# choi403/ALG

Measured on AMD Instinct MI355X. Metric: frames/sec (whole node) CogVideoX-5B-I2V 49f x 50-step ALG, higher is better.
Workload: dtype bf16; 1 GPU; BASELINE config 2: CogVideoX-5B-I2V bf16, 49 frames @ 480x720, 50 steps, ALG interval down_up (resize_factor 0.25, interval [0, 0.04]), guidance 6.0; one video per GPU; layers=42, dit_sample_forwards=12, parallelism=dp1

## Files before the change

alg_amd/_lib.py:

```python
from __future__ import annotations

import ctypes
from collections import OrderedDict
import os
from ctypes import POINTER, Structure, byref, c_char_p, c_float, c_int, c_int32, c_int64, c_void_p

import torch

_HERE = os.path.dirname(os.path.abspath(__file__))
LIB_PATH = os.environ.get("ALG_HIP_LIB") or os.path.join(_HERE, "libalg_hip.so")

ALG_F32, ALG_BF16 = 0, 1
ACT_NONE, ACT_GELU_TANH, ACT_SILU = 0, 1, 2
GEMM_BIAS_PER_ROW, GEMM_PERMUTE_COLS, GEMM_GATE_F32, GEMM_GATE_SEG_STRIDE = 1, 4, 8, 16
GEMM_B_PACKED11 = 32

EXPORTS = (
    "alg_version", "alg_last_error", "alg_reload_env", "alg_down_up", "alg_gaussian_blur", "alg_cfg_ddim_step", "alg_gemm_bf16", "alg_gemm_bf16_pair", "alg_gemm_bf16_pair_qk", "alg_pack_b_p11", "alg_pack_b_p11_bytes",
    "alg_flash_attn_d64", "alg_layernorm_modulate", "alg_layernorm_modulate_fp8", "alg_qk_norm_rope", "alg_patchify", "alg_unpatchify",
    "alg_timestep_embedding", "alg_cfg_combine", "alg_lincomb", "alg_unipc_update", "alg_concat_cast", "alg_flash_attn_d128", "alg_layernorm_mod_f32", "alg_layernorm_mod_f32_fp8", "alg_rmsnorm_rope",
    "alg_wan_modulation", "alg_patchify3d", "alg_unpatchify3d", "alg_timestep_embedding_f32", "alg_linear_f32",
    "alg_gelu_erf", "alg_layernorm_modulate_seg", "alg_headnorm_rope", "alg_masked_mean", "alg_silu", "alg_gemm_fp8", "alg_quantize_fp8_rows",
    "alg_conv_cl_bf16", "alg_vae_groupnorm_workspace", "alg_vae_groupnorm_stats", "alg_vae_spatial_norm", "alg_vae_upsample",
    "alg_vae_pack_latent", "alg_vae_unpack_video", "alg_vae_group_norm", "alg_vae_pad", "alg_vae_repitch",
    "alg_vae_unpack_planes", "alg_rms_norm_rows", "alg_softmax_hilo", "alg_flash_attn_d128_ex", "alg_flash_attn_d128_dual", "alg_rope_half", "alg_patchify_t", "alg_unpatchify_t", "alg_qk_norm_rope_scaled", "alg_flash_attn_d64_ex", "alg_embed_rows", "alg_t5_layernorm", "alg_attn_bias", "alg_mul_bf16", "alg_quick_gelu",
    "alg_lowpass_tables_bytes", "alg_lowpass_tables_build", "alg_down_up_workspace_bytes", "alg_gaussian_blur_workspace_bytes",
    "alg_flash_attn_d64_workspace_bytes", "alg_calib_mfma_bf16", "alg_wall_clock_khz", "alg_attn_clock_tap",
    "alg_flash_attn_d128_fp8", "alg_quantize_fp8_khead", "alg_quantize_fp8_vt", "alg_rmsnorm_rope_fp8", "alg_headnorm_rope_fp8",
)
_RET_I64 = ("alg_vae_groupnorm_workspace", "alg_lowpass_tables_bytes", "alg_down_up_workspace_bytes",
            "alg_gaussian_blur_workspace_bytes", "alg_flash_attn_d64_workspace_bytes", "alg_pack_b_p11_bytes")


class AlgHipError(RuntimeError):
    pass


class GemmArgs(Structure):
    _fields_ = [
        ("A", c_void_p), ("B", c_void_p), ("C", c_void_p), ("bias", c_void_p), ("R", c_void_p), ("gate", c_void_p),
        ("lda", c_int64), ("ldb", c_int64), ("ldc", c_int64), ("ldr", c_int64),
        ("strideA", c_int64), ("strideB", c_int64), ("strideC", c_int64), ("strideR", c_int64),
        ("strideGate", c_int64),
        ("M", c_int32), ("N", c_int32), ("K", c_int32), ("batch", c_int32),
        ("seg_split", c_int32), ("act", c_int32), ("flags", c_int32),
        ("gate_seg_stride", c_int64), ("perm_col0", c_int32), ("conv_cin_log2", c_int32),
        ("a_scale", c_void_p), ("b_scale", c_void_p), ("strideAScale", c_int64), ("strideBScale", c_int64),
        ("conv_wp", c_int32), ("conv_hpwp", c_int32), ("conv_kw", c_int32), ("reserved1", c_int32),
    ]


class QkNormRopeArgs(Structure):
    _fields_ = [("wq", c_void_p), ("bq", c_void_p), ("wk", c_void_p), ("bk", c_void_p), ("cos_tab", c_void_p),
                ("sin_tab", c_void_p), ("heads", c_int32), ("text_len", c_int32), ("eps", c_float),
                ("q_scale", c_float)]


class VaeGeom(Structure):
    _fields_ = [(n, c_int32) for n in ("frames", "H", "W", "C", "first_len", "seg_len", "lat_first_single", "lat_rate",
                                       "lat_scale", "lat_h", "lat_w")]


_lib = None


def build_library(verbose=False):
    import subprocess

    src = os.path.join(_HERE, "csrc")
    r = subprocess.run(["make", "-C", src, "-j8"], capture_output=True, text=True)
    if verbose or r.returncode != 0:
        print(r.stdout[-4000:])
        print(r.stderr[-4000:])
    if r.returncode != 0:
        raise AlgHipError("building libalg_hip.so failed (see output above)")
    return LIB_PATH


def load_library():
    global _lib
    if _lib is not None:
        return _lib
    if not os.path.exists(LIB_PATH):
        raise AlgHipError(
            "%s not found: the HIP extension is not built (run `python -c 'import __graft_entry__ as g; g.build()'` "
            "or `make -C alg_amd/csrc`).  There is no CPU fallback for the ALG hot path." % LIB_PATH)
    lib = ctypes.CDLL(LIB_PATH)
    lib.alg_version.restype = c_int
    lib.alg_last_error.restype = c_char_p
    lib.alg_reload_env.restype = None
    lib.alg_reload_env.argtypes = []
    lib.alg_down_up.argtypes = [c_void_p, c_void_p, c_int64, c_int, c_int, c_int, c_int, c_int, c_int, c_void_p, c_void_p,
                                c_int64, c_void_p]
    lib.alg_gaussian_blur.argtypes = [c_void_p, c_void_p, c_int64, c_int, c_int, c_int, c_float, c_int, c_void_p, c_int64,
                                      c_void_p]
    lib.alg_lowpass_tables_bytes.argtypes = [c_int] * 4
    lib.alg_lowpass_tables_build.argtypes = [c_void_p, c_int64] + [c_int] * 4 + [c_void_p]
    lib.alg_down_up_workspace_bytes.argtypes = [c_int64] + [c_int] * 4
    lib.alg_gaussian_blur_workspace_bytes.argtypes = [c_int64] + [c_int] * 3
    lib.alg_flash_attn_d64_workspace_bytes.argtypes = [c_int] * 4
    lib.alg_pack_b_p11_bytes.argtypes = [c_int, c_int]
    lib.alg_pack_b_p11_bytes.restype = c_int64
    lib.alg_pack_b_p11.argtypes = [c_void_p, c_void_p, c_int, c_int, c_int64, c_void_p]
    lib.alg_cfg_ddim_step.argtypes = [c_void_p, c_int, c_void_p, c_int, c_int, c_int64, c_float, c_float, c_float,
                                      c_float, c_float, c_void_p]
    lib.alg_cfg_combine.argtypes = [c_void_p, c_void_p, c_int, c_int, c_int64, c_float, c_void_p]
    lib.alg_lincomb.argtypes = [POINTER(c_void_p), POINTER(c_float), POINTER(c_int), c_int, c_void_p, c_int, c_int64,
                                c_void_p]
    lib.alg_concat_cast.argtypes = [POINTER(c_void_p), c_int, POINTER(c_void_p), c_int, c_int] + [c_int64] * 7 + [
        c_void_p, c_int, c_void_p]
    lib.alg_flash_attn_d128.argtypes = [c_void_p] * 4 + [c_int] * 4 + [c_int64] * 8 + [c_float, c_void_p]
    lib.alg_flash_attn_d128_ex.argtypes = [c_void_p] * 4 + [c_int] * 4 + [c_int64] * 8 + [c_float, c_int, c_int, c_void_p]
    lib.alg_flash_attn_d128_dual.argtypes = ([c_void_p] * 3 + [c_int] + [c_int64] * 4 + [c_void_p] * 2 + [c_int] + [c_int64] * 4 +
                                             [c_void_p] + [c_int] * 3 + [c_int64] * 4 + [c_float, c_void_p])
    lib.alg_flash_attn_d128_fp8.argtypes = [c_void_p] * 7 + [c_int] * 4 + [c_int64] * 8 + [c_float, c_int, c_int, c_void_p]
    lib.alg_quantize_fp8_khead.argtypes = [c_void_p, c_int64, c_int64, c_void_p, c_int64, c_int64, c_void_p] + [c_int] * 4 + [c_void_p]
    lib.alg_quantize_fp8_vt.argtypes = [c_void_p, c_int64, c_int64, c_void_p, c_int64, c_int64, c_void_p] + [c_int] * 4 + [c_void_p]
    lib.alg_rmsnorm_rope_fp8.argtypes = [c_void_p] * 4 + [c_int64, c_int, c_int, c_int, c_float, c_void_p, c_int64, c_void_p,
                                         c_void_p, c_void_p]
    lib.alg_headnorm_rope_fp8.argtypes = [c_void_p] * 4 + [c_int64, c_int64, c_int, c_int, c_int, c_int, c_float, c_void_p, c_int64,
                                          c_int64, c_void_p, c_int64, c_void_p, c_void_p]
    lib.alg_rope_half.argtypes = [c_void_p, c_void_p, c_void_p, c_void_p, c_int64, c_int, c_int64, c_void_p]
    lib.alg_layernorm_mod_f32.argtypes = [c_void_p] * 6 + [c_int64, c_int, c_int, c_int, c_float, c_void_p]
    lib.alg_layernorm_mod_f32_fp8.argtypes = [c_void_p] * 7 + [c_int64, c_int, c_int, c_int, c_float, c_void_p]
    lib.alg_rmsnorm_rope.argtypes = [c_void_p] * 4 + [c_int64, c_int, c_int, c_int, c_float, c_void_p]
    lib.alg_wan_modulation.argtypes = [c_void_p] * 3 + [c_int] * 5 + [c_void_p]
    lib.alg_patchify3d.argtypes = [c_void_p, c_void_p] + [c_int] * 8 + [c_void_p]
    lib.alg_unpatchify3d.argtypes = [c_void_p, c_int64, c_void_p] + [c_int] * 8 + [c_void_p]
    lib.alg_layernorm_modulate_seg.argtypes = [c_void_p] * 6 + [c_int64, c_int64, c_int, c_int, c_int, c_int64, c_int64,
                                               c_int, c_float, c_void_p]
    lib.alg_headnorm_rope.argtypes = [c_void_p] * 4 + [c_int64, c_int64, c_int, c_int, c_int, c_int, c_float, c_void_p]
    lib.alg_masked_mean.argtypes = [c_void_p, c_void_p, c_void_p, c_int, c_int, c_int, c_void_p]
    lib.alg_silu.argtypes = [c_void_p, c_void_p, c_int64, c_void_p]
    lib.alg_rms_norm_rows.argtypes = [c_void_p, c_void_p, c_void_p, c_int64, c_int, c_int, c_int, c_void_p]
    lib.alg_softmax_hilo.argtypes = [c_void_p, c_void_p, c_void_p, c_int64, c_int, c_int64, ctypes.c_float, c_void_p]
    lib.alg_gemm_fp8.argtypes = [POINTER(GemmArgs), c_void_p]
    lib.alg_conv_cl_bf16.argtypes = [c_void_p] * 5 + [c_int] * 7 + [c_void_p]
    lib.alg_vae_groupnorm_workspace.argtypes = [POINTER(VaeGeom)]
    lib.alg_vae_groupnorm_stats.argtypes = [c_void_p, POINTER(VaeGeom), c_float, c_void_p, c_void_p, c_void_p]
    lib.alg_vae_spatial_norm.argtypes = [c_void_p] * 6 + [POINTER(VaeGeom), c_int, c_void_p]
    lib.alg_vae_group_norm.argtypes = [c_void_p] * 5 + [POINTER(VaeGeom), c_int, c_void_p]
    lib.alg_vae_pad.argtypes = [c_void_p, c_void_p] + [c_int] * 4 + [c_void_p]
    lib.alg_vae_repitch.argtypes = [c_void_p, c_void_p] + [c_int] * 6 + [c_void_p]
    lib.alg_vae_unpack_planes.argtypes = [c_void_p, c_void_p] + [c_int] * 4 + [c_void_p]
    lib.alg_embed_rows.argtypes = [c_void_p, c_void_p, c_void_p, c_int64, c_int, c_int, c_void_p]
    lib.alg_t5_layernorm.argtypes = [c_void_p, c_void_p, c_void_p, c_int64, c_int, c_float, c_void_p]
    lib.alg_attn_bias.argtypes = [c_void_p] * 7 + [c_int, c_int, c_int, c_int, c_int64, c_int64, c_float, c_int, c_void_p]
    lib.alg_quick_gelu.argtypes = [c_void_p, c_int64, c_void_p]
    lib.alg_mul_bf16.argtypes = [c_void_p, c_void_p, c_void_p, c_int64, c_void_p]
    lib.alg_vae_upsample.argtypes = [c_void_p, c_void_p] + [c_int] * 6 + [c_void_p]
    lib.alg_vae_pack_latent.argtypes = [c_void_p, c_int64, c_int64, c_void_p, c_int, c_int, c_int, c_int, c_float, c_void_p]
    lib.alg_vae_unpack_video.argtypes = [c_void_p, c_void_p, c_int, c_int, c_int, c_int, c_void_p]
    lib.alg_quantize_fp8_rows.argtypes = [c_void_p, c_int64, c_void_p, c_void_p, c_int64, c_int, c_void_p]
    lib.alg_timestep_embedding_f32.argtypes = [c_void_p, c_void_p, c_int, c_int, c_void_p]
    lib.alg_linear_f32.argtypes = [c_void_p] * 6 + [c_int] * 4 + [c_void_p]
    lib.alg_gelu_erf.argtypes = [c_void_p, c_int64, c_void_p]
    lib.alg_unipc_update.argtypes = [c_void_p] * 5 + [c_int64] + [c_float] * 6 + [c_void_p]
    lib.alg_gemm_bf16.argtypes = [POINTER(GemmArgs), c_void_p]
    lib.alg_gemm_bf16_pair.argtypes = [POINTER(GemmArgs), POINTER(GemmArgs), c_void_p]
    lib.alg_gemm_bf16_pair_qk.argtypes = [POINTER(GemmArgs), POINTER(GemmArgs), POINTER(QkNormRopeArgs), c_void_p]
    lib.alg_flash_attn_d64.argtypes = [c_void_p, c_void_p, c_void_p, c_void_p, c_int, c_int, c_int, c_int64, c_int64,
                                       c_int64, c_int64, c_int64, c_int64, c_float, c_void_p]
    lib.alg_layernorm_modulate.argtypes = [c_void_p, c_void_p, c_void_p, c_void_p, c_void_p, c_void_p, c_int64, c_int,
                                           c_int, c_int, c_int64, c_int64, c_int, c_float, c_void_p]
    lib.alg_layernorm_modulate_fp8.argtypes = [c_void_p] * 7 + [c_int64, c_int, c_int, c_int, c_int64, c_int, c_float, c_void_p]
    lib.alg_qk_norm_rope.argtypes = [c_void_p, c_void_p, c_void_p, c_void_p, c_void_p, c_void_p, c_void_p, c_int,
                                     c_int, c_int, c_int, c_float, c_void_p]
    lib.alg_qk_norm_rope_scaled.argtypes = [c_void_p] * 7 + [c_int, c_int, c_int, c_int, c_float, c_float, c_void_p]
    lib.alg_flash_attn_d64_ex.argtypes = [c_void_p, c_void_p, c_void_p, c_void_p, c_int, c_int, c_int, c_int64, c_int64,
                                          c_int64, c_int64, c_int64, c_int64, c_float, c_int, c_void_p, c_int64, c_void_p]
    lib.alg_patchify.argtypes = [c_void_p, c_int64, POINTER(c_void_p), c_void_p, c_int, c_int, c_int, c_int, c_int,
                                 c_int, c_void_p]
    lib.alg_unpatchify.argtypes = [c_void_p, c_void_p, c_int, c_int, c_int, c_int, c_int, c_int, c_void_p]
    lib.alg_patchify_t.argtypes = [c_void_p, c_int64, POINTER(c_void_p), c_void_p] + [c_int] * 7 + [c_void_p]
    lib.alg_unpatchify_t.argtypes = [c_void_p, c_void_p] + [c_int] * 7 + [c_void_p]
    lib.alg_timestep_embedding.argtypes = [c_void_p, c_void_p, c_int, c_int, c_int, c_void_p]
    lib.alg_calib_mfma_bf16.argtypes = [c_void_p, c_int, ctypes.c_uint, c_int, c_void_p, c_void_p]
    lib.alg_attn_clock_tap.argtypes = [c_void_p, c_int]
    for name in EXPORTS:
        fn = getattr(lib, name)
        if name == "alg_attn_clock_tap":
            fn.restype = None
        elif name not in ("alg_version", "alg_last_error", "alg_reload_env"):
            fn.restype = c_int64 if name in _RET_I64 else c_int
    _lib = lib
    return lib


def reload_env():
    load_library().alg_reload_env()


def _check(rc, what):
    if rc != 0:
        msg = load_library().alg_last_error()
        raise AlgHipError("%s failed (code %d): %s" % (what, rc, msg.decode() if msg else "?"))


def _stream():
    return c_void_p(torch.cuda.current_stream().cuda_stream)


def _dt(t):
    if t.dtype == torch.float32:
        return ALG_F32
    if t.dtype == torch.bfloat16:
        return ALG_BF16
    raise AlgHipError("unsupported dtype %s (the HIP path handles float32 and bfloat16)" % t.dtype)


def _dev(t, name):
    if not t.is_cuda:
        raise AlgHipError("%s must be a device tensor: the ALG hot path is HIP-only (no CPU fallback)" % name)
    return t


def _ptr(t):
    return c_void_p(t.data_ptr()) if t is not None else c_void_p(0)



_TABLES = OrderedDict()
_TABLES_MAX = 64
_SCRATCH = {}
_PINNED = {}


def _stream_key(t):
    return (t.device.index, torch.cuda.current_stream(t.device).cuda_stream)


def _capturing():
    return torch.cuda.is_available() and torch.cuda.is_current_stream_capturing()


def _pin(t):
    _PINNED[id(t)] = t
    return t


def release_captured_buffers():
    _PINNED.clear()


def clear_caches():
    _TABLES.clear()
    _SCRATCH.clear()


def lowpass_tables(x, h1, w1):
    lib = load_library()
    H, W = x.shape[-2:]
    key = _stream_key(x) + (H, W, h1, w1)
    cap = _capturing()
    t = _TABLES.get(key)
    if t is not None:
        _TABLES.move_to_end(key)
        return _pin(t) if cap else t
    n = int(lib.alg_lowpass_tables_bytes(H, W, h1, w1))
    if n <= 0:
        return None
    t = torch.empty(n, dtype=torch.uint8, device=x.device)
    _check(lib.alg_lowpass_tables_build(_ptr(t), n, H, W, h1, w1, _stream()), "alg_lowpass_tables_build")
    if cap:
        return _pin(t)
    _TABLES[key] = t
    while len(_TABLES) > _TABLES_MAX:
        _TABLES.popitem(last=False)
    return t


def scratch(ref, nbytes, tag):
    if nbytes <= 0:
        return None
    key = _stream_key(ref) + (tag,)
    t = _SCRATCH.get(key)
    cap = _capturing()
    if t is None or t.numel() < nbytes:
        t = torch.empty(int(nbytes), dtype=torch.uint8, device=ref.device)
        if cap:
            return _pin(t)
        _SCRATCH[key] = t
    return _pin(t) if cap else t


def calib_mfma_bf16(sink, iters, seed=1, blocks=0, clocks=None):
    lib = load_library()
    if clocks is not None:
        if int(blocks) <= 0:
            blocks = 2 * torch.cuda.get_device_properties(sink.device).multi_processor_count
        if not (clocks.is_cuda and clocks.device == sink.device and clocks.dtype == torch.int64 and clocks.is_contiguous()
                and clocks.numel() >= 4 * int(blocks)):
            raise AlgHipError("calib_mfma_bf16: clocks must be a contiguous int64 tensor on the sink's device with >= 4 * %d "
                              "elements" % int(blocks))
    rc = lib.alg_calib_mfma_bf16(_ptr(_dev(sink, "sink")), int(iters), int(seed), int(blocks), _ptr(clocks), _stream())
    if rc <= 0:
        _check(rc if rc < 0 else -1, "alg_calib_mfma_bf16")
    return rc


def wall_clock_khz():
    return int(load_library().alg_wall_clock_khz())


def attn_clock_tap(buffer):
    lib = load_library()
    if buffer is None:
        lib.alg_attn_clock_tap(None, 0)
        return
    if not (buffer.is_cuda and buffer.dtype == torch.int64 and buffer.is_contiguous() and buffer.dim() == 2 and buffer.shape[1] == 4):
        raise AlgHipError("attn_clock_tap needs a contiguous int64 device tensor [slots, 4]")
    lib.alg_attn_clock_tap(_ptr(buffer), int(buffer.shape[0]))


def clock_mhz_from_taps(taps, wall_khz):
    t = taps.detach().cpu().to(torch.float64)
    dc, dw = t[:, 2] - t[:, 0], t[:, 3] - t[:, 1]
    ok = (dc > 0) & (dw > 0)
    if not bool(ok.any()) or wall_khz <= 0:
        return None
    mhz = dc[ok] / dw[ok] * (wall_khz / 1e3)
    return {"mean": float(mhz.mean()), "min": float(mhz.min()), "max": float(mhz.max()), "workgroups": int(ok.sum())}


def down_up(x, h1, w1, round_intermediate=True):
    lib = load_library()
    _dev(x, "x")
    if not x.is_contiguous():
        raise AlgHipError("down_up needs a contiguous tensor")
    H, W = x.shape[-2:]
    planes = x.numel() // (H * W) if x.numel() else 0
    out = torch.empty_like(x)
    if planes == 0:
        return out
    wsb = int(lib.alg_down_up_workspace_bytes(planes, H, W, h1, w1))
    ws = scratch(x, wsb, "down_up")
    tables = lowpass_tables(x, h1, w1) if wsb == 0 else None
    _check(lib.alg_down_up(_ptr(x), _ptr(out), planes, H, W, h1, w1, _dt(x), 1 if round_intermediate else 0,
                           _ptr(tables), _ptr(ws), wsb, _stream()), "alg_down_up")
    return out


def gaussian_blur(x, ksize, sigma):
    lib = load_library()
    _dev(x, "x")
    if not x.is_contiguous():
        raise AlgHipError("gaussian_blur needs a contiguous tensor")
    H, W = x.shape[-2:]
    planes = x.numel() // (H * W) if x.numel() else 0
    out = torch.empty_like(x)
    wsb = int(lib.alg_gaussian_blur_workspace_bytes(planes, H, W, int(ksize))) if planes else 0
    ws = scratch(x, wsb, "gaussian")
    _check(lib.alg_gaussian_blur(_ptr(x), _ptr(out), planes, H, W, int(ksize), float(sigma), _dt(x), _ptr(ws), wsb,
                                 _stream()), "alg_gaussian_blur")
    return out


def cfg_ddim_step_(pred, latents, n_pass, guidance_scale, sqrt_alpha_t, sqrt_beta_t, coef_a, coef_b):
    lib = load_library()
    _dev(pred, "pred")
    _dev(latents, "latents")
    if not (pred.is_contiguous() and latents.is_contiguous()):
        raise AlgHipError("cfg_ddim_step_ needs contiguous tensors")
    numel = latents.numel()
    if pred.numel() != n_pass * numel:
        raise AlgHipError("pred has %d elements, expected n_pass*numel = %d" % (pred.numel(), n_pass * numel))
    _check(lib.alg_cfg_ddim_step(_ptr(pred), _dt(pred), _ptr(latents), _dt(latents), n_pass, numel,
                                 float(guidance_scale), float(sqrt_alpha_t), float(sqrt_beta_t), float(coef_a),
                                 float(coef_b), _stream()), "alg_cfg_ddim_step")
    return latents


def cfg_combine(pred, n_pass, guidance_scale):
    lib = load_library()
    _dev(pred, "pred")
    if not pred.is_contiguous() or pred.shape[0] % n_pass:
        raise AlgHipError("cfg_combine needs a contiguous [n_pass * B, ...] tensor")
    out = torch.empty((pred.shape[0] // n_pass,) + tuple(pred.shape[1:]), device=pred.device, dtype=pred.dtype)
    _check(lib.alg_cfg_combine(_ptr(pred), _ptr(out), _dt(pred), n_pass, out.numel(), float(guidance_scale), _stream()),
           "alg_cfg_combine")
    return out


def lincomb(terms, out_dtype, out=None):
    lib = load_library()
    xs = [t for _, t in terms]
    for t in xs:
        _dev(t, "term")
        if not t.is_contiguous() or t.shape != xs[0].shape:
            raise AlgHipError("lincomb needs contiguous tensors of one shape")
    n = len(xs)
    if out is None:
        out = torch.empty(xs[0].shape, device=xs[0].device, dtype=out_dtype)
    elif out.dtype != out_dtype or out.shape != xs[0].shape or not out.is_contiguous():
        raise AlgHipError("lincomb: `out` must be a contiguous tensor of the requested dtype and shape")
    arr = (c_void_p * n)(*[t.data_ptr() for t in xs])
    cf = (c_float * n)(*[float(c) for c, _ in terms])
    dts = (c_int * n)(*[_dt(t) for t in xs])
    _check(lib.alg_lincomb(arr, cf, dts, n, _ptr(out), ALG_F32 if out_dtype == torch.float32 else ALG_BF16,
                           out.numel(), _stream()), "alg_lincomb")
    return out


def concat_cast(src0, src1, O, A0, A1, R, s0_ostride, s1_ostride, a1_off, out_dtype):
    lib = load_library()
    n = len(src0)
    for t in list(src0) + list(src1):
        _dev(t, "concat source")
        if not t.is_contiguous():
            raise AlgHipError("concat_cast needs contiguous sources")
    out = torch.empty((n, O, A0 + A1, R), device=src0[0].device, dtype=out_dtype)
    a0 = (c_void_p * n)(*[t.data_ptr() for t in src0])
    a1 = (c_void_p * n)(*[t.data_ptr() for t in src1])
    _check(lib.alg_concat_cast(a0, _dt(src0[0]), a1, _dt(src1[0]), n, O, A0, A1, R, s0_ostride, s1_ostride, a1_off,
                               _ptr(out), ALG_F32 if out_dtype == torch.float32 else ALG_BF16, _stream()),
           "alg_concat_cast")
    return out


def rope_half_(x, cos, sin, pos, rows, heads, x_rstride, x_off=0):
    _check(load_library().alg_rope_half(_p(x, x_off), _p(cos), _p(sin), _p(pos), rows, heads, x_rstride, _stream()),
           "alg_rope_half")
    return x


def flash_attn_d128_dual(q, k, vt, Skv, k_bs, k_rs, vt_bs, vt_rs, k2, vt2, Skv2, k2_bs, k2_rs, vt2_bs, vt2_rs, o, batch, heads, Sq,
                         q_bs, q_rs, o_bs, o_rs, scale):
    lib = load_library()
    for t in (q, k, vt, k2, vt2, o):
        _dev(t, "attention operand")
    _check(lib.alg_flash_attn_d128_dual(_p(q), _p(k), _p(vt), Skv, k_bs, k_rs, vt_bs, vt_rs, _p(k2), _p(vt2), Skv2, k2_bs, k2_rs,
                                        vt2_bs, vt2_rs, _p(o), batch, heads, Sq, q_bs, q_rs, o_bs, o_rs, float(scale), _stream()),
           "alg_flash_attn_d128_dual")
    return o


def flash_attn_d128(q, k, vt, o, batch, heads, Sq, Skv, q_bs, q_rs, k_bs, k_rs, vt_bs, vt_rs, o_bs, o_rs, scale,
                    q_off=0, k_off=0, vt_off=0, o_off=0, kv_group=1, causal=False):
    lib = load_library()
    for t in (q, k, vt, o):
        _dev(t, "attention operand")
    at = lambda t, off: c_void_p(t.data_ptr() + 2 * off)
    if kv_group != 1 or causal:
        _check(lib.alg_flash_attn_d128_ex(at(q, q_off), at(k, k_off), at(vt, vt_off), at(o, o_off), batch, heads, Sq, Skv, q_bs,
                                          q_rs, k_bs, k_rs, vt_bs, vt_rs, o_bs, o_rs, float(scale), int(kv_group),
                                          int(bool(causal)), _stream()), "alg_flash_attn_d128_ex")
        return o
    _check(lib.alg_flash_attn_d128(at(q, q_off), at(k, k_off), at(vt, vt_off), at(o, o_off), batch, heads, Sq, Skv, q_bs, q_rs, k_bs, k_rs, vt_bs, vt_rs, o_bs, o_rs, float(scale),
                                   _stream()), "alg_flash_attn_d128")
    return o


def flash_attn_d128_fp8(q8, q_scale, k8, k_scale, vt8, vt_scale, o, batch, heads, Sq, Skv, q_bs, q_rs, k_bs, k_rs, vt_bs, vt_rs,
                        o_bs, o_rs, scale, q_off=0, qs_off=0, k_off=0, ks_off=0, vt_off=0, vts_off=0, o_off=0, kv_group=1,
                        causal=False):
    lib = load_library()
    for t in (q8, q_scale, k8, k_scale, vt8, vt_scale, o):
        _dev(t, "attention operand")
    for t in (q8, k8, vt8):
        if t.element_size() != 1:
            raise AlgHipError("flash_attn_d128_fp8 takes e4m3 bytes (uint8 / float8_e4m3fn), got %s" % t.dtype)
    _check(lib.alg_flash_attn_d128_fp8(_p(q8, q_off), _p(q_scale, qs_off), _p(k8, k_off), _p(k_scale, ks_off), _p(vt8, vt_off),
                                       _p(vt_scale, vts_off), _p(o, o_off), batch, heads, Sq, Skv, q_bs, q_rs, k_bs, k_rs, vt_bs,
                                       vt_rs, o_bs, o_rs, float(scale), int(kv_group), int(bool(causal)), _stream()),
           "alg_flash_attn_d128_fp8")
    return o


def quantize_fp8_khead(x, q, scale, batch, heads, S, x_bs, x_rs, q_bs, q_rs, x_off=0, q_off=0, scale_off=0, scale_given=False):
    _check(load_library().alg_quantize_fp8_khead(_p(x, x_off), x_bs, x_rs, _p(q, q_off), q_bs, q_rs, _p(scale, scale_off), batch,
                                                 heads, S, int(bool(scale_given)), _stream()), "alg_quantize_fp8_khead")
    return q, scale


def quantize_fp8_vt(x, q, scale, batch, rows, Skv, x_bs, x_rs, q_bs, q_rs, src_permuted=True, x_off=0, q_off=0, scale_off=0):
    _check(load_library().alg_quantize_fp8_vt(_p(x, x_off), x_bs, x_rs, _p(q, q_off), q_bs, q_rs, _p(scale, scale_off), batch,
                                              rows, Skv, int(bool(src_permuted)), _stream()), "alg_quantize_fp8_vt")
    return q, scale


def rmsnorm_rope_fp8(x, weight, cos, sin, x_rstride, batch, rows, D, eps, q8, q8_rstride, scale=None, head_scale=None, x_off=0,
                     q8_off=0, scale_off=0, hs_off=0):
    _check(load_library().alg_rmsnorm_rope_fp8(_p(x, x_off), _p(weight), _p(cos), _p(sin), x_rstride, batch, rows, D, float(eps),
                                               _p(q8, q8_off), q8_rstride, _p(scale, scale_off), _p(head_scale, hs_off), _stream()),
           "alg_rmsnorm_rope_fp8")
    return q8


def headnorm_rope_fp8(x, weight, cos, sin, x_rstride, x_bstride, batch, rows, heads, rope_tokens, eps, q8, q8_rstride, q8_bstride,
                      scale=None, scale_bstride=0, head_scale=None, x_off=0, q8_off=0, scale_off=0, hs_off=0):
    _check(load_library().alg_headnorm_rope_fp8(_p(x, x_off), _p(weight), _p(cos), _p(sin), x_rstride, x_bstride, batch, rows,
                                                heads, rope_tokens, float(eps), _p(q8, q8_off), q8_rstride, q8_bstride,
                                                _p(scale, scale_off), scale_bstride, _p(head_scale, hs_off), _stream()),
           "alg_headnorm_rope_fp8")
    return q8


def _p(t, off=0):
    if t is None:
        return c_void_p(0)
    _dev(t, "tensor")
    return c_void_p(t.data_ptr() + off * t.element_size())


def layernorm_mod_f32(x, y, weight, bias, scale, shift, mod_bstride, batch, rows, D, eps, scale_off=0, shift_off=0):
    _check(load_library().alg_layernorm_mod_f32(_p(x), _p(y), _p(weight), _p(bias), _p(scale, scale_off),
                                                _p(shift, shift_off), mod_bstride, batch, rows, D, float(eps), _stream()),
           "alg_layernorm_mod_f32")
    return y


def layernorm_mod_f32_fp8(x, q8, q8_scale, weight, bias, scale, shift, mod_bstride, batch, rows, D, eps, scale_off=0,
                          shift_off=0):
    _check(load_library().alg_layernorm_mod_f32_fp8(_p(x), _p(q8), _p(q8_scale), _p(weight), _p(bias),
                                                    _p(scale, scale_off), _p(shift, shift_off), mod_bstride, batch, rows,
                                                    D, float(eps), _stream()), "alg_layernorm_mod_f32_fp8")
    return q8


def rmsnorm_rope_(x, weight, cos, sin, x_rstride, batch, rows, D, eps, x_off=0):
    _check(load_library().alg_rmsnorm_rope(_p(x, x_off), _p(weight), _p(cos), _p(sin), x_rstride, batch, rows, D,
                                           float(eps), _stream()), "alg_rmsnorm_rope")
    return x


def wan_modulation(table, vec, out, layers, batch, J, D, vec_per_j):
    _check(load_library().alg_wan_modulation(_p(table), _p(vec), _p(out), layers, batch, J, D, int(vec_per_j), _stream()),
           "alg_wan_modulation")
    return out


def patchify3d(x, out, n, C, F, H, W, ph, pw, Kpad):
    _check(load_library().alg_patchify3d(_p(x), _p(out), n, C, F, H, W, ph, pw, Kpad, _stream()), "alg_patchify3d")
    return out


def unpatchify3d(x, ldin, out, n, C, F, H, W, ph, pw, channel_major=False):
    _check(load_library().alg_unpatchify3d(_p(x), ldin, _p(out), n, C, F, H, W, ph, pw, int(channel_major), _stream()),
           "alg_unpatchify3d")
    return out


def layernorm_modulate_seg(x, y, weight, bias, scale, shift, mod_bstride, seg_stride, batch, rows, D, seg_split, eps,
                           x_bstride=None, y_bstride=None, x_off=0, y_off=0, scale_off=0, shift_off=0):
    x_bstride = rows * D if x_bstride is None else x_bstride
    y_bstride = rows * D if y_bstride is None else y_bstride
    _check(load_library().alg_layernorm_modulate_seg(_p(x, x_off), _p(y, y_off), _p(weight), _p(bias), _p(scale, scale_off),
                                                     _p(shift, shift_off), mod_bstride, seg_stride, batch, rows, D,
                                                     x_bstride, y_bstride, seg_split, float(eps), _stream()),
           "alg_layernorm_modulate_seg")
    return y


def headnorm_rope_(x, weight, cos, sin, x_rstride, x_bstride, batch, rows, heads, rope_tokens, eps, x_off=0):
    _check(load_library().alg_headnorm_rope(_p(x, x_off), _p(weight), _p(cos), _p(sin), x_rstride, x_bstride, batch, rows,
                                            heads, rope_tokens, float(eps), _stream()), "alg_headnorm_rope")
    return x


def masked_mean(x, valid, out, batch, L, D):
    _check(load_library().alg_masked_mean(_p(x), _p(valid), _p(out), batch, L, D, _stream()), "alg_masked_mean")
    return out


def silu(x, y):
    _check(load_library().alg_silu(_p(x), _p(y), x.numel(), _stream()), "alg_silu")
    return y


def rms_norm_rows(x, gamma, y, rows, C, Cp, silu=True):
    _check(load_library().alg_rms_norm_rows(_p(x), _p(gamma), _p(y), rows, C, Cp, int(silu), _stream()), "alg_rms_norm_rows")
    return y


def softmax_hilo(neg_hi, lo, p, rows, cols, ld, scale):
    _check(load_library().alg_softmax_hilo(_p(neg_hi), _p(lo), _p(p), rows, cols, ld, float(scale), _stream()),
           "alg_softmax_hilo")
    return p


CONV_PLAIN, CONV_PAIR, CONV_STRIDE2 = 0, 1, 2


def conv_cl(x, w, bias, res, y, frames, Hp, Wp, Cin, Cout, kt, pair=False, stride2=False, x_off=0, y_off=0, res_off=0):
    mode = CONV_STRIDE2 if stride2 else (CONV_PAIR if pair else CONV_PLAIN)
    _check(load_library().alg_conv_cl_bf16(_p(x, x_off), _p(w), _p(bias), _p(res, res_off), _p(y, y_off), frames, Hp, Wp,
                                           Cin, Cout, kt, mode, _stream()), "alg_conv_cl_bf16")
    return y


def embed_rows(ids, table, out):
    _check(load_library().alg_embed_rows(_p(ids), _p(table), _p(out), ids.numel(), table.shape[1], table.shape[0],
                                         _stream()), "alg_embed_rows")
    return out


def t5_layernorm(x, weight, y, rows, D, eps):
    _check(load_library().alg_t5_layernorm(_p(x), _p(weight), _p(y), rows, D, eps, _stream()), "alg_t5_layernorm")
    return y


def attn_bias(qkv, out, bias_table, rel_bucket, key_mask, batch, heads, L, scale=1.0, head_dim=64, causal=False):
    inner = heads * head_dim
    _check(load_library().alg_attn_bias(_p(qkv), _p(qkv, inner), _p(qkv, 2 * inner), _p(out), _p(bias_table),
                                        _p(rel_bucket), _p(key_mask), batch, heads, head_dim, L, 3 * inner, inner,
                                        float(scale), int(causal), _stream()), "alg_attn_bias")
    return out


def quick_gelu_(x):
    _check(load_library().alg_quick_gelu(_p(x), x.numel(), _stream()), "alg_quick_gelu")
    return x


def mul_bf16(a, b, out):
    _check(load_library().alg_mul_bf16(_p(a), _p(b), _p(out), a.numel(), _stream()), "alg_mul_bf16")
    return out


def vae_group_norm(x, stats, gamma, beta, out, g, silu=True):
    _check(load_library().alg_vae_group_norm(_p(x), _p(stats), _p(gamma), _p(beta), _p(out), byref(g), int(silu),
                                             _stream()), "alg_vae_group_norm")
    return out


def vae_pad(x, out, frames, H, W, C):
    _check(load_library().alg_vae_pad(_p(x), _p(out), frames, H, W, C, _stream()), "alg_vae_pad")
    return out


def vae_repitch(x, out, frames, H, W, C, src_rows, src_wp):
    _check(load_library().alg_vae_repitch(_p(x), _p(out), frames, H, W, C, src_rows, src_wp, _stream()), "alg_vae_repitch")
    return out


def vae_unpack_planes(x, out, frames, H, W, C):
    _check(load_library().alg_vae_unpack_planes(_p(x), _p(out), frames, H, W, C, _stream()), "alg_vae_unpack_planes")
    return out


def pack_conv_pair(w, bias, taps_t):
    co = w.shape[0]
    w = w.reshape(co, taps_t, 3, 3, -1)
    wp = w.new_zeros(2, co, taps_t, 3, 4, w.shape[-1])
    wp[0, :, :, :, 0:3] = w
    wp[1, :, :, :, 1:4] = w
    return wp.reshape(2 * co, -1).contiguous(), torch.cat([bias, bias]).contiguous()


def vae_geom(**kw):
    g = VaeGeom()
    for k, v in kw.items():
        setattr(g, k, v)
    return g


def vae_groupnorm_workspace(g):
    n = load_library().alg_vae_groupnorm_workspace(byref(g))
    if n < 0:
        _check(1, "alg_vae_groupnorm_workspace")
    return n


def vae_groupnorm_stats(x, g, eps, workspace, stats):
    _check(load_library().alg_vae_groupnorm_stats(_p(x), byref(g), eps, _p(workspace), _p(stats), _stream()),
           "alg_vae_groupnorm_stats")
    return stats


def vae_spatial_norm(x, stats, gamma, beta, zyb, out, g, silu=True):
    _check(load_library().alg_vae_spatial_norm(_p(x), _p(stats), _p(gamma), _p(beta), _p(zyb), _p(out), byref(g),
                                               int(silu), _stream()), "alg_vae_spatial_norm")
    return out


def vae_upsample(x, out, frames_out, H, W, C, compress_time, first_single):
    _check(load_library().alg_vae_upsample(_p(x), _p(out), frames_out, H, W, C, int(compress_time), int(first_single),
                                           _stream()), "alg_vae_upsample")
    return out


def vae_pack_latent(z, c_stride, frame_stride, out, frames, h, w, channels, scale, z_off=0):
    _check(load_library().alg_vae_pack_latent(_p(z, z_off), c_stride, frame_stride, _p(out), frames, h, w, channels, scale,
                                              _stream()), "alg_vae_pack_latent")
    return out


def vae_unpack_video(x, out, frames, H, W, to_uint8=False):
    _check(load_library().alg_vae_unpack_video(_p(x), _p(out), frames, H, W, int(to_uint8), _stream()),
           "alg_vae_unpack_video")
    return out


def timestep_embedding_f32(t, out, n, dim):
    _check(load_library().alg_timestep_embedding_f32(_p(t), _p(out), n, dim, _stream()), "alg_timestep_embedding_f32")
    return out


def linear_f32(x, W, b, y, y_bf16, y_silu_bf16, M, N, K, act=0):
    _check(load_library().alg_linear_f32(_p(x), _p(W), _p(b), _p(y), _p(y_bf16), _p(y_silu_bf16), M, N, K, act, _stream()),
           "alg_linear_f32")


def gelu_erf_(x):
    _check(load_library().alg_gelu_erf(_p(x), x.numel(), _stream()), "alg_gelu_erf")
    return x


def unipc_update(x, m0, m1, m_new, r, c, k, rk=1.0, rho0=0.0, rho_new=0.0):
    lib = load_library()
    for t in (x, m0, m1, m_new):
        if t is None:
            continue
        _dev(t, "unipc term")
        if t.dtype != torch.float32 or not t.is_contiguous() or t.shape != x.shape:
            raise AlgHipError("unipc_update needs contiguous fp32 tensors of one shape")
    out = torch.empty_like(x)
    p = lambda t: None if t is None else _ptr(t)
    _check(lib.alg_unipc_update(p(x), p(m0), p(m1), p(m_new), _ptr(out), x.numel(), float(r), float(c), float(k),
                                float(rk), float(rho0), float(rho_new), _stream()), "alg_unipc_update")
    return out


def gemm_args(A, B, C, M, N, K, lda, ldb, ldc, bias=None, R=None, ldr=0, gate=None, batch=1, strideA=0, strideB=0,
              strideC=0, strideR=0, strideGate=0, seg_split=0, act=ACT_NONE, flags=0, a_off=0, b_off=0, c_off=0, r_off=0,
              gate_off=0, gate_seg_stride=None, bias_off=0, perm_col0=0, a_scale=None, b_scale=None, strideAScale=0,
              strideBScale=0, a_scale_off=0, b_scale_off=0):
    args = GemmArgs()
    fp8 = a_scale is not None
    if isinstance(B, PackedB):
        if fp8:
            raise AlgHipError("a packed B holds bf16 weight fragments for GEMM schedule 11: the e4m3 GEMM takes a row-major B")
        if (B.N, B.K) != (N, K) or b_off or strideB:
            raise AlgHipError("packed B was built for N = %d, K = %d (shared by the batch, no offset)" % (B.N, B.K))
        flags |= GEMM_B_PACKED11
    args.A = A.data_ptr() + A.element_size() * a_off
    args.B = B.data_ptr() + B.element_size() * b_off
    if fp8:
        args.a_scale = a_scale.data_ptr() + 4 * a_scale_off
        args.b_scale = b_scale.data_ptr() + 4 * b_scale_off
        args.strideAScale, args.strideBScale = strideAScale, strideBScale
    args.C = C.data_ptr() + 2 * c_off
    args.bias = (bias.data_ptr() + 2 * bias_off) if bias is not None else None
    if gate_seg_stride is not None:
        flags |= GEMM_GATE_SEG_STRIDE
        args.gate_seg_stride = gate_seg_stride
    args.R = (R.data_ptr() + 2 * r_off) if R is not None else None
    args.gate = (gate.data_ptr() + gate.element_size() * gate_off) if gate is not None else None
    args.lda, args.ldb, args.ldc, args.ldr = lda, ldb, ldc, ldr
    args.strideA, args.strideB, args.strideC, args.strideR, args.strideGate = strideA, strideB, strideC, strideR, strideGate
    args.M, args.N, args.K, args.batch = M, N, K, batch
    args.seg_split, args.act, args.flags = seg_split, act, flags
    args.perm_col0 = perm_col0
    return args, fp8


class PackedB:

    def __init__(self, w):
        lib = load_library()
        _dev(w, "weight")
        if w.dtype != torch.bfloat16 or w.dim() != 2 or w.stride(1) != 1:
            raise AlgHipError("PackedB takes a 2-D bf16 weight with unit column stride")
        self.N, self.K = int(w.shape[0]), int(w.shape[1])
        nbytes = int(lib.alg_pack_b_p11_bytes(self.N, self.K))
        if nbytes <= 0:
            raise AlgHipError("PackedB: K = %d must be a positive multiple of 64" % self.K)
        self.data = torch.empty(nbytes, dtype=torch.uint8, device=w.device)
        _check(lib.alg_pack_b_p11(_ptr(w), _ptr(self.data), self.N, self.K, int(w.stride(0)), _stream()), "alg_pack_b_p11")

    def data_ptr(self):
        return self.data.data_ptr()

    def element_size(self):
        return 2


def gemm(*a, **kw):
    lib = load_library()
    args, fp8 = gemm_args(*a, **kw)
    if fp8:
        _check(lib.alg_gemm_fp8(ctypes.byref(args), _stream()), "alg_gemm_fp8")
    else:
        _check(lib.alg_gemm_bf16(ctypes.byref(args), _stream()), "alg_gemm_bf16")


def gemm_pair(first, second):
    lib = load_library()
    a, fa = gemm_args(*first[0], **first[1])
    b, fb = gemm_args(*second[0], **second[1])
    if fa or fb:
        raise AlgHipError("gemm_pair takes bf16 problems")
    _check(lib.alg_gemm_bf16_pair(ctypes.byref(a), ctypes.byref(b), _stream()), "alg_gemm_bf16_pair")


def gemm_pair_qk(first, second, wq, bq, wk, bk, cos, sin, heads, text_len, eps, q_scale=1.0):
    lib = load_library()
    a, fa = gemm_args(*first[0], **first[1])
    b, fb = gemm_args(*second[0], **second[1])
    if fa or fb:
        raise AlgHipError("gemm_pair_qk takes bf16 problems")
    ptrs = [t.data_ptr() if t is not None else None for t in (wq, bq, wk, bk, cos, sin)]
    e = QkNormRopeArgs(*ptrs, heads, text_len, float(eps), float(q_scale))
    _check(lib.alg_gemm_bf16_pair_qk(ctypes.byref(a), ctypes.byref(b), ctypes.byref(e), _stream()), "alg_gemm_bf16_pair_qk")


def quantize_fp8_rows(x, q, scale, rows, K, x_rstride=None, x_off=0, q_off=0, scale_off=0):
    x_rstride = K if x_rstride is None else x_rstride
    _check(load_library().alg_quantize_fp8_rows(_p(x, x_off), x_rstride, _p(q, q_off), _p(scale, scale_off), rows, K,
                                                _stream()), "alg_quantize_fp8_rows")
    return q, scale


ATTN_Q_PRESCALED = 1


def flash_attn_d64(q, k, vt, o, batch, heads, S, q_bstride, q_rstride, vt_bstride, vt_rstride, o_bstride, o_rstride,
                   scale, q_off=0, k_off=0, q_prescaled=False):
    lib = load_library()
    flags = ATTN_Q_PRESCALED if q_prescaled else 0
    wsb = int(lib.alg_flash_attn_d64_workspace_bytes(batch, heads, S, flags))
    ws = scratch(o, wsb, "attn_d64")
    _check(lib.alg_flash_attn_d64_ex(c_void_p(q.data_ptr() + 2 * q_off), c_void_p(k.data_ptr() + 2 * k_off), _ptr(vt),
                                     _ptr(o), batch, heads, S, q_bstride, q_rstride, vt_bstride, vt_rstride, o_bstride,
                                     o_rstride, float(scale), flags, _ptr(ws), wsb, _stream()),
           "alg_flash_attn_d64")


def layernorm_modulate(x, y, weight, bias, scale, shift, mod_bstride, batch, rows, D, seg_split, eps,
                       x_bstride=None, y_bstride=None, x_off=0, y_off=0, scale_off=0, shift_off=0):
    lib = load_library()
    x_bstride = rows * D if x_bstride is None else x_bstride
    y_bstride = rows * D if y_bstride is None else y_bstride
    sc = c_void_p(scale.data_ptr() + 2 * scale_off) if scale is not None else c_void_p(0)
    sh = c_void_p(shift.data_ptr() + 2 * shift_off) if shift is not None else c_void_p(0)
    _check(lib.alg_layernorm_modulate(c_void_p(x.data_ptr() + 2 * x_off), c_void_p(y.data_ptr() + 2 * y_off),
                                      _ptr(weight), _ptr(bias), sc, sh, mod_bstride, batch, rows, D, x_bstride,
                                      y_bstride, seg_split, float(eps), _stream()), "alg_layernorm_modulate")


def layernorm_modulate_fp8(x, q8, q8_scale, weight, bias, scale, shift, mod_bstride, batch, rows, D, seg_split, eps,
                           x_bstride=None, x_off=0, scale_off=0, shift_off=0, q8_off=0, q8_scale_off=0):
    x_bstride = rows * D if x_bstride is None else x_bstride
    _check(load_library().alg_layernorm_modulate_fp8(_p(x, x_off), _p(q8, q8_off), _p(q8_scale, q8_scale_off), _p(weight), _p(bias),
                                                     _p(scale, scale_off), _p(shift, shift_off), mod_bstride, batch, rows, D,
                                                     x_bstride, seg_split, float(eps), _stream()), "alg_layernorm_modulate_fp8")
    return q8, q8_scale


def qk_norm_rope_(qk, wq, bq, wk, bk, cos, sin, batch, S, heads, text_len, eps, q_scale=1.0):
    lib = load_library()
    _check(lib.alg_qk_norm_rope_scaled(_ptr(qk), _ptr(wq), _ptr(bq), _ptr(wk), _ptr(bk), _ptr(cos), _ptr(sin), batch, S,
                                       heads, text_len, float(eps), float(q_scale), _stream()), "alg_qk_norm_rope")


def patchify(latents, lat_bstride, conds, out, n_samples, frames, C, H, W, p, p_t=1):
    lib = load_library()
    arr = (c_void_p * n_samples)(*[c.data_ptr() for c in conds])
    _check(lib.alg_patchify_t(_ptr(latents), lat_bstride, arr, _ptr(out), n_samples, frames, C, H, W, p, p_t, _stream()),
           "alg_patchify")


def unpatchify(x, out, n_samples, frames, C, H, W, p, p_t=1):
    lib = load_library()
    _check(lib.alg_unpatchify_t(_ptr(x), _ptr(out), n_samples, frames, C, H, W, p, p_t, _stream()), "alg_unpatchify")


def timestep_embedding(t, out, n, dim, flip_sin_to_cos=True):
    lib = load_library()
    _check(lib.alg_timestep_embedding(_ptr(t), _ptr(out), n, dim, 1 if flip_sin_to_cos else 0, _stream()),
           "alg_timestep_embedding")
```

alg_amd/csrc/gemm.hip:

```cpp
#include <stdlib.h>

#include "common.h"

namespace alg {
constexpr int BM = 256, BN = 256;
int launch_gemm_p6(const alg_gemm_args* a, int m_tiles, int n_tiles, int64_t nwg, hipStream_t s);
int launch_gemm_p9(const alg_gemm_args* a, int m_tiles, int n_tiles, int64_t nwg, hipStream_t s);
int launch_gemm_p9_pair(const alg_gemm_args* a, int m_tiles_a, int n_tiles_a, const alg_gemm_args* b, int m_tiles_b, int n_tiles_b,
                        hipStream_t s);
int launch_gemm_p9_pair_qk(const alg_gemm_args* a, int m_tiles_a, int n_tiles_a, const alg_gemm_args* b, int m_tiles_b, int n_tiles_b,
                           const alg_qk_norm_rope_args* e, hipStream_t s);
int launch_gemm_p10(const alg_gemm_args* a, int m_tiles, int n_tiles, int64_t nwg, hipStream_t s);
int launch_gemm_p10_pair(const alg_gemm_args* a, int m_tiles_a, int n_tiles_a, const alg_gemm_args* b, int m_tiles_b, int n_tiles_b,
                         hipStream_t s);
int launch_gemm_p10_pair_qk(const alg_gemm_args* a, int m_tiles_a, int n_tiles_a, const alg_gemm_args* b, int m_tiles_b, int n_tiles_b,
                            const alg_qk_norm_rope_args* e, hipStream_t s);
int launch_gemm_p11(const alg_gemm_args* a, int m_tiles, int n_tiles, int64_t nwg, hipStream_t s);
int launch_gemm_p6_fp8(const alg_gemm_args* a, int m_tiles, int n_tiles, int64_t nwg, hipStream_t s);
int launch_gemm_p9_fp8(const alg_gemm_args* a, int m_tiles, int n_tiles, int64_t nwg, hipStream_t s);
int launch_gemm_p6_conv(const alg_gemm_args* a, int m_tiles, int n_tiles, int64_t nwg, hipStream_t s);
static int gemm_pipe() { return opt(OPT_GEMM_PIPE); }
static bool asm_pipe() { return gemm_pipe() == 9 || gemm_pipe() == 10; }
}

using namespace alg;

static int gemm_entry(const alg_gemm_args* a, void* stream, bool fp8, bool validate_only = false) {
  if (!a || !a->A || !a->B || !a->C) {
    set_error("alg_gemm_bf16: null argument");
    return ALG_EINVAL;
  }
  if (a->M <= 0 || a->N <= 0 || a->K <= 0 || a->batch <= 0) {
    set_error("alg_gemm_bf16: bad shape M=%d N=%d K=%d batch=%d", a->M, a->N, a->K, a->batch);
    return ALG_EINVAL;
  }
  if (a->K % (fp8 ? 128 : 64) != 0) {
    set_error("alg_gemm_%s: K=%d must be a multiple of %d", fp8 ? "fp8" : "bf16", a->K, fp8 ? 128 : 64);
    return ALG_EINVAL;
  }
  const int al = fp8 ? 16 : 8;
  if (a->lda % al || a->ldb % al || a->strideA % al || a->strideB % al || ((uintptr_t)a->A & 15) ||
      ((uintptr_t)a->B & 15)) {
    set_error("alg_gemm: A/B must be 16-byte aligned with lda/ldb/strides multiples of 16 bytes");
    return ALG_EINVAL;
  }
  if (fp8 && (!a->a_scale || !a->b_scale || ((uintptr_t)a->b_scale & 15) || (a->strideBScale & 3))) {
    set_error("alg_gemm_fp8: a_scale / b_scale are required (b_scale 16-byte aligned)");
    return ALG_EINVAL;
  }
  if (a->act < ALG_ACT_NONE || a->act > ALG_ACT_SILU) {
    set_error("alg_gemm_bf16: unknown activation %d", a->act);
    return ALG_EINVAL;
  }
  if ((a->flags & ALG_GEMM_PERMUTE_COLS) && (a->R || a->gate)) {
    set_error("alg_gemm_bf16: PERMUTE_COLS cannot be combined with residual/gate");
    return ALG_EINVAL;
  }
  if (a->R && a->act != ALG_ACT_NONE) {
    set_error("alg_gemm_bf16: an activation cannot be combined with the residual epilogue");
    return ALG_EINVAL;
  }
  if (a->gate && !a->R) {
    set_error("alg_gemm_bf16: gate needs a residual");
    return ALG_EINVAL;
  }
  if ((a->N & 3) == 0) {
    const bool bad = (a->ldc & 3) || (a->strideC & 3) || ((uintptr_t)a->C & 7) ||
                     (a->bias && !(a->flags & ALG_GEMM_BIAS_PER_ROW) && ((uintptr_t)a->bias & 7)) ||
                     (a->R && ((a->ldr & 3) || (a->strideR & 3) || ((uintptr_t)a->R & 7))) ||
                     (a->gate && ((a->strideGate & 3) ||
                                  ((uintptr_t)a->gate & ((a->flags & ALG_GEMM_GATE_F32) ? 15 : 7))));
    if (bad) {
      set_error("alg_gemm_bf16: C/bias/R/gate must be 8-byte aligned with ldc/ldr/strides multiples of 4 elements");
      return ALG_EINVAL;
    }
  }
  if (a->conv_wp) {
    const int cl = a->conv_cin_log2;
    const int taps = (cl >= 6 && cl <= 12) ? a->K >> cl : 0;
    const int kw = a->conv_kw;
    if (fp8 || (kw != 3 && kw != 4) || (taps != 3 * kw && taps != 9 * kw) || (taps << cl) != a->K ||
        (a->lda != ((int64_t)(kw - 2) << cl) && !(kw == 3 && a->lda == (2ll << cl))) || a->conv_wp < 3 ||
        a->conv_hpwp < 3 * a->conv_wp || a->act != ALG_ACT_NONE ||
        ((2ll * a->conv_hpwp + 2ll * a->conv_wp + 3) << cl) >= (1ll << 31)) {
      set_error("alg_gemm_bf16: bad convolution addressing (cin_log2=%d K=%d lda=%lld wp=%d hpwp=%d)", cl, a->K,
                (long long)a->lda, a->conv_wp, a->conv_hpwp);
      return ALG_EINVAL;
    }
  }
  if (a->flags & ALG_GEMM_B_PACKED11) {
    if (fp8) {
      set_error("alg_gemm_fp8: a packed B (ALG_GEMM_B_PACKED11) holds bf16 fragments for schedule 11; the e4m3 GEMM reads a row-major B");
      return ALG_EINVAL;
    }
    if (a->conv_wp) {
      set_error("alg_gemm_bf16: convolution addressing cannot be combined with a packed B (ALG_GEMM_B_PACKED11)");
      return ALG_EINVAL;
    }
    if (a->K < 128 || 256 * a->lda * 2 + (int64_t)a->K * 2 >= (1ll << 32) || a->strideB != 0 ||
        (a->flags & (ALG_GEMM_BIAS_PER_ROW | ALG_GEMM_PERMUTE_COLS)) || ((uintptr_t)a->B & 15)) {
      set_error("alg_gemm_bf16: a packed B (ALG_GEMM_B_PACKED11) needs K >= 128, 32-bit byte offsets inside a 256-row A panel, a B shared by "
                "the batch (strideB = 0) and a plain column layout (no per-row bias / column permutation)");
      return ALG_EINVAL;
    }
  }
  if (validate_only) return ALG_OK;
  if ((int64_t)a->M * a->ldc >= (1ll << 31) || (a->R && (int64_t)a->M * a->ldr >= (1ll << 31))) {
    const int64_t ld = (a->R && a->ldr > a->ldc) ? a->ldr : a->ldc;
    const int64_t rows = ((1ll << 31) - 1) / ld / BM * BM;
    if (a->conv_wp || rows <= 0) {
      set_error("alg_gemm_bf16: M*ldc must stay below 2^31 (32-bit epilogue offsets)");
      return ALG_ELIMIT;
    }
    const int64_t esz = fp8 ? 1 : 2;
    for (int64_t m0 = 0; m0 < a->M; m0 += rows) {
      alg_gemm_args c = *a;
      c.M = (int32_t)((a->M - m0) < rows ? (a->M - m0) : rows);
      c.A = (const char*)a->A + m0 * a->lda * esz;
      c.C = (char*)a->C + m0 * a->ldc * 2;
      if (a->R) c.R = (const char*)a->R + m0 * a->ldr * 2;
      if (a->bias && (a->flags & ALG_GEMM_BIAS_PER_ROW)) c.bias = (const char*)a->bias + m0 * 2;
      if (a->a_scale) c.a_scale = a->a_scale + m0;
      c.seg_split = a->seg_split > m0 ? (int32_t)(a->seg_split - m0) : 0;
      const int rc = gemm_entry(&c, stream, fp8);
      if (rc != ALG_OK) return rc;
    }
    return ALG_OK;
  }
  const int m_tiles = (a->M + BM - 1) / BM, n_tiles = (a->N + BN - 1) / BN;
  const int64_t nwg = (int64_t)m_tiles * n_tiles * a->batch;
  if (nwg > 0x7fffffff) {
    set_error("alg_gemm_bf16: grid too large");
    return ALG_ELIMIT;
  }
  hipStream_t s = (hipStream_t)stream;
  if (fp8) {
    if (asm_pipe() && a->K >= 256 && 256 * a->lda + (int64_t)a->K < (1ll << 32) && 256 * a->ldb + (int64_t)a->K < (1ll << 32))
      return launch_gemm_p9_fp8(a, m_tiles, n_tiles, nwg, s);
    return launch_gemm_p6_fp8(a, m_tiles, n_tiles, nwg, s);
  }
  if (a->conv_wp) return launch_gemm_p6_conv(a, m_tiles, n_tiles, nwg, s);
  if (a->flags & ALG_GEMM_B_PACKED11) return launch_gemm_p11(a, m_tiles, n_tiles, nwg, s);
  switch (gemm_pipe()) {
    case 9:
    case 10:
      if (a->K >= 128 && 256 * a->lda * 2 + (int64_t)a->K * 2 < (1ll << 32) && 256 * a->ldb * 2 + (int64_t)a->K * 2 < (1ll << 32))
        return gemm_pipe() == 10 ? launch_gemm_p10(a, m_tiles, n_tiles, nwg, s) : launch_gemm_p9(a, m_tiles, n_tiles, nwg, s);
      return launch_gemm_p6(a, m_tiles, n_tiles, nwg, s);
    default: return launch_gemm_p6(a, m_tiles, n_tiles, nwg, s);
  }
}

extern "C" int alg_gemm_bf16(const alg_gemm_args* a, void* stream) { return gemm_entry(a, stream, false); }

static bool pair_eligible(const alg_gemm_args* a) {
  return a && a->A && a->B && a->C && !(a->flags & ALG_GEMM_B_PACKED11) && !a->R && !a->gate && a->act == ALG_ACT_NONE &&
         !a->conv_wp && a->M > 0 && a->N > 0 && a->batch > 0 && a->K >= 128 && a->K % 64 == 0 && 256 * a->lda * 2 + (int64_t)a->K * 2 < (1ll << 32) &&
         256 * a->ldb * 2 + (int64_t)a->K * 2 < (1ll << 32) && (int64_t)a->M * a->ldc < (1ll << 31) &&
         !(a->lda % 8 || a->ldb % 8 || a->strideA % 8 || a->strideB % 8 || ((uintptr_t)a->A & 15) || ((uintptr_t)a->B & 15)) &&
         ((a->N & 3) != 0 || !((a->ldc & 3) || (a->strideC & 3) || ((uintptr_t)a->C & 7) ||
                               (a->bias && !(a->flags & ALG_GEMM_BIAS_PER_ROW) && ((uintptr_t)a->bias & 7))));
}

extern "C" int alg_gemm_bf16_pair(const alg_gemm_args* a, const alg_gemm_args* b, void* stream) {
  int rc = gemm_entry(a, stream, false, true);
  if (rc == ALG_OK) rc = gemm_entry(b, stream, false, true);
  if (rc != ALG_OK) return rc;
  if (asm_pipe() && pair_eligible(a) && pair_eligible(b)) {
    const int64_t ta = (int64_t)((a->M + BM - 1) / BM) * ((a->N + BN - 1) / BN) * a->batch;
    const int64_t tb = (int64_t)((b->M + BM - 1) / BM) * ((b->N + BN - 1) / BN) * b->batch;
    if (ta + tb <= 0x7fffffff)
      return (gemm_pipe() == 10 ? launch_gemm_p10_pair : launch_gemm_p9_pair)(a, (a->M + BM - 1) / BM, (a->N + BN - 1) / BN, b, (b->M + BM - 1) / BM, (b->N + BN - 1) / BN,
                                 (hipStream_t)stream);
  }
  rc = gemm_entry(a, stream, false);
  return rc != ALG_OK ? rc : gemm_entry(b, stream, false);
}

extern "C" int alg_gemm_bf16_pair_qk(const alg_gemm_args* a, const alg_gemm_args* b, const alg_qk_norm_rope_args* e, void* stream) {
  int rc = gemm_entry(a, stream, false, true);
  if (rc == ALG_OK) rc = gemm_entry(b, stream, false, true);
  if (rc != ALG_OK) return rc;
  if (!e || !e->wq || !e->bq || !e->wk || !e->bk || e->heads <= 0 || e->text_len < 0 || e->text_len > a->M ||
      (e->cos_tab == nullptr) != (e->sin_tab == nullptr)) {
    set_error("alg_gemm_bf16_pair_qk: bad LayerNorm / rotary arguments");
    return ALG_EINVAL;
  }
  if (((uintptr_t)e->wq & 15) || ((uintptr_t)e->bq & 15) || ((uintptr_t)e->wk & 15) || ((uintptr_t)e->bk & 15) ||
      ((uintptr_t)e->cos_tab & 15) || ((uintptr_t)e->sin_tab & 15) || ((uintptr_t)a->C & 15)) {
    set_error("alg_gemm_bf16_pair_qk: pointers must be 16-byte aligned");
    return ALG_EINVAL;
  }
  if (a->N != 2 * e->heads * 64 || a->ldc != a->N || a->strideC != (int64_t)a->M * a->N || (a->flags & ALG_GEMM_PERMUTE_COLS) ||
      a->R || a->act != ALG_ACT_NONE) {
    set_error("alg_gemm_bf16_pair_qk: qk must be a plain GEMM onto the contiguous [batch][S][2][heads][64] tensor (N=%d heads=%d ldc=%lld)",
              a->N, e->heads, (long long)a->ldc);
    return ALG_EINVAL;
  }
  const bool fused = asm_pipe() && pair_eligible(a) && pair_eligible(b) && e->heads % 4 == 0 &&
                     !(a->bias && (a->flags & ALG_GEMM_BIAS_PER_ROW));
  if (fused) {
    const int64_t ta = (int64_t)((a->M + BM - 1) / BM) * ((a->N + BN - 1) / BN) * a->batch;
    const int64_t tb = (int64_t)((b->M + BM - 1) / BM) * ((b->N + BN - 1) / BN) * b->batch;
    if (ta + tb <= 0x7fffffff)
      return (gemm_pipe() == 10 ? launch_gemm_p10_pair_qk : launch_gemm_p9_pair_qk)(a, (a->M + BM - 1) / BM, (a->N + BN - 1) / BN, b, (b->M + BM - 1) / BM, (b->N + BN - 1) / BN, e,
                                    (hipStream_t)stream);
  }
  rc = alg_gemm_bf16_pair(a, b, stream);
  if (rc != ALG_OK) return rc;
  return alg_qk_norm_rope_scaled(a->C, e->wq, e->bq, e->wk, e->bk, e->cos_tab, e->sin_tab, a->batch, a->M, e->heads, e->text_len,
                                 e->eps, e->q_scale, stream);
}

extern "C" int alg_gemm_fp8(const alg_gemm_args* a, void* stream) { return gemm_entry(a, stream, true); }

extern "C" int alg_conv_cl_bf16(const void* x, const void* w, const void* bias, const void* res, void* y, int frames,
                                int Hp, int Wp, int Cin, int Cout, int kt, int mode, void* stream) {
  const bool pair = mode == ALG_CONV_PAIR, down = mode == ALG_CONV_STRIDE2;
  if (frames <= 0 || Hp < 3 || Wp < 3 || (kt != 1 && kt != 3) || Cin < 64 || (Cin & (Cin - 1)) || Cout <= 0 || (Cout & 3) ||
      mode < 0 || mode > ALG_CONV_STRIDE2 || (pair && (((Hp * Wp) & 1) || Cout > 128)) ||
      (down && (kt != 1 || (Hp & 1) || (Wp & 1)))) {
    set_error("alg_conv_cl_bf16: bad shape frames=%d Hp=%d Wp=%d Cin=%d Cout=%d kt=%d (Cin a power of two >= 64, Cout %% 4 == 0)",
              frames, Hp, Wp, Cin, Cout, kt);
    return ALG_EINVAL;
  }
  alg_gemm_args a = {};
  a.A = x, a.B = w, a.C = y, a.bias = bias, a.R = res;
  const int vox = pair ? 2 : 1, kw = pair ? 4 : 3;
  a.lda = (int64_t)vox * Cin, a.ldb = (int64_t)kt * 3 * kw * Cin, a.ldc = (int64_t)vox * Cout, a.ldr = a.ldc;
  a.strideA = (int64_t)Hp * Wp * Cin, a.strideB = 0, a.strideC = (int64_t)Hp * Wp * Cout, a.strideR = a.strideC;
  a.M = Hp * Wp / vox, a.N = vox * Cout, a.K = kt * 3 * kw * Cin, a.batch = frames;
  a.act = ALG_ACT_NONE;
  a.conv_cin_log2 = __builtin_ctz((unsigned)Cin), a.conv_wp = Wp, a.conv_hpwp = Hp * Wp, a.conv_kw = kw;
  if (down) {
    a.A = (const bf16_t*)x + (int64_t)(Wp + 1) * Cin;
    a.lda = 2ll * Cin;
    a.M = (Hp - 2) / 2 * Wp;
    a.strideC = a.strideR = (int64_t)a.M * Cout;
  }
  return gemm_entry(&a, stream, false);
}
```

alg_amd/csrc/gemm_kernel.h:

```cpp
#pragma once
#include <stdlib.h>

#include <type_traits>

#include "common.h"
#include "qk_norm_rope.h"
#ifdef ALG_P9_LOOP_INC
#include ALG_P9_LOOP_INC
#else
#include "gemm_p9_loop.inc"
#endif
#include "gemm_p9_fp8_loop.inc"
#ifdef ALG_P11_LOOP_INC
#include ALG_P11_LOOP_INC
#else
#include "gemm_p11_loop.inc"
#endif
#ifdef ALG_P10_LOOP_INC
#include ALG_P10_LOOP_INC
#else
#include "gemm_p10_loop.inc"
#endif

#ifndef ALG_FP8_MX
#define ALG_FP8_MX 1
#endif

namespace alg {

#ifdef ALG_ABL_NOSTORE
#define ALG_STORE16(ptr, val) asm volatile("" ::"v"((val).x), "v"((val).y), "v"((val).z), "v"((val).w))
#else
#define ALG_STORE16(ptr, val) (*(uint4*)(ptr) = (val))
#endif
#ifdef ALG_GEMM_TAP
static __device__ uint64_t gemm_tap_buf[1024 * 4];
static inline int gemm_tap_read(uint64_t* host) { return hipMemcpyFromSymbol(host, HIP_SYMBOL(gemm_tap_buf), sizeof(uint64_t) * 4096) == hipSuccess ? 0 : -1; }
#endif

#ifndef ALG_AUX_A
#define ALG_AUX_A 0
#endif
#ifndef ALG_AUX_B
#define ALG_AUX_B 0
#endif
constexpr int BM = 256, BN = 256;
constexpr int GEMM_LDS = 128 * 1024;
constexpr int GEMM_LDS_P9 = 160 * 1024;
constexpr int GROUP_M = 8;

template <int V>
struct IntC { static constexpr int value = V; };

template <typename F, int... I>
__device__ __forceinline__ void static_for_impl(F&& f, std::integer_sequence<int, I...>) {
  (f(IntC<I>{}), ...);
}
template <int N, typename F>
__device__ __forceinline__ void static_for(F&& f) {
  static_for_impl(f, std::make_integer_sequence<int, N>{});
}

template <int BLK>
__device__ __forceinline__ f32x16 read_acc_block() {
  float f[16];
  asm volatile("v_accvgpr_read_b32 %0, a[%c16]\n\tv_accvgpr_read_b32 %1, a[%c17]\n\tv_accvgpr_read_b32 %2, a[%c18]\n\t"
               "v_accvgpr_read_b32 %3, a[%c19]\n\tv_accvgpr_read_b32 %4, a[%c20]\n\tv_accvgpr_read_b32 %5, a[%c21]\n\t"
               "v_accvgpr_read_b32 %6, a[%c22]\n\tv_accvgpr_read_b32 %7, a[%c23]\n\tv_accvgpr_read_b32 %8, a[%c24]\n\t"
               "v_accvgpr_read_b32 %9, a[%c25]\n\tv_accvgpr_read_b32 %10, a[%c26]\n\tv_accvgpr_read_b32 %11, a[%c27]\n\t"
               "v_accvgpr_read_b32 %12, a[%c28]\n\tv_accvgpr_read_b32 %13, a[%c29]\n\tv_accvgpr_read_b32 %14, a[%c30]\n\t"
               "v_accvgpr_read_b32 %15, a[%c31]\n\ts_nop 0"
               : "=v"(f[0]), "=v"(f[1]), "=v"(f[2]), "=v"(f[3]), "=v"(f[4]), "=v"(f[5]), "=v"(f[6]), "=v"(f[7]), "=v"(f[8]),
                 "=v"(f[9]), "=v"(f[10]), "=v"(f[11]), "=v"(f[12]), "=v"(f[13]), "=v"(f[14]), "=v"(f[15])
               : "n"(BLK * 16), "n"(BLK * 16 + 1), "n"(BLK * 16 + 2), "n"(BLK * 16 + 3), "n"(BLK * 16 + 4), "n"(BLK * 16 + 5),
                 "n"(BLK * 16 + 6), "n"(BLK * 16 + 7), "n"(BLK * 16 + 8), "n"(BLK * 16 + 9), "n"(BLK * 16 + 10),
                 "n"(BLK * 16 + 11), "n"(BLK * 16 + 12), "n"(BLK * 16 + 13), "n"(BLK * 16 + 14), "n"(BLK * 16 + 15)
               : ALG_GEMM_P9_ACC_CLOBBERS);
  f32x16 r;
#pragma unroll
  for (int e = 0; e < 16; ++e) r[e] = f[e];
  return r;
}

typedef const __attribute__((address_space(1))) void* gptr_t;
typedef __attribute__((address_space(3))) void* lptr_t;

__device__ __forceinline__ float act_apply(float x, int act) {
  if (act == ALG_ACT_GELU_TANH) {
    const float k1 = -2.0f * 1.4426950408889634f * 0.7978845608028654f, k2 = 0.044715f * k1;
    return x * __builtin_amdgcn_rcpf(1.0f + __builtin_amdgcn_exp2f(x * fmaf(k2, x * x, k1)));
  }
  if (act == ALG_ACT_SILU) {
    return x * __builtin_amdgcn_rcpf(1.0f + __builtin_amdgcn_exp2f(-1.4426950408889634f * x));
  }
  return x;
}

__device__ __forceinline__ void unpack4(const uint2 v, float (&f)[4]) {
  f[0] = __uint_as_float(v.x << 16);
  f[1] = __uint_as_float(v.x & 0xffff0000u);
  f[2] = __uint_as_float(v.y << 16);
  f[3] = __uint_as_float(v.y & 0xffff0000u);
}

struct GemmNoPair {};
struct GemmPairArgs {
  alg_gemm_args p;
  int m_tiles, n_tiles, group_m;
};
struct GemmPairQkArgs : GemmPairArgs {
  QkNormRope qe;
};
template <int PAIR> struct GemmPairT { typedef GemmNoPair type; };
template <> struct GemmPairT<1> { typedef GemmPairArgs type; };
template <> struct GemmPairT<2> { typedef GemmPairQkArgs type; };
template <int ACT, bool RES, int PIPE, int WNW = 4, bool FP8 = false, bool CONV = false, int PAIR = 0>
__global__ __launch_bounds__((PIPE == 11 ? 1 : 2) * WNW * 64) void gemm_bf16_kernel(
    const alg_gemm_args p1, int m_tiles1, int n_tiles1, int group_m1, const typename GemmPairT<PAIR>::type pr) {
  constexpr bool P9 = PIPE == 9 || PIPE == 10 || PIPE == 11;
  constexpr bool M16 = PIPE == 10 || PIPE == 11;
  constexpr bool P11 = PIPE == 11;
  constexpr int WMW = P11 ? 1 : 2;
  constexpr int MT = BM / WMW / 32;
  static_assert(!PAIR || (P9 && !P11 && !RES && ACT == ALG_ACT_NONE), "the pair launch is built for the plain schedule-9 / 10 kernels");
  static_assert(!FP8 || PIPE == 6 || PIPE == 9, "the fp8 operands are built on the ping-pong schedule and on schedule 9");
  static_assert(!CONV || (PIPE == 6 && !FP8), "the convolution addressing is built on the bf16 ping-pong schedule");
  typedef typename std::conditional<FP8, uint8_t, bf16_t>::type elem_t;
  constexpr int EPS = 16 / (int)sizeof(elem_t);
  constexpr int GEMM_THREADS = WMW * WNW * 64;
  constexpr int NT = BN / WNW / 32;
  static_assert(PIPE == 0 || PIPE == 6 || PIPE == 7 || PIPE == 8 || P9,
                "schedules built: 0 (2-stage ring), 6 (ping-pong), 7 (4-wave interleaved), 8 (4-wave BK = 32 ring), 9 / 10 (asm loops)");
  static_assert((PIPE == 7 || PIPE == 8 || PIPE == 9 || PIPE == 10) == (WNW == 2) && P11 == (WNW == 4 && WMW == 1),
                "PIPE 7 / 8 / 9 / 10 are the 2 x 2 4-wave layouts, 11 the 1 x 4 one, the others run 8 waves");
  static_assert(!P11 || (!FP8 && !CONV), "schedule 11 takes bf16 plain GEMM addressing with a packed B");
  static_assert(!P9 || !CONV, "schedules 9 / 10 take plain GEMM addressing (bf16, or e4m3 on 9 since round 4)");
  constexpr bool BK64 = true;
  constexpr bool PP = PIPE == 6;
  constexpr int BK = FP8 ? 128 : 64;
  constexpr int NSTAGE = 2;
  constexpr int ROW_BYTES = BK * (int)sizeof(elem_t);
  constexpr int SLOTS = ROW_BYTES / 16;
  constexpr int TILE_BYTES = BM * ROW_BYTES;
  constexpr int STAGE_BYTES = 2 * TILE_BYTES;
  constexpr int LD_PER_OP = TILE_BYTES / (GEMM_THREADS * 16);
  constexpr int ROWS_PER_LD = GEMM_THREADS / SLOTS;
  static_assert(NSTAGE * STAGE_BYTES == GEMM_LDS, "ring must fill the 128 KiB LDS budget");

  extern __shared__ __attribute__((aligned(16))) char smem[];
  const int tid = threadIdx.x;
  const int lane = tid & 63;
  const int wave = __builtin_amdgcn_readfirstlane(tid >> 6);
  const int wm = wave / WNW, wn = wave % WNW;

  constexpr int abl = 0;
#ifdef ALG_GEMM_TAP
  uint64_t tap_loop = 0, tap_tiles = 0;
  const uint64_t tap_c0 = __builtin_readcyclecounter(), tap_r0 = wall_clock64();
#endif
  group_m1 &= 0xffff;
  const int total1 = m_tiles1 * n_tiles1 * p1.batch;
  auto do_tile = [&](const int wg_in) __attribute__((always_inline)) {
  bool second = false;
  if constexpr (PAIR) second = wg_in >= total1;
  const alg_gemm_args& p = [&]() -> const alg_gemm_args& {
    if constexpr (PAIR) return second ? pr.p : p1;
    else return p1;
  }();
  int m_tiles = m_tiles1, n_tiles = n_tiles1, group_m = group_m1, wg = wg_in;
  if constexpr (PAIR) {
    if (second) m_tiles = pr.m_tiles, n_tiles = pr.n_tiles, group_m = pr.group_m, wg = wg_in - total1;
  }
  const int tiles = m_tiles * n_tiles;
  const int b = wg / tiles;
  int t = wg - b * tiles;
  const int grp = t / (group_m * n_tiles);
  const int first_m = grp * group_m;
  const int gsize = min(m_tiles - first_m, group_m);
  t -= grp * group_m * n_tiles;
  const int m0 = (first_m + t % gsize) * BM;
  const int n0 = (t / gsize) * BN;

  const elem_t* A = (const elem_t*)p.A + (int64_t)b * p.strideA;
  const elem_t* B = (const elem_t*)p.B + (int64_t)b * p.strideB;

  const int srow = tid / SLOTS;
  const int sw_src = !BK64 ? ((tid >> 4) & 3) : ((tid >> 4) & 7);
  const int sslot = (tid & (SLOTS - 1)) ^ sw_src;
  const elem_t* a_src[LD_PER_OP];
  const elem_t* b_src[LD_PER_OP];
#pragma unroll
  for (int i = 0; i < LD_PER_OP; ++i) {
    const int r = i * ROWS_PER_LD + srow;
    const int am = (abl & 8) ? 0 : m0, bn = (abl & 8) ? 0 : n0;
    a_src[i] = A + (int64_t)min(am + r, p.M - 1) * p.lda + sslot * EPS;
    b_src[i] = B + (int64_t)min(bn + r, p.N - 1) * p.ldb + sslot * EPS;
  }
  auto a_koff = [&](int kt) -> int {
    if constexpr (CONV) {
      const int cl = p.conv_cin_log2 - 6;
      const int tap = kt >> cl;
      const bool k4 = p.conv_kw == 4;
      const int dt = k4 ? tap / 12 : tap / 9, r9 = tap - dt * (k4 ? 12 : 9);
      const int dy = k4 ? r9 >> 2 : r9 / 3, dx = r9 - dy * (k4 ? 4 : 3);
      return ((dt * p.conv_hpwp + dy * p.conv_wp + dx) << p.conv_cin_log2) + (kt & ((1 << cl) - 1)) * BK;
    } else {
      return kt * BK;
    }
  };
  auto stage = [&](int buf, int kt) {
    char* base = smem + buf * STAGE_BYTES;
#pragma unroll
    for (int i = 0; i < LD_PER_OP; ++i) {
      __builtin_amdgcn_global_load_lds((gptr_t)(a_src[i] + kt * BK),
                                       (lptr_t)(base + (i * GEMM_THREADS + wave * 64) * 16), 16, 0, 0);
      __builtin_amdgcn_global_load_lds((gptr_t)(b_src[i] + kt * BK),
                                       (lptr_t)(base + TILE_BYTES + (i * GEMM_THREADS + wave * 64) * 16), 16, 0, 0);
    }
  };

  auto stage_piece = [&](int buf, int kt, int w) {
    char* base = smem + buf * STAGE_BYTES;
    const int i = w >> 1;
    if (w & 1)
      __builtin_amdgcn_global_load_lds((gptr_t)(b_src[i] + kt * BK),
                                       (lptr_t)(base + TILE_BYTES + (i * GEMM_THREADS + wave * 64) * 16), 16, 0, 0);
    else
      __builtin_amdgcn_global_load_lds((gptr_t)(a_src[i] + kt * BK),
                                       (lptr_t)(base + (i * GEMM_THREADS + wave * 64) * 16), 16, 0, 0);
  };

  const int l31 = lane & 31, h2 = lane >> 5;
  const int sw = !BK64 ? ((l31 >> 2) & 3) : ((l31 >> 1) & 7);
  const int a_row_off = (wm * 128 + l31) * ROW_BYTES;
  const int b_row_off = (wn * (NT * 32) + l31) * ROW_BYTES;
  auto pp_a_row = [&](int mt) { return ((mt >> 1) * 128 + wm * 64 + (mt & 1) * 32 + l31) * ROW_BYTES; };
  auto pp_b_row = [&](int nt) { return (nt * 128 + wn * 32 + l31) * ROW_BYTES; };

  auto fma_frag = [](const bf16x8 bfrag, const bf16x8 afrag, f32x16 c) -> f32x16 {
    if constexpr (FP8) {
      typedef long l2 __attribute__((ext_vector_type(2)));
      const l2 bq = __builtin_bit_cast(l2, bfrag), aq = __builtin_bit_cast(l2, afrag);
      c = __builtin_amdgcn_mfma_f32_32x32x16_fp8_fp8(bq[0], aq[0], c, 0, 0, 0);
      return __builtin_amdgcn_mfma_f32_32x32x16_fp8_fp8(bq[1], aq[1], c, 0, 0, 0);
    } else {
      return __builtin_amdgcn_mfma_f32_32x32x16_bf16(bfrag, afrag, c, 0, 0, 0);
    }
  };

  f32x16 acc[4][NT];
  if constexpr (!P9) {
#pragma unroll
    for (int i = 0; i < 4; ++i)
#pragma unroll
      for (int j = 0; j < NT; ++j)
#pragma unroll
        for (int e = 0; e < 16; ++e) acc[i][j][e] = 0.0f;
  }
  auto get_acc = [&](auto mt_c, auto nt_c) -> f32x16 {
    constexpr int mt = decltype(mt_c)::value, nt = decltype(nt_c)::value;
    if constexpr (P9)
      return read_acc_block<NT * mt + nt>();
    else
      return acc[mt][nt];
  };

  auto load_frags = [&](const char* As, const char* Bs, int ks, bf16x8 (&af)[4], bf16x8 (&bfr)[NT]) {
    const int so = ((2 * ks + h2) ^ sw) * 16;
#pragma unroll
    for (int nt = 0; nt < NT; ++nt) bfr[nt] = *(const bf16x8*)(Bs + b_row_off + nt * 32 * ROW_BYTES + so);
#pragma unroll
    for (int mt = 0; mt < 4; ++mt) af[mt] = *(const bf16x8*)(As + a_row_off + mt * 32 * ROW_BYTES + so);
  };
  auto mma = [&](const bf16x8 (&af)[4], const bf16x8 (&bfr)[NT]) {
#pragma unroll
    for (int mt = 0; mt < 4; ++mt)
#pragma unroll
      for (int nt = 0; nt < NT; ++nt)
        acc[mt][nt] = fma_frag(bfr[nt], af[mt], acc[mt][nt]);
  };
  auto compute = [&](int buf) {
    const char* As = smem + buf * STAGE_BYTES;
    const char* Bs = As + TILE_BYTES;
    constexpr int KS = BK / 16;
    bf16x8 af0[4], bf0[NT], af1[4], bf1[NT];
    load_frags(As, Bs, 0, af0, bf0);
    auto interleave = [&]() {
#pragma unroll
      for (int i = 0; i < 4 + NT; ++i) {
        __builtin_amdgcn_sched_group_barrier(0x008, 1, 0);
        __builtin_amdgcn_sched_group_barrier(0x100, 1, 0);
      }
      __builtin_amdgcn_sched_group_barrier(0x008, 4 * NT - (4 + NT), 0);
    };
    __builtin_amdgcn_sched_barrier(0);
#pragma unroll
    for (int ks = 0; ks < KS; ks += 2) {
      load_frags(As, Bs, ks + 1, af1, bf1);
      mma(af0, bf0);
      interleave();
      __builtin_amdgcn_sched_barrier(0);
      if (ks + 2 < KS) {
        load_frags(As, Bs, ks + 2, af0, bf0);
        mma(af1, bf1);
        interleave();
      } else {
        mma(af1, bf1);
      }
      __builtin_amdgcn_sched_barrier(0);
    }
  };

  const int nk = p.K / BK;
  if constexpr (PIPE == 0) {
    stage(0, 0);
    for (int kt = 0; kt < nk; ++kt) {
      asm volatile("s_waitcnt vmcnt(0)" ::: "memory");
      __syncthreads();
      if (kt + 1 < nk) stage((kt + 1) & 1, kt + 1);
      compute(kt & 1);
    }
  } else if constexpr (PIPE == 6) {
    auto stage_half = [&](int kt, int kind) {
      char* base = smem + (kt & 1) * STAGE_BYTES + (kind >> 1) * TILE_BYTES;
#pragma unroll
      for (int ii = 0; ii < 2; ++ii) {
        const int i = (kind & 1) * 2 + ii;
        const elem_t* src = (kind >> 1) ? b_src[i] + kt * BK : a_src[i] + a_koff(kt);
        if (kind >> 1)
          __builtin_amdgcn_global_load_lds((gptr_t)src, (lptr_t)(base + (i * GEMM_THREADS + wave * 64) * 16), 16, 0, ALG_AUX_B);
        else
          __builtin_amdgcn_global_load_lds((gptr_t)src, (lptr_t)(base + (i * GEMM_THREADS + wave * 64) * 16), 16, 0, ALG_AUX_A);
      }
    };
    bf16x8 af[2][4], b0f[4], b1f[4];
    auto load_a = [&](const char* As, int half) {
#pragma unroll
      for (int m2 = 0; m2 < 2; ++m2)
#pragma unroll
        for (int ks = 0; ks < 4; ++ks)
          af[m2][ks] = *(const bf16x8*)(As + pp_a_row(half * 2 + m2) + (((2 * ks + h2) ^ sw) * 16));
    };
    auto load_b = [&](const char* Bs, int half, bf16x8 (&bf)[4]) {
#pragma unroll
      for (int ks = 0; ks < 4; ++ks) bf[ks] = *(const bf16x8*)(Bs + pp_b_row(half) + (((2 * ks + h2) ^ sw) * 16));
    };
    auto quad = [&](int mh, int nt, const bf16x8 (&bf)[4]) {
      __builtin_amdgcn_s_setprio(1);
      if constexpr (FP8 && ALG_FP8_MX) {
        typedef int i8v __attribute__((ext_vector_type(8)));
        typedef int i4v __attribute__((ext_vector_type(4)));
        auto cat = [](const bf16x8 lo, const bf16x8 hi) -> i8v {
          const i4v l = __builtin_bit_cast(i4v, lo), h = __builtin_bit_cast(i4v, hi);
          return i8v{l[0], l[1], l[2], l[3], h[0], h[1], h[2], h[3]};
        };
#pragma unroll
        for (int kp = 0; kp < 2; ++kp) {
          const i8v bq = cat(bf[2 * kp], bf[2 * kp + 1]);
#pragma unroll
          for (int m2 = 0; m2 < 2; ++m2)
            acc[mh * 2 + m2][nt] = __builtin_amdgcn_mfma_scale_f32_32x32x64_f8f6f4(
                bq, cat(af[m2][2 * kp], af[m2][2 * kp + 1]), acc[mh * 2 + m2][nt], 0, 0, 0, 0x7f7f7f7f, 0, 0x7f7f7f7f);
        }
      } else {
#pragma unroll
        for (int ks = 0; ks < 4; ++ks)
#pragma unroll
          for (int m2 = 0; m2 < 2; ++m2)
            acc[mh * 2 + m2][nt] = fma_frag(bf[ks], af[m2][ks], acc[mh * 2 + m2][nt]);
      }
      __builtin_amdgcn_s_setprio(0);
    };
    auto enter_mfma = [&]() {
      asm volatile("s_waitcnt lgkmcnt(0)" ::: "memory");
      __builtin_amdgcn_s_barrier();
      __builtin_amdgcn_sched_barrier(0);
    };
    auto leave_mfma = [&]() {
      __builtin_amdgcn_sched_barrier(0);
      __builtin_amdgcn_s_barrier();
      __builtin_amdgcn_sched_barrier(0);
    };
    stage_half(0, 0); stage_half(0, 3); stage_half(0, 1); stage_half(0, 2);
    if (nk > 1) {
      stage_half(1, 0); stage_half(1, 3); stage_half(1, 1);
      asm volatile("s_waitcnt vmcnt(6)" ::: "memory");
    } else {
      asm volatile("s_waitcnt vmcnt(0)" ::: "memory");
    }
    __builtin_amdgcn_s_barrier();
    if (wm == 1) __builtin_amdgcn_s_barrier();
    for (int t = 0; t < nk; ++t) {
      const char* As = smem + (t & 1) * STAGE_BYTES;
      const char* Bs = As + TILE_BYTES;
      bool do_b0 = true, do_b1 = true;
      if constexpr (CONV) {
        if (p.conv_kw == 4 && p.N == 256) {
          const int dx = (t >> (p.conv_cin_log2 - 6)) & 3;
          do_b0 = dx != 3, do_b1 = dx != 0;
        }
      }
      load_a(As, 0);
      if (do_b0) load_b(Bs, 0, b0f);
      if (t + 1 < nk) stage_half(t + 1, 2);
      enter_mfma();
      if (do_b0) quad(0, 0, b0f);
      leave_mfma();
      if (do_b1) load_b(Bs, 1, b1f);
      if (t + 2 < nk) stage_half(t + 2, 0);
      enter_mfma();
      if (do_b1) quad(0, 1, b1f);
      leave_mfma();
      load_a(As, 1);
      if (t + 2 < nk) stage_half(t + 2, 3);
      enter_mfma();
      if (do_b1) quad(1, 1, b1f);
      leave_mfma();
      if (t + 2 < nk) {
        stage_half(t + 2, 1);
        asm volatile("s_waitcnt vmcnt(6)" ::: "memory");
      } else {
        asm volatile("s_waitcnt vmcnt(0)" ::: "memory");
      }
      enter_mfma();
      if (do_b0) quad(1, 0, b0f);
      leave_mfma();
    }
// ... 578 lines not shown
              gq[4] = gfb[nt].x; gq[5] = gfb[nt].y; gq[6] = gfb[nt].z; gq[7] = gfb[nt].w;
            }
            float y[8];
#pragma unroll
            for (int k = 0; k < 4; ++k) {
              const float x0 = __uint_as_float(u[k] << 16), x1 = __uint_as_float(u[k] & 0xffff0000u);
              const float r0f = __uint_as_float(ru[k] << 16), r1f = __uint_as_float(ru[k] & 0xffff0000u);
              if constexpr (KIND == 0) {
                y[2 * k] = r0f + x0;
                y[2 * k + 1] = r1f + x1;
              } else if constexpr (KIND == 1) {
                const uint32_t pk = pack_bf2(__uint_as_float(gu[k] << 16) * x0, __uint_as_float(gu[k] & 0xffff0000u) * x1);
                y[2 * k] = r0f + __uint_as_float(pk << 16);
                y[2 * k + 1] = r1f + __uint_as_float(pk & 0xffff0000u);
              } else {
                float m0_ = gq[2 * k] * x0, m1_ = gq[2 * k + 1] * x1;
                asm volatile("" : "+v"(m0_), "+v"(m1_));
                y[2 * k] = r0f + m0_;
                y[2 * k + 1] = r1f + m1_;
              }
            }
            if (ok) {
              uint4 outv;
              outv.x = pack_bf2(y[0], y[1]); outv.y = pack_bf2(y[2], y[3]);
              outv.z = pack_bf2(y[4], y[5]); outv.w = pack_bf2(y[6], y[7]);
              ALG_STORE16(cp + voff, outv);
            }
            __builtin_amdgcn_sched_barrier(0);
          });
        };
        if (gkind == 0) { res_loop(IntC<0>{}); return; }
        if (gkind == 1) { res_loop(IntC<1>{}); return; }
        if (gkind == 2) { res_loop(IntC<2>{}); return; }
      } else {
        const int lrow = lane_e >> 2, ch = lane_e & 3;
        const uint32_t voff = (uint32_t)(lrow * ldc + ch * 8) * 2;
        const char* ldsl = my + lrow * 64 + ((ch ^ ((lrow >> 2) & 3)) * 16);
        auto plain_loop = [&](auto perm_c) {
          constexpr bool PERM = decltype(perm_c)::value != 0;
          static_for<NIT / 8>([&](auto grp_c) {
            constexpr int g0 = decltype(grp_c)::value * 8;
            uint4 raw[8];
            static_for<8>([&](auto j_c) {
              constexpr int it = g0 + decltype(j_c)::value;
              raw[decltype(j_c)::value] = *(const uint4*)(ldsl + (it >> 1) * 2048 + (it & 1) * 1024);
            });
            static_for<8>([&](auto j_c) {
              constexpr int it = g0 + decltype(j_c)::value;
              constexpr int blk = it >> 1, mt = blk / NT, nt = blk % NT;
              const int r0 = m0 + blk_row(mt) + (it & 1) * 16, cb = n0 + blk_col(nt);
              const uint4 outv = raw[decltype(j_c)::value];
              if (lrow < p.M - r0 && ch * 8 < p.N - cb) {
                if constexpr (PERM) {
                  const int c0 = cb + ch * 8;
                  bf16_t* crow = Cb + (int64_t)(r0 + lrow) * ldc;
                  const int base = col0 + (c0 & ~12), b3 = (c0 >> 3) & 1;
                  *(uint2*)(crow + base + (b3 << 2)) = make_uint2(outv.x, outv.y);
                  *(uint2*)(crow + base + 8 + (b3 << 2)) = make_uint2(outv.z, outv.w);
                } else {
                  ALG_STORE16((char*)(Cb + (int64_t)r0 * ldc + cb) + voff, outv);
                }
              }
            });
            __builtin_amdgcn_sched_barrier(0);
          });
        };
        if constexpr (PAIR == 2) {
          if (!second) {
            const QkNormRope& e = pr.qe;
            const bool is_k = n0 >= e.heads * 64;
            const float qs = is_k ? 1.0f : e.q_scale;
            float wA[8], bA[8], wB[8], bB[8];
            unpack8(*(const uint4*)((is_k ? e.wk : e.wq) + ch * 8), wA);
            unpack8(*(const uint4*)((is_k ? e.wk : e.wq) + 32 + ch * 8), wB);
            unpack8(*(const uint4*)((is_k ? e.bk : e.bq) + ch * 8), bA);
            unpack8(*(const uint4*)((is_k ? e.bk : e.bq) + 32 + ch * 8), bB);
            const bool any_rope = e.cos_tab && e.text_len < p.M;
            float tab[2][32] = {};
            bool rp[2];
            auto fetch = [&](auto u_c) {
              constexpr int u = decltype(u_c)::value, slot = u & 1;
              const int srow = m0 + blk_row(u >> 1) + (u & 1) * 16 + lrow;
              rp[slot] = any_rope && srow >= e.text_len && srow < p.M;
              if (any_rope) {
                const int64_t pos = rp[slot] ? (int64_t)(srow - e.text_len) * 64 + ch * 8 : (int64_t)ch * 8;
                const float4 c0 = *(const float4*)(e.cos_tab + pos), c1 = *(const float4*)(e.cos_tab + pos + 4);
                const float4 c2 = *(const float4*)(e.cos_tab + pos + 32), c3 = *(const float4*)(e.cos_tab + pos + 36);
                const float4 s0 = *(const float4*)(e.sin_tab + pos), s1 = *(const float4*)(e.sin_tab + pos + 4);
                const float4 s2 = *(const float4*)(e.sin_tab + pos + 32), s3 = *(const float4*)(e.sin_tab + pos + 36);
                const float4 q[8] = {c0, c1, c2, c3, s0, s1, s2, s3};
#pragma unroll
                for (int k = 0; k < 8; ++k)
                  tab[slot][4 * k] = q[k].x, tab[slot][4 * k + 1] = q[k].y, tab[slot][4 * k + 2] = q[k].z, tab[slot][4 * k + 3] = q[k].w;
              }
            };
            fetch(IntC<0>{});
            static_for<8>([&](auto u_c) {
              constexpr int u = decltype(u_c)::value, mt = u >> 1, half = u & 1, slot = u & 1;
              uint4 raw[4];
              static_for<4>([&](auto nt_c) {
                constexpr int nt = decltype(nt_c)::value;
                raw[nt] = *(const uint4*)(ldsl + (mt * NT + nt) * 2048 + half * 1024);
              });
              const bool roped = rp[slot];
              float csA[8], csB[8], snA[8], snB[8];
#pragma unroll
              for (int k = 0; k < 8; ++k)
                csA[k] = tab[slot][k], csB[k] = tab[slot][8 + k], snA[k] = tab[slot][16 + k], snB[k] = tab[slot][24 + k];
              if constexpr (u + 1 < 8) fetch(IntC<u + 1>{});
              static_for<2>([&](auto hh_c) {
                constexpr int hh = decltype(hh_c)::value;
                uint4& ra = raw[2 * hh];
                uint4& rb = raw[2 * hh + 1];
                float va[8], vb[8];
                unpack8(ra, va);
                unpack8(rb, vb);
                float sa = qk_chunk_sum(va), sb = qk_chunk_sum(vb);
                sa += __shfl_xor(sa, 1, 64); sb += __shfl_xor(sb, 1, 64);
                sa += __shfl_xor(sa, 2, 64); sb += __shfl_xor(sb, 2, 64);
                const float mean = qk_mean(sa + sb);
                float qa = qk_chunk_sqdev(va, mean), qb = qk_chunk_sqdev(vb, mean);
                qa += __shfl_xor(qa, 1, 64); qb += __shfl_xor(qb, 1, 64);
                qa += __shfl_xor(qa, 2, 64); qb += __shfl_xor(qb, 2, 64);
                const float rstd = qk_rstd(qa + qb, e.eps);
                float oa[8], ob[8];
                qk_ln_chunk(va, mean, rstd, wA, bA, roped, qs, oa);
                qk_ln_chunk(vb, mean, rstd, wB, bB, roped, qs, ob);
                float ta[8], tb[8];
#pragma unroll
                for (int k = 0; k < 8; ++k) ta[k] = oa[k], tb[k] = ob[k];
                qk_rope_chunk(ta, csA, snA, qs);
                qk_rope_chunk(tb, csB, snB, qs);
#pragma unroll
                for (int k = 0; k < 8; ++k) oa[k] = roped ? ta[k] : oa[k], ob[k] = roped ? tb[k] : ob[k];
                ra = pack8(oa);
                rb = pack8(ob);
              });
              const int r0 = m0 + blk_row(mt) + half * 16;
              static_for<4>([&](auto nt_c) {
                constexpr int nt = decltype(nt_c)::value;
                const int cb = n0 + blk_col(nt);
                if (lrow < p.M - r0 && ch * 8 < p.N - cb) *(uint4*)((char*)(Cb + (int64_t)r0 * ldc + cb) + voff) = raw[nt];
              });
              __builtin_amdgcn_sched_barrier(0);
            });
            return;
          }
        }
        if (perm) plain_loop(IntC<1>{}); else plain_loop(IntC<0>{});
        return;
      }
#pragma unroll
      for (int it = 0; it < NIT; ++it) {
        const int blk = it >> 1, mt = blk / NT, nt = blk % NT;
        const int rr = (it & 1) * 16 + (lane_e >> 2), ch = lane_e & 3;
        const uint4 raw = *(const uint4*)(my + blk * 2048 + rr * 64 + ((ch ^ ((rr >> 2) & 3)) * 16));
        const int row = m0 + blk_row(mt) + rr;
        const int c0 = n0 + blk_col(nt) + ch * 8;
        if (row < p.M && c0 < p.N) {
          uint4 outv = raw;
          if (RES) {
            float x[8], r[8], gq[8];
            const uint32_t u[4] = {raw.x, raw.y, raw.z, raw.w};
            const uint4 rraw = rbuf[it];
            const uint32_t ru[4] = {rraw.x, rraw.y, rraw.z, rraw.w};
#pragma unroll
            for (int k = 0; k < 4; ++k) {
              x[2 * k] = __uint_as_float(u[k] << 16);
              x[2 * k + 1] = __uint_as_float(u[k] & 0xffff0000u);
              r[2 * k] = __uint_as_float(ru[k] << 16);
              r[2 * k + 1] = __uint_as_float(ru[k] & 0xffff0000u);
              gq[2 * k] = gq[2 * k + 1] = 1.0f;
            }
            const bool seg1 = row >= p.seg_split;
            if (gate) {
              if (gate_f32) {
                const float* gp = (const float*)p.gate + (int64_t)b * p.strideGate + (seg1 ? gate_seg : 0) + c0;
                const float4 g0 = *(const float4*)gp, g1 = *(const float4*)(gp + 4);
                gq[0] = g0.x; gq[1] = g0.y; gq[2] = g0.z; gq[3] = g0.w; gq[4] = g1.x; gq[5] = g1.y; gq[6] = g1.z; gq[7] = g1.w;
              } else {
                const uint4 graw = *(const uint4*)(gate + (seg1 ? gate_seg : 0) + c0);
                const uint32_t gu[4] = {graw.x, graw.y, graw.z, graw.w};
#pragma unroll
                for (int k = 0; k < 4; ++k) {
                  gq[2 * k] = __uint_as_float(gu[k] << 16);
                  gq[2 * k + 1] = __uint_as_float(gu[k] & 0xffff0000u);
                }
              }
            }
            float y[8];
#pragma unroll
            for (int k = 0; k < 8; ++k) y[k] = gate_f32 ? r[k] + gq[k] * x[k] : r[k] + rbf(gq[k] * x[k]);
            outv.x = pack_bf2(y[0], y[1]); outv.y = pack_bf2(y[2], y[3]);
            outv.z = pack_bf2(y[4], y[5]); outv.w = pack_bf2(y[6], y[7]);
          }
          bf16_t* crow = Cb + row * ldc;
          if (perm) {
            const int base = col0 + (c0 & ~12), b3 = (c0 >> 3) & 1;
            *(uint2*)(crow + base + (b3 << 2)) = make_uint2(outv.x, outv.y);
            *(uint2*)(crow + base + 8 + (b3 << 2)) = make_uint2(outv.z, outv.w);
          } else {
            *(uint4*)(crow + c0) = outv;
          }
        }
      }
      return;
    }
  }

  auto epilogue_band = [&](auto mt_c) {
    constexpr int mt = decltype(mt_c)::value;
    int row_[NRQ], rowc_[NRQ];
    float brow_[NRQ];
#pragma unroll
    for (int r = 0; r < NRQ; ++r) {
      row_[r] = (PP ? m0 + (mt >> 1) * 128 + wm * 64 + (mt & 1) * 32 : m0 + wm * (MT * 32) + mt * 32) + quad_row(2 * r, lane);
      rowc_[r] = row_[r] < p.M ? row_[r] : p.M - 1;
      brow_[r] = (bias && bias_row) ? bf2f(bias[rowc_[r]]) : 0.0f;
    }
    const float a_sc = FP8 ? p.a_scale[(int64_t)b * p.strideAScale + rowc_[0]] : 1.0f;
    static_for<NT>([&](auto nt_c) {
      constexpr int nt = decltype(nt_c)::value;
      const f32x16 blk = get_acc(mt_c, nt_c);
#pragma unroll
      for (int g = 0; g < 4; ++g) {
        const int row = row_[rq(g)], rowc = rowc_[rq(g)];
        const bool row_ok = row < p.M;
        const float brow = brow_[rq(g)];
        const bool seg1 = row >= p.seg_split;
        const int n = (PP ? n0 + nt * 128 + wn * 32 : n0 + wn * (NT * 32) + nt * 32) + quad_col(g, lane);
        if (n_vec) {
          if (n < p.N) {
            float bv[4] = {0.f, 0.f, 0.f, 0.f}, gv[4] = {1.f, 1.f, 1.f, 1.f}, rv[4] = {0.f, 0.f, 0.f, 0.f};
            if (bias && !bias_row) unpack4(*(const uint2*)(bias + n), bv);
            if (RES && gate) {
              if (gate_f32) {
                const float4 g4 = *(const float4*)((const float*)p.gate + (int64_t)b * p.strideGate + (seg1 ? gate_seg : 0) + n);
                gv[0] = g4.x; gv[1] = g4.y; gv[2] = g4.z; gv[3] = g4.w;
              } else {
                unpack4(*(const uint2*)(gate + (seg1 ? gate_seg : 0) + n), gv);
              }
            }
            if (RES) unpack4(*(const uint2*)(R + rowc * ldr + n), rv);
            float sv[4] = {1.f, 1.f, 1.f, 1.f};
            if (FP8) {
              const float4 s4 = *(const float4*)(p.b_scale + (int64_t)b * p.strideBScale + n);
              sv[0] = s4.x * a_sc; sv[1] = s4.y * a_sc; sv[2] = s4.z * a_sc; sv[3] = s4.w * a_sc;
            }
            float v[4];
#pragma unroll
            for (int i = 0; i < 4; ++i) {
              const float dot = FP8 ? blk[4 * g + i] * sv[i] : blk[4 * g + i];
              float x = rbf(dot + bv[i] + brow);
              if (ACT != ALG_ACT_NONE) x = rbf(act_apply(x, ACT));
              if (RES) x = gate_f32 ? rv[i] + gv[i] * x : rv[i] + rbf(gv[i] * x);
              v[i] = x;
            }
            if (row_ok) {
              const int nc = perm ? col0 + ((n & ~12) | ((n & 4) << 1) | ((n & 8) >> 1)) : n;
              uint2 o;
              o.x = pack_bf2(v[0], v[1]);
              o.y = pack_bf2(v[2], v[3]);
              *(uint2*)(Cb + row * ldc + nc) = o;
            }
          }
        } else {
#pragma unroll
          for (int i = 0; i < 4; ++i) {
            const int nn = n + i;
            if (nn < p.N && row_ok) {
              const float dot = FP8 ? blk[4 * g + i] * (a_sc * p.b_scale[(int64_t)b * p.strideBScale + nn]) : blk[4 * g + i];
              float x = rbf(dot + ((bias && !bias_row) ? bf2f(bias[nn]) : 0.0f) + brow);
              if (ACT != ALG_ACT_NONE) x = rbf(act_apply(x, ACT));
              if (RES) {
                if (gate_f32) {
                  x = bf2f(R[rowc * ldr + nn]) +
                      ((const float*)p.gate)[(int64_t)b * p.strideGate + (seg1 ? gate_seg : 0) + nn] * x;
                } else {
                  const float gg = gate ? bf2f(gate[(seg1 ? gate_seg : 0) + nn]) : 1.0f;
                  x = bf2f(R[rowc * ldr + nn]) + rbf(gg * x);
                }
              }
              const int nj = nn + col0;
              const int nc = perm ? ((nj & ~12) | ((nj & 4) << 1) | ((nj & 8) >> 1)) : nn;
              Cb[row * ldc + nc] = f2bf(x);
            }
          }
        }
      }
    });
  };
#ifndef ALG_EPI_STAGED_ONLY
  static_for<MT>([&](auto mt_c) { epilogue_band(mt_c); });
#endif
  };

  int total_wg = total1;
  if constexpr (PAIR) total_wg += pr.m_tiles * pr.n_tiles * pr.p.batch;
  for (int L = blockIdx.x; L < total_wg; L += gridDim.x) {
    const int xcd = L & 7, q = total_wg >> 3, r = total_wg & 7;
    const int wg = (xcd < r ? xcd * (q + 1) : r * (q + 1) + (xcd - r) * q) + (L >> 3);
    if (L != (int)blockIdx.x) __syncthreads();
    do_tile(wg);
  }
#ifdef ALG_GEMM_TAP
  if (threadIdx.x == 0 && blockIdx.x < 1024) {
    uint64_t* t = gemm_tap_buf + blockIdx.x * 4;
    t[0] = __builtin_readcyclecounter() - tap_c0, t[1] = wall_clock64() - tap_r0, t[2] = tap_loop, t[3] = tap_tiles;
  }
#endif
}

inline unsigned gemm_grid(int64_t nwg) {
  static std::atomic<int> cus{0};
  int n = cus.load();
  if (n == 0) {
    hipDeviceProp_t prop;
    int dev = 0;
    n = (hipGetDevice(&dev) == hipSuccess && hipGetDeviceProperties(&prop, dev) == hipSuccess) ? prop.multiProcessorCount : 256;
    n &= ~7;
    if (n < 8) n = 8;
    cus.store(n);
  }
  return (unsigned)(nwg < n ? nwg : n);
}

inline int gemm_group_m(int pipe, int n_tiles = 0, int K = 0) {
  const int dflt = (pipe != 9 && pipe != 10 && pipe != 11) ? GROUP_M : n_tiles >= 32 ? 4 : (K >= 8192 && n_tiles <= 16) ? 2 : 3;
#ifdef ALG_GROUP_M_OVERRIDE
  return ALG_GROUP_M_OVERRIDE;
#endif
  return dflt;
}

}

using namespace alg;

template <int PIPE, int WNW = 4, bool FP8 = false>
int launch_gemm(const alg_gemm_args* a, int m_tiles, int n_tiles, int64_t nwg, hipStream_t s) {
  constexpr int LDS = (PIPE == 9 || PIPE == 10 || PIPE == 11) ? GEMM_LDS_P9 : GEMM_LDS;
  static PerDeviceOnce attr_set;
  const int dev_slot = current_device_slot();
  if (!device_done(attr_set, dev_slot)) {
    const void* fns[4] = {(const void*)gemm_bf16_kernel<ALG_ACT_NONE, true, PIPE, WNW, FP8>,
                          (const void*)gemm_bf16_kernel<ALG_ACT_GELU_TANH, false, PIPE, WNW, FP8>,
                          (const void*)gemm_bf16_kernel<ALG_ACT_SILU, false, PIPE, WNW, FP8>,
                          (const void*)gemm_bf16_kernel<ALG_ACT_NONE, false, PIPE, WNW, FP8>};
    for (const void* fn : fns) {
      hipError_t e = hipFuncSetAttribute(fn, hipFuncAttributeMaxDynamicSharedMemorySize, LDS);
      if (e != hipSuccess) {
        set_error("alg_gemm_bf16: hipFuncSetAttribute(%d B LDS): %s", LDS, hipGetErrorString(e));
        return ALG_ELAUNCH;
      }
    }
    device_mark(attr_set, dev_slot);
  }
  const dim3 grid(gemm_grid(nwg)), block((PIPE == 11 ? 1 : 2) * WNW * 64);
  const int gm = gemm_group_m(PIPE, n_tiles, a->K);
  if (a->R) {
    hipLaunchKernelGGL((gemm_bf16_kernel<ALG_ACT_NONE, true, PIPE, WNW, FP8>), grid, block, LDS, s, *a, m_tiles,
                       n_tiles, gm, GemmNoPair{});
  } else if (a->act == ALG_ACT_GELU_TANH) {
    hipLaunchKernelGGL((gemm_bf16_kernel<ALG_ACT_GELU_TANH, false, PIPE, WNW, FP8>), grid, block, LDS, s, *a, m_tiles,
                       n_tiles, gm, GemmNoPair{});
  } else if (a->act == ALG_ACT_SILU) {
    hipLaunchKernelGGL((gemm_bf16_kernel<ALG_ACT_SILU, false, PIPE, WNW, FP8>), grid, block, LDS, s, *a, m_tiles,
                       n_tiles, gm, GemmNoPair{});
  } else {
    hipLaunchKernelGGL((gemm_bf16_kernel<ALG_ACT_NONE, false, PIPE, WNW, FP8>), grid, block, LDS, s, *a, m_tiles,
                       n_tiles, gm, GemmNoPair{});
  }
  return check_launch("alg_gemm_bf16");
}
```

alg_amd/csrc/gemm_p10.hip:

```cpp
#include "gemm_kernel.h"

namespace alg {
int launch_gemm_p10(const alg_gemm_args* a, int m_tiles, int n_tiles, int64_t nwg, hipStream_t s) {
  return launch_gemm<10, 2>(a, m_tiles, n_tiles, nwg, s);
}

int launch_gemm_p10_pair(const alg_gemm_args* a, int m_tiles_a, int n_tiles_a, const alg_gemm_args* b, int m_tiles_b, int n_tiles_b,
                        hipStream_t s) {
  const void* fn = (const void*)gemm_bf16_kernel<ALG_ACT_NONE, false, 10, 2, false, false, 1>;
  static PerDeviceOnce attr_set;
  const int dev_slot = current_device_slot();
  if (!device_done(attr_set, dev_slot)) {
    hipError_t e = hipFuncSetAttribute(fn, hipFuncAttributeMaxDynamicSharedMemorySize, GEMM_LDS_P9);
    if (e != hipSuccess) {
      set_error("alg_gemm_bf16_pair: hipFuncSetAttribute(%d B LDS): %s", GEMM_LDS_P9, hipGetErrorString(e));
      return ALG_ELAUNCH;
    }
    device_mark(attr_set, dev_slot);
  }
  const int64_t nwg = (int64_t)m_tiles_a * n_tiles_a * a->batch + (int64_t)m_tiles_b * n_tiles_b * b->batch;
  GemmPairArgs pr;
  pr.p = *b, pr.m_tiles = m_tiles_b, pr.n_tiles = n_tiles_b, pr.group_m = gemm_group_m(10, n_tiles_b, b->K) & 0xffff;
  hipLaunchKernelGGL((gemm_bf16_kernel<ALG_ACT_NONE, false, 10, 2, false, false, 1>), dim3(gemm_grid(nwg)), dim3(256),
                     GEMM_LDS_P9, s, *a, m_tiles_a, n_tiles_a, gemm_group_m(10, n_tiles_a, a->K), pr);
  return check_launch("alg_gemm_bf16_pair");
}

int launch_gemm_p10_pair_qk(const alg_gemm_args* a, int m_tiles_a, int n_tiles_a, const alg_gemm_args* b, int m_tiles_b, int n_tiles_b,
                           const alg_qk_norm_rope_args* e, hipStream_t s) {
  const void* fn = (const void*)gemm_bf16_kernel<ALG_ACT_NONE, false, 10, 2, false, false, 2>;
  static PerDeviceOnce attr_set;
  const int dev_slot = current_device_slot();
  if (!device_done(attr_set, dev_slot)) {
    hipError_t err = hipFuncSetAttribute(fn, hipFuncAttributeMaxDynamicSharedMemorySize, GEMM_LDS_P9);
    if (err != hipSuccess) {
      set_error("alg_gemm_bf16_pair_qk: hipFuncSetAttribute(%d B LDS): %s", GEMM_LDS_P9, hipGetErrorString(err));
      return ALG_ELAUNCH;
    }
    device_mark(attr_set, dev_slot);
  }
  const int64_t nwg = (int64_t)m_tiles_a * n_tiles_a * a->batch + (int64_t)m_tiles_b * n_tiles_b * b->batch;
  GemmPairQkArgs pr;
  pr.p = *b, pr.m_tiles = m_tiles_b, pr.n_tiles = n_tiles_b, pr.group_m = gemm_group_m(10, n_tiles_b, b->K) & 0xffff;
  pr.qe.wq = (const bf16_t*)e->wq, pr.qe.bq = (const bf16_t*)e->bq, pr.qe.wk = (const bf16_t*)e->wk, pr.qe.bk = (const bf16_t*)e->bk;
  pr.qe.cos_tab = e->cos_tab, pr.qe.sin_tab = e->sin_tab, pr.qe.heads = e->heads, pr.qe.text_len = e->text_len;
  pr.qe.eps = e->eps, pr.qe.q_scale = e->q_scale;
  hipLaunchKernelGGL((gemm_bf16_kernel<ALG_ACT_NONE, false, 10, 2, false, false, 2>), dim3(gemm_grid(nwg)), dim3(256),
                     GEMM_LDS_P9, s, *a, m_tiles_a, n_tiles_a, gemm_group_m(10, n_tiles_a, a->K), pr);
  return check_launch("alg_gemm_bf16_pair_qk");
}
}

#ifdef ALG_GEMM_TAP
extern "C" int alg_dbg_gemm_tap(uint64_t* host) { return alg::gemm_tap_read(host); }
#endif
```

alg_amd/csrc/gemm_p11.hip:

```cpp
#include "gemm_kernel.h"

namespace alg {
int launch_gemm_p11(const alg_gemm_args* a, int m_tiles, int n_tiles, int64_t nwg, hipStream_t s) {
  return launch_gemm<11, 4>(a, m_tiles, n_tiles, nwg, s);
}

__global__ __launch_bounds__(256) void pack_b_p11_kernel(const bf16_t* __restrict__ w, uint4* __restrict__ out, int N, int K, int64_t ldb,
                                                          int64_t total) {
  const int64_t i = (int64_t)blockIdx.x * 256 + threadIdx.x;
  if (i >= total) return;
  const int lane = (int)(i & 63);
  const int f = (int)((i >> 6) & 7), wv = (int)((i >> 9) & 3);
  const int64_t tile = i >> 11;
  const int nkt = K / 64;
  const int kt = (int)(tile % nkt);
  const int64_t nt = tile / nkt;
  const int n = (int)(nt * 256) + wv * 64 + (f & 3) * 16 + (lane & 15);
  const int k = kt * 64 + (f >> 2) * 32 + (lane >> 4) * 8;
  uint4 v = make_uint4(0u, 0u, 0u, 0u);
  if (n < N) v = *(const uint4*)(w + (int64_t)n * ldb + k);
  out[i] = v;
}
}

using namespace alg;

extern "C" int64_t alg_pack_b_p11_bytes(int N, int K) {
  if (N <= 0 || K <= 0 || K % 64) return 0;
  return (int64_t)((N + 255) / 256) * (K / 64) * 32768;
}

extern "C" int alg_pack_b_p11(const void* w, void* packed, int N, int K, int64_t ldb, void* stream) {
  if (!w || !packed || N <= 0 || K < 128 || K % 64 || ldb < K || ldb % 8 || ((uintptr_t)w & 15) || ((uintptr_t)packed & 15)) {
    set_error("alg_pack_b_p11: bad argument (N=%d K=%d ldb=%lld; K a multiple of 64 and >= 128, 16-byte aligned rows)", N, K, (long long)ldb);
    return ALG_EINVAL;
  }
  const int64_t total = alg_pack_b_p11_bytes(N, K) / 16;
  hipLaunchKernelGGL(pack_b_p11_kernel, dim3((unsigned)((total + 255) / 256)), dim3(256), 0, (hipStream_t)stream, (const bf16_t*)w,
                     (uint4*)packed, N, K, ldb, total);
  return check_launch("alg_pack_b_p11");
}

#ifdef ALG_GEMM_TAP
extern "C" int alg_dbg_gemm_tap(uint64_t* host) { return alg::gemm_tap_read(host); }
#endif
```

alg_amd/csrc/norm.hip:

```cpp
#include "common.h"
#include "qk_norm_rope.h"

namespace alg {

__device__ __forceinline__ float wave_sum(float v) {
#pragma unroll
  for (int m = 32; m >= 1; m >>= 1) v += __shfl_xor(v, m, 64);
  return v;
}

template <int ITERS>
__global__ __launch_bounds__(256) void ln_mod_kernel(const bf16_t* __restrict__ x, bf16_t* __restrict__ y,
                                                     const bf16_t* __restrict__ w, const bf16_t* __restrict__ bs,
                                                     const bf16_t* __restrict__ scale,
                                                     const bf16_t* __restrict__ shift, int64_t mod_bs,
                                                     int64_t x_bs, int64_t y_bs, int64_t total_rows, int rows,
                                                     int seg_split, int64_t seg_stride, float eps) {
  constexpr int D = ITERS * 512;
  const int lane = threadIdx.x & 63;
  const int64_t row = (int64_t)blockIdx.x * 4 + (threadIdx.x >> 6);
  if (row >= total_rows) return;
  const int bidx = (int)(row / rows);
  const int r = (int)(row - (int64_t)bidx * rows);
  const int seg = r >= seg_split ? 1 : 0;
  const bf16_t* xr = x + (int64_t)bidx * x_bs + (int64_t)r * D;
  float v[ITERS][8];
  float s = 0.0f;
#pragma unroll
  for (int i = 0; i < ITERS; ++i) {
    unpack8(*(const uint4*)(xr + i * 512 + lane * 8), v[i]);
#pragma unroll
    for (int k = 0; k < 8; ++k) s += v[i][k];
  }
  const float mean = wave_sum(s) * (1.0f / D);
  float q = 0.0f;
#pragma unroll
  for (int i = 0; i < ITERS; ++i)
#pragma unroll
    for (int k = 0; k < 8; ++k) {
      const float d = v[i][k] - mean;
      q = fmaf(d, d, q);
    }
  const float rstd = rsqrtf(wave_sum(q) * (1.0f / D) + eps);
  const bf16_t* sc = scale ? scale + (int64_t)bidx * mod_bs + (int64_t)seg * seg_stride : nullptr;
  const bf16_t* sh = shift ? shift + (int64_t)bidx * mod_bs + (int64_t)seg * seg_stride : nullptr;
  bf16_t* yr = y + (int64_t)bidx * y_bs + (int64_t)r * D;
#pragma unroll
  for (int i = 0; i < ITERS; ++i) {
    const int c0 = i * 512 + lane * 8;
    float wv[8], bv[8], o[8];
    if (w) unpack8(*(const uint4*)(w + c0), wv);
    if (bs) unpack8(*(const uint4*)(bs + c0), bv);
#pragma unroll
    for (int k = 0; k < 8; ++k) {
      float n = (v[i][k] - mean) * rstd;
      if (w) n = n * wv[k];
      if (bs) n = n + bv[k];
      o[k] = rbf(n);
    }
    if (sc) {
      float scv[8], shv[8];
      unpack8(*(const uint4*)(sc + c0), scv);
      unpack8(*(const uint4*)(sh + c0), shv);
#pragma unroll
      for (int k = 0; k < 8; ++k) o[k] = rbf(rbf(o[k] * rbf(1.0f + scv[k])) + shv[k]);
    }
    *(uint4*)(yr + c0) = pack8(o);
  }
}

template <int ITERS>
__global__ __launch_bounds__(256) void ln_mod_rows_kernel(const bf16_t* __restrict__ x, bf16_t* __restrict__ y,
                                                          const bf16_t* __restrict__ w, const bf16_t* __restrict__ bs,
                                                          const bf16_t* __restrict__ scale,
                                                          const bf16_t* __restrict__ shift, int64_t mod_bs, int64_t x_bs,
                                                          int64_t y_bs, int64_t total_rows, int rows, int seg_split,
                                                          int64_t seg_stride, float eps, int rpw) {
  constexpr int D = ITERS * 512;
  const int lane = threadIdx.x & 63;
  const int64_t row0 = ((int64_t)blockIdx.x * 4 + (threadIdx.x >> 6)) * rpw;
  if (row0 >= total_rows) return;
  const int64_t row_end = row0 + rpw < total_rows ? row0 + rpw : total_rows;
  uint4 wp[ITERS], bp[ITERS], s1p[ITERS], shp[ITERS];
#pragma unroll
  for (int i = 0; i < ITERS; ++i) {
    wp[i] = *(const uint4*)(w + i * 512 + lane * 8);
    bp[i] = *(const uint4*)(bs + i * 512 + lane * 8);
  }
  auto src = [&](int64_t row) -> const bf16_t* {
    const int bidx = (int)(row / rows);
    return x + (int64_t)bidx * x_bs + (int64_t)(row - (int64_t)bidx * rows) * D + lane * 8;
  };
  uint4 nxt[ITERS];
  {
    const bf16_t* xr = src(row0);
#pragma unroll
    for (int i = 0; i < ITERS; ++i) nxt[i] = *(const uint4*)(xr + i * 512);
  }
  int cur_key = -1;
  for (int64_t row = row0; row < row_end; ++row) {
    float v[ITERS][8];
    float s = 0.0f;
#pragma unroll
    for (int i = 0; i < ITERS; ++i) {
      unpack8(nxt[i], v[i]);
#pragma unroll
      for (int k = 0; k < 8; ++k) s += v[i][k];
    }
    if (row + 1 < row_end) {
      const bf16_t* xr = src(row + 1);
#pragma unroll
      for (int i = 0; i < ITERS; ++i) nxt[i] = *(const uint4*)(xr + i * 512);
    }
    const int bidx = (int)(row / rows);
    const int r = (int)(row - (int64_t)bidx * rows);
    const int key = bidx * 2 + (r >= seg_split ? 1 : 0);
    if (key != cur_key) {
      cur_key = key;
      const int64_t off = (int64_t)bidx * mod_bs + (int64_t)(key & 1) * seg_stride + lane * 8;
#pragma unroll
      for (int i = 0; i < ITERS; ++i) {
        float scv[8];
        unpack8(*(const uint4*)(scale + off + i * 512), scv);
#pragma unroll
        for (int k = 0; k < 8; ++k) scv[k] = 1.0f + scv[k];
        s1p[i] = pack8(scv);
        shp[i] = *(const uint4*)(shift + off + i * 512);
      }
    }
    const float mean = wave_sum(s) * (1.0f / D);
    float q = 0.0f;
#pragma unroll
    for (int i = 0; i < ITERS; ++i)
#pragma unroll
      for (int k = 0; k < 8; ++k) {
        const float d = v[i][k] - mean;
        q = fmaf(d, d, q);
      }
    const float rstd = rsqrtf(wave_sum(q) * (1.0f / D) + eps);
    bf16_t* yr = y + (int64_t)bidx * y_bs + (int64_t)r * D + lane * 8;
#pragma unroll
    for (int i = 0; i < ITERS; ++i) {
      float wv[8], bv[8], s1[8], shv[8], o[8];
      unpack8(wp[i], wv);
      unpack8(bp[i], bv);
      unpack8(s1p[i], s1);
      unpack8(shp[i], shv);
#pragma unroll
      for (int k = 0; k < 8; ++k) {
        float n = (v[i][k] - mean) * rstd;
        n = n * wv[k];
        n = n + bv[k];
        o[k] = rbf(rbf(rbf(n) * s1[k]) + shv[k]);
      }
      *(uint4*)(yr + i * 512) = pack8(o);
    }
  }
}


template <int CTRL, int ROW_MASK>
__device__ __forceinline__ float dpp_max(float v) {
  const int i = __builtin_bit_cast(int, v);
  return fmaxf(v, __builtin_bit_cast(float, __builtin_amdgcn_update_dpp(i, i, CTRL, ROW_MASK, 0xf, false)));
}
__device__ __forceinline__ float wave_max(float v) {
  v = dpp_max<0xB1, 0xf>(v);
  v = dpp_max<0x4E, 0xf>(v);
  v = dpp_max<0x141, 0xf>(v);
  v = dpp_max<0x140, 0xf>(v);
  v = dpp_max<0x142, 0xa>(v);
  v = dpp_max<0x143, 0xc>(v);
  return __builtin_bit_cast(float, __builtin_amdgcn_readlane(__builtin_bit_cast(int, v), 63));
}

template <int ITERS>
__device__ __forceinline__ void quantize_row_store(const float (&v)[ITERS][8], int lane, uint8_t* __restrict__ qr,
                                                   float* __restrict__ scale_out) {
  float amax = 0.0f;
#pragma unroll
  for (int i = 0; i < ITERS; ++i)
#pragma unroll
    for (int k = 0; k < 8; ++k) amax = fmaxf(amax, fabsf(v[i][k]));
  amax = wave_max(amax);
  const float qs = amax > 0.0f ? amax * (1.0f / 448.0f) : 1.0f;
  const float inv = 1.0f / qs;
  if (lane == 0) *scale_out = qs;
#pragma unroll
  for (int i = 0; i < ITERS; ++i) {
    float f[8];
#pragma unroll
    for (int k = 0; k < 8; ++k) f[k] = fminf(fmaxf(v[i][k] * inv, -448.0f), 448.0f);
    int lo = 0, hi = 0;
    lo = __builtin_amdgcn_cvt_pk_fp8_f32(f[0], f[1], lo, false);
    lo = __builtin_amdgcn_cvt_pk_fp8_f32(f[2], f[3], lo, true);
    hi = __builtin_amdgcn_cvt_pk_fp8_f32(f[4], f[5], hi, false);
    hi = __builtin_amdgcn_cvt_pk_fp8_f32(f[6], f[7], hi, true);
    *(uint2*)(qr + i * 512 + lane * 8) = make_uint2((unsigned)lo, (unsigned)hi);
  }
}

template <int ITERS>
__global__ __launch_bounds__(256) void ln_mod_fp8_kernel(const bf16_t* __restrict__ x, uint8_t* __restrict__ q8,
                                                         float* __restrict__ q8_scale, const bf16_t* __restrict__ w,
                                                         const bf16_t* __restrict__ bs, const bf16_t* __restrict__ scale,
                                                         const bf16_t* __restrict__ shift, int64_t mod_bs, int64_t x_bs,
                                                         int64_t total_rows, int rows, int seg_split, int64_t seg_stride,
                                                         float eps) {
  constexpr int D = ITERS * 512;
  const int lane = threadIdx.x & 63;
  const int64_t row = (int64_t)blockIdx.x * 4 + (threadIdx.x >> 6);
  if (row >= total_rows) return;
  const int bidx = (int)(row / rows);
  const int r = (int)(row - (int64_t)bidx * rows);
  const int seg = r >= seg_split ? 1 : 0;
  const bf16_t* xr = x + (int64_t)bidx * x_bs + (int64_t)r * D;
  float v[ITERS][8];
  float s = 0.0f;
#pragma unroll
  for (int i = 0; i < ITERS; ++i) {
    unpack8(*(const uint4*)(xr + i * 512 + lane * 8), v[i]);
#pragma unroll
    for (int k = 0; k < 8; ++k) s += v[i][k];
  }
  const float mean = wave_sum(s) * (1.0f / D);
  float q = 0.0f;
#pragma unroll
  for (int i = 0; i < ITERS; ++i)
#pragma unroll
    for (int k = 0; k < 8; ++k) {
      const float d = v[i][k] - mean;
      q = fmaf(d, d, q);
    }
  const float rstd = rsqrtf(wave_sum(q) * (1.0f / D) + eps);
  const bf16_t* sc = scale ? scale + (int64_t)bidx * mod_bs + (int64_t)seg * seg_stride : nullptr;
  const bf16_t* sh = shift ? shift + (int64_t)bidx * mod_bs + (int64_t)seg * seg_stride : nullptr;
#pragma unroll
  for (int i = 0; i < ITERS; ++i) {
    const int c0 = i * 512 + lane * 8;
    float wv[8], bv[8];
    if (w) unpack8(*(const uint4*)(w + c0), wv);
    if (bs) unpack8(*(const uint4*)(bs + c0), bv);
#pragma unroll
    for (int k = 0; k < 8; ++k) {
      float n = (v[i][k] - mean) * rstd;
      if (w) n = n * wv[k];
      if (bs) n = n + bv[k];
      v[i][k] = rbf(n);
    }
    if (sc) {
      float scv[8], shv[8];
      unpack8(*(const uint4*)(sc + c0), scv);
      unpack8(*(const uint4*)(sh + c0), shv);
#pragma unroll
      for (int k = 0; k < 8; ++k) v[i][k] = rbf(rbf(v[i][k] * rbf(1.0f + scv[k])) + shv[k]);
    }
  }
  quantize_row_store<ITERS>(v, lane, q8 + row * D, q8_scale + row);
}

__global__ __launch_bounds__(256) void qk_norm_rope_kernel(bf16_t* __restrict__ qk, const bf16_t* __restrict__ wq,
                                                           const bf16_t* __restrict__ bq,
                                                           const bf16_t* __restrict__ wk,
                                                           const bf16_t* __restrict__ bk,
                                                           const float* __restrict__ cos_tab,
                                                           const float* __restrict__ sin_tab, int64_t total_vec, int S,
                                                           int heads, int text_len, float eps, float q_scale) {
  const int lane = threadIdx.x & 63;
  const int sub = lane & 7;
  const int64_t vec = ((int64_t)blockIdx.x * 4 + (threadIdx.x >> 6)) * 8 + (lane >> 3);
  const bool live = vec < total_vec;
  const int64_t vv = live ? vec : total_vec - 1;
  const int hv = (int)(vv % (2 * heads));
  const int64_t tok = vv / (2 * heads);
  const int s = (int)(tok % S);
  const bool is_k = hv >= heads;
  bf16_t* ptr = qk + vv * 64 + sub * 8;
  float v[8];
  unpack8(*(const uint4*)ptr, v);
  float sum = qk_chunk_sum(v);
  sum += __shfl_xor(sum, 1, 64);
  sum += __shfl_xor(sum, 2, 64);
  sum += __shfl_xor(sum, 4, 64);
  const float mean = qk_mean(sum);
  float q = qk_chunk_sqdev(v, mean);
  q += __shfl_xor(q, 1, 64);
  q += __shfl_xor(q, 2, 64);
  q += __shfl_xor(q, 4, 64);
  const float rstd = qk_rstd(q, eps);
  float wv[8], bv[8];
  unpack8(*(const uint4*)((is_k ? wk : wq) + sub * 8), wv);
  unpack8(*(const uint4*)((is_k ? bk : bq) + sub * 8), bv);
  float o[8];
  const float qs = is_k ? 1.0f : q_scale;
  const bool roped = s >= text_len && cos_tab;
  qk_ln_chunk(v, mean, rstd, wv, bv, roped, qs, o);
  if (roped) {
    const int64_t pos = (int64_t)(s - text_len) * 64 + sub * 8;
    const float4 c0 = *(const float4*)(cos_tab + pos), c1 = *(const float4*)(cos_tab + pos + 4);
    const float4 s0 = *(const float4*)(sin_tab + pos), s1 = *(const float4*)(sin_tab + pos + 4);
    const float cs[8] = {c0.x, c0.y, c0.z, c0.w, c1.x, c1.y, c1.z, c1.w};
    const float sn[8] = {s0.x, s0.y, s0.z, s0.w, s1.x, s1.y, s1.z, s1.w};
    qk_rope_chunk(o, cs, sn, qs);
  }
  if (live) *(uint4*)ptr = pack8(o);
}

__global__ __launch_bounds__(256) void qk_norm_rope_token_kernel(bf16_t* __restrict__ qk, const bf16_t* __restrict__ wq,
                                                                 const bf16_t* __restrict__ bq, const bf16_t* __restrict__ wk,
                                                                 const bf16_t* __restrict__ bk, const float* __restrict__ cos_tab,
                                                                 const float* __restrict__ sin_tab, int64_t tokens, int S, int heads,
                                                                 int text_len, float eps, float q_scale) {
  const int lane = threadIdx.x & 63;
  const int sub = lane & 7, slot = lane >> 3;
  const int64_t tok = (int64_t)blockIdx.x * 4 + (threadIdx.x >> 6);
  if (tok >= tokens) return;
  const int s = (int)(tok % S);
  const bool roped = s >= text_len && cos_tab;
  float cs[8], sn[8];
  if (roped) {
    const int64_t pos = (int64_t)(s - text_len) * 64 + sub * 8;
    const float4 c0 = *(const float4*)(cos_tab + pos), c1 = *(const float4*)(cos_tab + pos + 4);
    const float4 s0 = *(const float4*)(sin_tab + pos), s1 = *(const float4*)(sin_tab + pos + 4);
    cs[0] = c0.x, cs[1] = c0.y, cs[2] = c0.z, cs[3] = c0.w, cs[4] = c1.x, cs[5] = c1.y, cs[6] = c1.z, cs[7] = c1.w;
    sn[0] = s0.x, sn[1] = s0.y, sn[2] = s0.z, sn[3] = s0.w, sn[4] = s1.x, sn[5] = s1.y, sn[6] = s1.z, sn[7] = s1.w;
  }
  float wqv[8], bqv[8], wkv[8], bkv[8];
  unpack8(*(const uint4*)(wq + sub * 8), wqv);
  unpack8(*(const uint4*)(bq + sub * 8), bqv);
  unpack8(*(const uint4*)(wk + sub * 8), wkv);
  unpack8(*(const uint4*)(bk + sub * 8), bkv);
  bf16_t* const base = qk + tok * (int64_t)(2 * heads) * 64 + sub * 8;
  const int passes = 2 * heads / 8;
  for (int p0 = 0; p0 < passes; p0 += 4) {
    uint4 raw[4];
#pragma unroll
    for (int u = 0; u < 4; ++u) raw[u] = *(const uint4*)(base + (int64_t)((p0 + u) * 8 + slot) * 64);
#pragma unroll
    for (int u = 0; u < 4; ++u) {
      const int hv = (p0 + u) * 8 + slot;
      const bool is_k = hv >= heads;
      float v[8];
      unpack8(raw[u], v);
      float sum = qk_chunk_sum(v);
      sum += __shfl_xor(sum, 1, 64);
      sum += __shfl_xor(sum, 2, 64);
      sum += __shfl_xor(sum, 4, 64);
      const float mean = qk_mean(sum);
      float q = qk_chunk_sqdev(v, mean);
      q += __shfl_xor(q, 1, 64);
      q += __shfl_xor(q, 2, 64);
      q += __shfl_xor(q, 4, 64);
      const float rstd = qk_rstd(q, eps);
      const float qs = is_k ? 1.0f : q_scale;
      float o[8];
      qk_ln_chunk(v, mean, rstd, is_k ? wkv : wqv, is_k ? bkv : bqv, roped, qs, o);
      if (roped) qk_rope_chunk(o, cs, sn, qs);
      *(uint4*)(base + (int64_t)hv * 64) = pack8(o);
    }
  }
}

}

using namespace alg;

extern "C" int alg_layernorm_modulate(const void* x, void* y, const void* weight, const void* bias,
                                      const void* scale, const void* shift, int64_t mod_bstride, int batch, int rows,
                                      int D, int64_t x_bstride, int64_t y_bstride, int seg_split, float eps,
                                      void* stream) {
  return alg_layernorm_modulate_seg(x, y, weight, bias, scale, shift, mod_bstride, D, batch, rows, D, x_bstride, y_bstride,
                                    seg_split, eps, stream);
}

extern "C" int alg_layernorm_modulate_seg(const void* x, void* y, const void* weight, const void* bias,
                                          const void* scale, const void* shift, int64_t mod_bstride,
                                          int64_t seg_stride, int batch, int rows, int D, int64_t x_bstride,
                                          int64_t y_bstride, int seg_split, float eps, void* stream) {
  if (!x || !y || batch <= 0 || rows <= 0 || D <= 0 || seg_stride % 8) {
    set_error("alg_layernorm_modulate: bad argument (batch=%d rows=%d D=%d)", batch, rows, D);
    return ALG_EINVAL;
  }
  if (D % 512 != 0 || D > 8192) {
    set_error("alg_layernorm_modulate: D=%d must be a multiple of 512 and <= 8192", D);
    return ALG_EINVAL;
  }
  if ((scale == nullptr) != (shift == nullptr)) {
    set_error("alg_layernorm_modulate: scale and shift must be given together");
    return ALG_EINVAL;
  }
  if (((uintptr_t)x & 15) || ((uintptr_t)y & 15) || ((uintptr_t)weight & 15) || ((uintptr_t)bias & 15) ||
      ((uintptr_t)scale & 15) || ((uintptr_t)shift & 15) || (mod_bstride % 8) || (x_bstride % 8) ||
      (y_bstride % 8)) {
    set_error("alg_layernorm_modulate: pointers must be 16-byte aligned");
    return ALG_EINVAL;
  }
  const int64_t total = (int64_t)batch * rows;
  const unsigned grid = (unsigned)((total + 3) / 4);
  hipStream_t s = (hipStream_t)stream;
  if (weight && bias && scale && D <= 3072 && total >= 4096) {
    const int64_t resident_waves = (int64_t)device_cus() * 8;
    const int rpw = (int)std::max<int64_t>(8, (total + resident_waves - 1) / resident_waves);
    const unsigned g2 = (unsigned)((total + 4 * (int64_t)rpw - 1) / (4 * (int64_t)rpw));
#define LN_ROWS(I)                                                                                                      \
  case I:                                                                                                               \
    hipLaunchKernelGGL((ln_mod_rows_kernel<I>), dim3(g2), dim3(256), 0, s, (const bf16_t*)x, (bf16_t*)y,                 \
                       (const bf16_t*)weight, (const bf16_t*)bias, (const bf16_t*)scale, (const bf16_t*)shift,          \
                       mod_bstride, x_bstride, y_bstride, total, rows, seg_split, seg_stride, eps, rpw);                \
    break;
    switch (D / 512) { LN_ROWS(1) LN_ROWS(2) LN_ROWS(3) LN_ROWS(4) LN_ROWS(5) LN_ROWS(6) }
#undef LN_ROWS
    return check_launch("alg_layernorm_modulate");
  }
#define LN_CASE(I)                                                                                                  \
  case I:                                                                                                           \
    hipLaunchKernelGGL(ln_mod_kernel<I>, dim3(grid), dim3(256), 0, s, (const bf16_t*)x, (bf16_t*)y,                  \
                       (const bf16_t*)weight, (const bf16_t*)bias, (const bf16_t*)scale, (const bf16_t*)shift,      \
                       mod_bstride, x_bstride, y_bstride, total, rows, seg_split, seg_stride, eps);                                                   \
    break;
  switch (D / 512) {
    LN_CASE(1) LN_CASE(2) LN_CASE(3) LN_CASE(4) LN_CASE(5) LN_CASE(6) LN_CASE(7) LN_CASE(8)
    LN_CASE(9) LN_CASE(10) LN_CASE(11) LN_CASE(12) LN_CASE(13) LN_CASE(14) LN_CASE(15) LN_CASE(16)
  }
#undef LN_CASE
  return check_launch("alg_layernorm_modulate");
}

extern "C" int alg_layernorm_modulate_fp8(const void* x, void* q8, float* q8_scale, const void* weight, const void* bias,
                                          const void* scale, const void* shift, int64_t mod_bstride, int batch, int rows,
                                          int D, int64_t x_bstride, int seg_split, float eps, void* stream) {
  if (!x || !q8 || !q8_scale || batch <= 0 || rows <= 0 || D <= 0) {
    set_error("alg_layernorm_modulate_fp8: bad argument (batch=%d rows=%d D=%d)", batch, rows, D);
    return ALG_EINVAL;
  }
  if (D % 512 != 0 || D > 8192) {
    set_error("alg_layernorm_modulate_fp8: D=%d must be a multiple of 512 and <= 8192", D);
    return ALG_EINVAL;
  }
  if ((scale == nullptr) != (shift == nullptr)) {
    set_error("alg_layernorm_modulate_fp8: scale and shift must be given together");
    return ALG_EINVAL;
  }
  if (((uintptr_t)x & 15) || ((uintptr_t)q8 & 7) || ((uintptr_t)q8_scale & 3) || ((uintptr_t)weight & 15) ||
      ((uintptr_t)bias & 15) || ((uintptr_t)scale & 15) || ((uintptr_t)shift & 15) || (mod_bstride % 8) || (x_bstride % 8)) {
    set_error("alg_layernorm_modulate_fp8: x and the parameter rows must be 16-byte aligned, q8 8-byte aligned");
    return ALG_EINVAL;
  }
  const int64_t total = (int64_t)batch * rows;
  if ((total + 3) / 4 > 0x7fffffff) {
    set_error("alg_layernorm_modulate_fp8: batch * rows = %lld is more than one launch covers", (long long)total);
    return ALG_EINVAL;
  }
  const unsigned grid = (unsigned)((total + 3) / 4);
  const int64_t seg_stride = D;
  hipStream_t s = (hipStream_t)stream;
#define LN_CASE(I)                                                                                                  \
  case I:                                                                                                           \
    hipLaunchKernelGGL(ln_mod_fp8_kernel<I>, dim3(grid), dim3(256), 0, s, (const bf16_t*)x, (uint8_t*)q8, q8_scale,  \
                       (const bf16_t*)weight, (const bf16_t*)bias, (const bf16_t*)scale, (const bf16_t*)shift,      \
                       mod_bstride, x_bstride, total, rows, seg_split, seg_stride, eps);                            \
// ... 45 lines not shown
```

alg_amd/transformer_cogvideox.py:

```python
from __future__ import annotations

import math
import os
from dataclasses import dataclass, asdict
from typing import Optional

import torch

from . import _lib


@dataclass
class CogVideoXTransformerConfig:

    num_attention_heads: int = 48
    attention_head_dim: int = 64
    in_channels: int = 32
    out_channels: int = 16
    num_layers: int = 42
    time_embed_dim: int = 512
    text_embed_dim: int = 4096
    max_text_seq_length: int = 226
    sample_width: int = 90
    sample_height: int = 60
    sample_frames: int = 49
    patch_size: int = 2
    patch_size_t: Optional[int] = None
    temporal_compression_ratio: int = 4
    ff_inner_mult: int = 4
    norm_eps: float = 1e-5
    qk_norm_eps: float = 1e-6
    flip_sin_to_cos: bool = True
    freq_shift: int = 0
    use_rotary_positional_embeddings: bool = True
    use_learned_positional_embeddings: bool = True
    ofs_embed_dim: Optional[int] = None
    spatial_interpolation_scale: float = 1.875
    temporal_interpolation_scale: float = 1.0

    @property
    def inner_dim(self):
        return self.num_attention_heads * self.attention_head_dim

    def to_dict(self):
        return asdict(self)


def _bf(t, device):
    return t.to(device=device, dtype=torch.bfloat16).contiguous()


class CogVideoXTransformer3DModel:
    dtype = torch.bfloat16

    FP8_WEIGHTS = ("wqk", "wv", "wo", "wf1", "wf2")

    def __init__(self, config: CogVideoXTransformerConfig, weights: dict, device="cuda", fp8=False):
        cfg = self.config = config
        self.device = torch.device(device)
        if self.device.type != "cuda":
            raise _lib.AlgHipError("CogVideoXTransformer3DModel runs on the GPU only (HIP kernels, no CPU fallback)")
        if cfg.attention_head_dim != 64:
            raise _lib.AlgHipError("the attention kernel is specialised for head_dim 64")
        if cfg.ofs_embed_dim is not None and cfg.ofs_embed_dim != cfg.time_embed_dim:
            raise _lib.AlgHipError("ofs_embed_dim must equal time_embed_dim (emb = emb + ofs_emb)")
        D = cfg.inner_dim
        if D % 512:
            raise _lib.AlgHipError("inner_dim must be a multiple of 512 (LayerNorm kernel tiling)")
        self.fp8 = bool(fp8)
        if self.fp8:
            self._check_fp8_shapes()
        self.fuse_quant = True
        _lib.load_library()
        self.attn_prescale = True
        self.pair_qkv = True
        self.fuse_qk_norm = False
        self.packed_weights = True
        self._sincos = {}
        dev = self.device
        w = weights
        p = cfg.patch_size
        self.p_t = cfg.patch_size_t or 1
        self.k_patch = cfg.in_channels * p * p * self.p_t
        if self.k_patch % 64 or cfg.text_embed_dim % 64 or cfg.time_embed_dim % 64:
            raise _lib.AlgHipError("GEMM K dimensions must be multiples of 64")
        self.w_patch = _bf(w["patch_embed.proj.weight"].reshape(D, self.k_patch), dev)
        self.b_patch = _bf(w["patch_embed.proj.bias"], dev)
        self.w_text = _bf(w["patch_embed.text_proj.weight"], dev)
        self.b_text = _bf(w["patch_embed.text_proj.bias"], dev)
        self.pos_emb = _bf(w["patch_embed.pos_embedding"][0], dev) if cfg.use_learned_positional_embeddings else None
        self.w_t1 = _bf(w["time_embedding.linear_1.weight"], dev)
        self.b_t1 = _bf(w["time_embedding.linear_1.bias"], dev)
        self.w_t2 = _bf(w["time_embedding.linear_2.weight"], dev)
        self.b_t2 = _bf(w["time_embedding.linear_2.bias"], dev)
        if cfg.ofs_embed_dim is not None:
            self.w_o1, self.b_o1 = _bf(w["ofs_embedding.linear_1.weight"], dev), _bf(w["ofs_embedding.linear_1.bias"], dev)
            self.w_o2, self.b_o2 = _bf(w["ofs_embedding.linear_2.weight"], dev), _bf(w["ofs_embedding.linear_2.bias"], dev)

        def reorder6(t):
            c = t.chunk(6, dim=0)
            return torch.cat([c[3], c[0], c[4], c[1], c[5], c[2]], dim=0)

        mw, mb = [], []
        self.layers = []
        for i in range(cfg.num_layers):
            b = "transformer_blocks.%d." % i
            L = {}
            for nm in ("norm1", "norm2"):
                mw.append(reorder6(w[b + nm + ".linear.weight"]))
                mb.append(reorder6(w[b + nm + ".linear.bias"]))
                L[nm + "_w"] = _bf(w[b + nm + ".norm.weight"], dev)
                L[nm + "_b"] = _bf(w[b + nm + ".norm.bias"], dev)
            L["wqk"] = _bf(torch.cat([w[b + "attn1.to_q.weight"], w[b + "attn1.to_k.weight"]], dim=0), dev)
            L["bqk"] = _bf(torch.cat([w[b + "attn1.to_q.bias"], w[b + "attn1.to_k.bias"]], dim=0), dev)
            L["wv"] = _bf(w[b + "attn1.to_v.weight"], dev)
            L["bv"] = _bf(w[b + "attn1.to_v.bias"], dev)
            for nm in ("norm_q", "norm_k"):
                L[nm + "_w"] = _bf(w[b + "attn1." + nm + ".weight"], dev)
                L[nm + "_b"] = _bf(w[b + "attn1." + nm + ".bias"], dev)
            L["wo"] = _bf(w[b + "attn1.to_out.0.weight"], dev)
            L["bo"] = _bf(w[b + "attn1.to_out.0.bias"], dev)
            L["wf1"] = _bf(w[b + "ff.net.0.proj.weight"], dev)
            L["bf1"] = _bf(w[b + "ff.net.0.proj.bias"], dev)
            L["wf2"] = _bf(w[b + "ff.net.2.weight"], dev)
            L["bf2"] = _bf(w[b + "ff.net.2.bias"], dev)
            if self.fp8:
                self._quantize_layer(L, drop_bf16=True)
            else:
                for nm in ("wo", "wf1", "wf2"):
                    L["p" + nm] = _lib.PackedB(L[nm])
            self.layers.append(L)
        ow, ob = w["norm_out.linear.weight"], w["norm_out.linear.bias"]
        sh_w, sc_w = ow.chunk(2, dim=0)
        sh_b, sc_b = ob.chunk(2, dim=0)
        mw.append(torch.cat([sh_w, sh_w, sc_w, sc_w], dim=0))
        mb.append(torch.cat([sh_b, sh_b, sc_b, sc_b], dim=0))
        self.w_mod = _bf(torch.cat(mw, dim=0), dev)
        self.b_mod = _bf(torch.cat(mb, dim=0), dev)
        self.mod_cols = self.w_mod.shape[0]
        self.norm_final_w = _bf(w["norm_final.weight"], dev)
        self.norm_final_b = _bf(w["norm_final.bias"], dev)
        self.norm_out_w = _bf(w["norm_out.norm.weight"], dev)
        self.norm_out_b = _bf(w["norm_out.norm.bias"], dev)
        self.w_out = _bf(w["proj_out.weight"], dev)
        self.b_out = _bf(w["proj_out.bias"], dev)
        self._ws = {}
        self._rope_cache = {}
        self.profile = None

    def _check_fp8_shapes(self):
        cfg = self.config
        D, F4 = cfg.inner_dim, cfg.ff_inner_mult * cfg.inner_dim
        if D % 128 or F4 % 128:
            raise ValueError("fp8=True: the e4m3 GEMM needs K %% 128 == 0, this config has inner_dim = %d and a feed-forward "
                             "width of %d" % (D, F4))

    @staticmethod
    def _quantize_layer(L, drop_bf16):
        for nm in CogVideoXTransformer3DModel.FP8_WEIGHTS:
            wt = L[nm]
            q = torch.empty(wt.shape, dtype=torch.uint8, device=wt.device)
            sc = torch.empty(wt.shape[0], dtype=torch.float32, device=wt.device)
            _lib.quantize_fp8_rows(wt, q, sc, wt.shape[0], wt.shape[1])
            L[nm + "8"] = (q, sc)
            if drop_bf16:
                del L[nm]

    def _positional(self, Hh, Ww, Fr, S):
        cfg = self.config
        learned = cfg.use_learned_positional_embeddings
        if not learned and cfg.use_rotary_positional_embeddings:
            return None
        pre_frames = (Fr - 1) * cfg.temporal_compression_ratio + 1
        if learned and pre_frames == cfg.sample_frames and self.pos_emb is not None and self.pos_emb.shape[0] == S:
            return self.pos_emb
        p = cfg.patch_size
        gh, gw, gt = Hh // p, Ww // p, Fr // self.p_t
        key = (gh, gw, gt)
        hit = self._sincos.get(key)
        if hit is None:
            D = cfg.inner_dim
            ds, dt = 3 * D // 4, D // 4

            def sc1(dim, pos):
                omega = 1.0 / 10000 ** (torch.arange(dim // 2, dtype=torch.float64) / (dim / 2.0))
                out = torch.outer(pos.reshape(-1).double(), omega)
                return torch.cat([out.sin(), out.cos()], dim=1)

            hh = torch.arange(gh, dtype=torch.float32) / cfg.spatial_interpolation_scale
            ww = torch.arange(gw, dtype=torch.float32) / cfg.spatial_interpolation_scale
            tt = torch.arange(gt, dtype=torch.float32) / cfg.temporal_interpolation_scale
            grid = torch.stack(torch.meshgrid(ww, hh, indexing="xy"), dim=0).reshape(2, 1, gh, gw)
            sp = torch.cat([sc1(ds // 2, grid[0]), sc1(ds // 2, grid[1])], dim=1)
            tp = sc1(dt, tt)
            pe = torch.cat([tp[:, None].expand(-1, gh * gw, -1), sp[None].expand(gt, -1, -1)], dim=-1).reshape(gt * gh * gw, D)
            joint = torch.zeros(cfg.max_text_seq_length + pe.shape[0], D, dtype=torch.float32)
            joint[cfg.max_text_seq_length:] = pe.float()
            hit = joint.to(device=self.device, dtype=torch.bfloat16).contiguous()
            self._sincos[key] = hit
        if hit.shape[0] != S:
            raise ValueError("positional embedding covers %d tokens, the sequence has %d" % (hit.shape[0], S))
        return hit

    def _timed(self, name, fn, *args, **kwargs):
        if self.profile is None:
            return fn(*args, **kwargs)
        e0, e1 = torch.cuda.Event(enable_timing=True), torch.cuda.Event(enable_timing=True)
        e0.record()
        out = fn(*args, **kwargs)
        e1.record()
        self.profile.setdefault(name, []).append((e0, e1))
        return out

    @classmethod
    def from_synthetic(cls, config=None, seed=1234, std=0.02, device="cuda", randomize_affine=False, fp8=False):
        from .weights import synthetic_state_dict

        config = config or CogVideoXTransformerConfig()
        return cls(config, synthetic_state_dict(config, seed=seed, std=std, device=device,
                                                 randomize_affine=randomize_affine), device=device, fp8=fp8)

    @classmethod
    def from_pretrained(cls, path, subfolder="transformer", torch_dtype=torch.bfloat16, device="cuda", fp8=False, **_):
        from .weights import load_diffusers_transformer

        config, sd = load_diffusers_transformer(path, subfolder)
        return cls(config, sd, device=device, fp8=fp8)

    def to(self, *args, **kwargs):
        return self

    def _workspace(self, N, S, P):
        key = (N, S, P)
        ws = self._ws.get(key)
        if ws is not None:
            return ws
        cfg, dev = self.config, self.device
        D = cfg.inner_dim
        bf = dict(device=dev, dtype=torch.bfloat16)
        S_pad = (S + 127) // 128 * 128
        ws = dict(
            S_pad=S_pad,
            x=torch.empty(N, S, D, **bf),
            y=torch.empty(N, S, D, **bf),
            qk=torch.empty(N, S, 2 * D, **bf),
            vt=torch.zeros(N, D, S_pad, **bf),
            att=torch.empty(N, S, D, **bf),
            h=torch.empty(N, S, cfg.ff_inner_mult * D, **bf),
            patches=torch.empty(N, P, self.k_patch, **bf),
            tsin=torch.empty(N, D, **bf),
            t1=torch.empty(N, cfg.time_embed_dim, **bf),
            semb=torch.empty(N, cfg.time_embed_dim, **bf),
            mod=torch.empty(N, self.mod_cols, **bf),
            po=torch.empty(N * P, self.w_out.shape[0], **bf),
        )
        if len(self._ws) >= 4:
            self._ws.pop(next(iter(self._ws)))
        self._ws[key] = ws
        return ws

    def _fp8_state(self, ws, N, S):
        if "q8" not in ws:
            F4 = self.config.ff_inner_mult * self.config.inner_dim
            ws["q8"] = torch.empty(N * S, F4, dtype=torch.uint8, device=self.device)
            ws["q8s"] = torch.empty(N * ((S + 3) // 4 * 4), dtype=torch.float32, device=self.device)
        if self.layers and "wqk8" not in self.layers[0]:
            self._check_fp8_shapes()
            for L in self.layers:
                self._quantize_layer(L, drop_bf16=False)
        return ws["q8"], ws["q8s"]

    def _block_fp8(self, L, ws, q8, q8s, N, S, T, m1, m2, cos, sin, scale, q_scale, prescale):
        cfg, G, TM = self.config, _lib.gemm, self._timed
        D, Hn = cfg.inner_dim, cfg.num_attention_heads
        F4 = cfg.ff_inner_mult * D
        x, y, qk, vt, att, h, mod, S_pad = ws["x"], ws["y"], ws["qk"], ws["vt"], ws["att"], ws["h"], ws["mod"], ws["S_pad"]
        SS = (S + 3) // 4 * 4
        items = ((0, N),) if SS == S else tuple((n, 1) for n in range(N))

        def quant(src, K_):
            for n0, nb in items:
                TM("quant", _lib.quantize_fp8_rows, src, q8, q8s, nb * S, K_, x_off=n0 * S * K_, q_off=n0 * S * K_,
                   scale_off=n0 * SS)

        def ln_mod(nw, nb, m):
            if not self.fuse_quant:
                TM("ln_mod", _lib.layernorm_modulate, x, y, nw, nb, mod, mod, self.mod_cols, N, S, D, T, cfg.norm_eps,
                   scale_off=m + 2 * D, shift_off=m)
                return quant(y, D)
            for n0, n_ in items:
                TM("ln_mod", _lib.layernorm_modulate_fp8, x, q8, q8s, nw, nb, mod, mod, self.mod_cols, n_, S, D, T, cfg.norm_eps,
                   x_off=n0 * S * D, scale_off=n0 * self.mod_cols + m + 2 * D, shift_off=n0 * self.mod_cols + m,
                   q8_off=n0 * S * D, q8_scale_off=n0 * SS)

        def lin(name, wt, C, N_, K_, ldc, **kw):
            TM(name, G, q8, wt[0], C, S, N_, K_, K_, K_, ldc, a_scale=q8s, b_scale=wt[1], batch=N, strideA=S * K_,
               strideAScale=SS, strideC=S * ldc, **kw)

        ln_mod(L["norm1_w"], L["norm1_b"], m1)
        lin("gemm_qk", L["wqk8"], qk, 2 * D, D, 2 * D, bias=L["bqk"])
        TM("gemm_vt", G, L["wv8"][0], q8, vt, D, S, D, D, D, S_pad, a_scale=L["wv8"][1], b_scale=q8s, strideBScale=SS,
           bias=L["bv"], batch=N, strideB=S * D, strideC=D * S_pad, flags=_lib.GEMM_BIAS_PER_ROW | _lib.GEMM_PERMUTE_COLS)
        TM("qk_norm_rope", _lib.qk_norm_rope_, qk, L["norm_q_w"], L["norm_q_b"], L["norm_k_w"], L["norm_k_b"], cos, sin, N, S, Hn, T,
           cfg.qk_norm_eps, q_scale=q_scale)
        TM("attn", _lib.flash_attn_d64, qk, qk, vt, att, N, Hn, S, S * 2 * D, 2 * D, D * S_pad, S_pad, S * D, D, scale,
           k_off=D, q_prescaled=prescale)
        quant(att, D)
        lin("gemm_out", L["wo8"], x, D, D, D, bias=L["bo"], R=x, ldr=D, gate=mod, gate_off=m1 + 4 * D,
            strideGate=self.mod_cols, seg_split=T, strideR=S * D)
        ln_mod(L["norm2_w"], L["norm2_b"], m2)
        lin("gemm_ff1", L["wf18"], h, F4, D, F4, bias=L["bf1"], act=_lib.ACT_GELU_TANH)
        quant(h, F4)
        lin("gemm_ff2", L["wf28"], x, D, F4, D, bias=L["bf2"], R=x, ldr=D, gate=mod, gate_off=m2 + 4 * D,
            strideGate=self.mod_cols, seg_split=T, strideR=S * D)

    def _rope(self, image_rotary_emb):
        if image_rotary_emb is None:
            return None, None
        cos, sin = image_rotary_emb
        key = (cos.data_ptr(), sin.data_ptr(), tuple(cos.shape))
        hit = self._rope_cache.get(key)
        if hit is None:
            hit = (cos.to(device=self.device, dtype=torch.float32).contiguous(),
                   sin.to(device=self.device, dtype=torch.float32).contiguous())
            self._rope_cache = {key: hit}
        return hit

    def forward_assembled(self, latents, conds, encoder_hidden_states, timestep, image_rotary_emb=None, ofs=None):
        cfg = self.config
        N = len(conds)
        lat = latents.to(device=self.device, dtype=torch.bfloat16).contiguous()
        Bl, Fr, C, Hh, Ww = lat.shape
        if Bl not in (1, N):
            raise ValueError("latents batch must be 1 or len(conds)")
        if 2 * C != cfg.in_channels:
            raise ValueError("latents have %d channels, transformer expects in_channels=%d" % (C, cfg.in_channels))
        conds = [c.to(device=self.device, dtype=torch.bfloat16).contiguous() for c in conds]
        for c in conds:
            if c.numel() != Fr * C * Hh * Ww:
                raise ValueError("conditioning latents must have shape [1, F, C, H, W] matching the latents")
        ehs = encoder_hidden_states.to(device=self.device, dtype=torch.bfloat16).contiguous()
        if ehs.shape[0] != N:
            raise ValueError("encoder_hidden_states batch %d != %d samples" % (ehs.shape[0], N))
        T = ehs.shape[1]
        p, p_t = cfg.patch_size, self.p_t
        if Fr % p_t:
            raise ValueError("latent frames (%d) must be a multiple of patch_size_t=%d (cog:963-968 pads them)" % (Fr, p_t))
        P = (Fr // p_t) * (Hh // p) * (Ww // p)
        S = T + P
        D, Hn = cfg.inner_dim, cfg.num_attention_heads
        if cfg.use_learned_positional_embeddings:
            if cfg.sample_width != Ww or cfg.sample_height != Hh:
                raise ValueError(
                    "It is currently not possible to generate videos at a different resolution that the defaults. "
                    "This should only be the case with 'THUDM/CogVideoX-5b-I2V'.")
        pos_emb = self._positional(Hh, Ww, Fr, S)
        ws = self._workspace(N, S, P)
        x, y, qk, vt, att, h, mod = ws["x"], ws["y"], ws["qk"], ws["vt"], ws["att"], ws["h"], ws["mod"]
        fp8 = bool(self.fp8)
        if fp8:
            q8, q8s = self._fp8_state(ws, N, S)
        elif self.layers and "wqk" not in self.layers[0]:
            raise _lib.AlgHipError("this model was built with fp8=True and holds no bf16 copy of its block weights: build it "
                                   "with fp8=False to run (or switch between) both modes")
        S_pad = ws["S_pad"]
        cos, sin = self._rope(image_rotary_emb)
        G = _lib.gemm
        TM = self._timed

        ts = timestep.to(device=self.device, dtype=torch.float32).contiguous()
        if ts.numel() != N:
            ts = ts.reshape(-1)[:1].expand(N).contiguous()
        _lib.timestep_embedding(ts, ws["tsin"], N, D, cfg.flip_sin_to_cos)
        E = cfg.time_embed_dim
        G(ws["tsin"], self.w_t1, ws["t1"], N, E, D, D, D, E, bias=self.b_t1, act=_lib.ACT_SILU)
        if cfg.ofs_embed_dim is None:
            G(ws["t1"], self.w_t2, ws["semb"], N, E, E, E, E, E, bias=self.b_t2, act=_lib.ACT_SILU)
        else:
            if ofs is None:
                raise ValueError("this transformer has an ofs embedding: pass `ofs` (cog:998)")
            O = cfg.ofs_embed_dim
            emb, osin, o1, oemb = (torch.empty(N, E, device=self.device, dtype=torch.bfloat16) for _ in range(4))
            G(ws["t1"], self.w_t2, emb, N, E, E, E, E, E, bias=self.b_t2)
            ofs_v = ofs.to(device=self.device, dtype=torch.float32).reshape(-1)
            ofs_v = (ofs_v if ofs_v.numel() == N else ofs_v[:1].expand(N)).contiguous()
            _lib.timestep_embedding(ofs_v, osin, N, O, cfg.flip_sin_to_cos)
            G(osin, self.w_o1, o1, N, O, O, O, O, O, bias=self.b_o1, act=_lib.ACT_SILU)
            G(o1, self.w_o2, oemb, N, O, O, O, O, O, bias=self.b_o2)
            _lib.lincomb([(1.0, emb), (1.0, oemb)], torch.bfloat16, out=emb)
            _lib.silu(emb, ws["semb"])
        G(ws["semb"], self.w_mod, mod, N, self.mod_cols, E, E, E, self.mod_cols, bias=self.b_mod)

        G(ehs, self.w_text, x, T, D, cfg.text_embed_dim, cfg.text_embed_dim, cfg.text_embed_dim, D,
          bias=self.b_text, R=pos_emb, ldr=D, batch=N, strideA=T * cfg.text_embed_dim, strideC=S * D)
        _lib.patchify(lat, 0 if Bl == 1 else Fr * C * Hh * Ww, conds, ws["patches"], N, Fr, C, Hh, Ww, p, p_t)
        G(ws["patches"], self.w_patch, x, P, D, self.k_patch, self.k_patch, self.k_patch, D, bias=self.b_patch,
          R=pos_emb, ldr=D, r_off=T * D, batch=N, strideA=P * self.k_patch, strideC=S * D, c_off=T * D)

        scale = 1.0 / math.sqrt(cfg.attention_head_dim)
        prescale = self.attn_prescale
        q_scale = scale * 1.4426950408889634 if prescale else 1.0
        F4 = cfg.ff_inner_mult * D
        packed = self.packed_weights and os.environ.get("ALG_GEMM_PIPE", "10") == "10"
        wo_k, wf1_k, wf2_k = ("pwo", "pwf1", "pwf2") if packed else ("wo", "wf1", "wf2")
        for li, L in enumerate(self.layers):
            m1 = li * 12 * D
            m2 = m1 + 6 * D
            if fp8:
                self._block_fp8(L, ws, q8, q8s, N, S, T, m1, m2, cos, sin, scale, q_scale, prescale)
                continue
            TM("ln_mod", _lib.layernorm_modulate, x, y, L["norm1_w"], L["norm1_b"], mod, mod, self.mod_cols, N, S, D,
               T, cfg.norm_eps, scale_off=m1 + 2 * D, shift_off=m1)
            qk_call = ((y, L["wqk"], qk, S, 2 * D, D, D, D, 2 * D), dict(bias=L["bqk"], batch=N, strideA=S * D, strideC=S * 2 * D))
            vt_call = ((L["wv"], y, vt, D, S, D, D, D, S_pad), dict(bias=L["bv"], batch=N, strideB=S * D, strideC=D * S_pad,
                                                                   flags=_lib.GEMM_BIAS_PER_ROW | _lib.GEMM_PERMUTE_COLS))
            if self.pair_qkv and self.fuse_qk_norm:
                TM("gemm_qkv", _lib.gemm_pair_qk, qk_call, vt_call, L["norm_q_w"], L["norm_q_b"], L["norm_k_w"], L["norm_k_b"], cos, sin,
                               Hn, T, cfg.qk_norm_eps, q_scale=q_scale)
            else:
                if self.pair_qkv:
                    TM("gemm_qkv", _lib.gemm_pair, qk_call, vt_call)
                else:
                    TM("gemm_qk", G, *qk_call[0], **qk_call[1])
                    TM("gemm_vt", G, *vt_call[0], **vt_call[1])
                TM("qk_norm_rope", _lib.qk_norm_rope_, qk, L["norm_q_w"], L["norm_q_b"], L["norm_k_w"], L["norm_k_b"], cos, sin, N, S, Hn, T,
                                   cfg.qk_norm_eps, q_scale=q_scale)
            TM("attn", _lib.flash_attn_d64, qk, qk, vt, att, N, Hn, S, S * 2 * D, 2 * D, D * S_pad, S_pad, S * D, D, scale,
                                k_off=D, q_prescaled=prescale)
            TM("gemm_out", G, att, L[wo_k], x, S, D, D, D, D, D, bias=L["bo"], R=x, ldr=D, gate=mod, gate_off=m1 + 4 * D,
              strideGate=self.mod_cols, seg_split=T, batch=N, strideA=S * D, strideC=S * D, strideR=S * D)
            TM("ln_mod", _lib.layernorm_modulate, x, y, L["norm2_w"], L["norm2_b"], mod, mod, self.mod_cols, N, S, D,
               T, cfg.norm_eps, scale_off=m2 + 2 * D, shift_off=m2)
            TM("gemm_ff1", G, y, L[wf1_k], h, S, F4, D, D, D, F4, bias=L["bf1"], act=_lib.ACT_GELU_TANH, batch=N, strideA=S * D,
              strideC=S * F4)
            TM("gemm_ff2", G, h, L[wf2_k], x, S, D, F4, F4, F4, D, bias=L["bf2"], R=x, ldr=D, gate=mod, gate_off=m2 + 4 * D,
              strideGate=self.mod_cols, seg_split=T, batch=N, strideA=S * F4, strideC=S * D, strideR=S * D)

        _lib.layernorm_modulate(x, y, self.norm_final_w, self.norm_final_b, None, None, 0, N, S, D, T, cfg.norm_eps)
        mo = cfg.num_layers * 12 * D
        _lib.layernorm_modulate(y, att, self.norm_out_w, self.norm_out_b, mod, mod, self.mod_cols, N, P, D, 0,
                                cfg.norm_eps, x_bstride=S * D, y_bstride=P * D, x_off=T * D, scale_off=mo + 2 * D,
                                shift_off=mo)
        n_out = self.w_out.shape[0]
        G(att, self.w_out, ws["po"], N * P, n_out, D, D, D, n_out, bias=self.b_out)
        out = torch.empty(N, Fr, cfg.out_channels, Hh, Ww, device=self.device, dtype=torch.bfloat16)
        _lib.unpatchify(ws["po"], out, N, Fr, cfg.out_channels, Hh, Ww, p, p_t)
        return out

    def __call__(self, hidden_states, encoder_hidden_states, timestep, timestep_cond=None, ofs=None,
                 image_rotary_emb=None, attention_kwargs=None, return_dict=True):
        if timestep_cond is not None:
            raise NotImplementedError("timestep_cond is not used by the CogVideoX I2V checkpoints")
        C = hidden_states.shape[2] // 2
        lat = hidden_states[:, :, :C].contiguous()
        conds = [hidden_states[n:n + 1, :, C:].contiguous() for n in range(hidden_states.shape[0])]
        out = self.forward_assembled(lat, conds, encoder_hidden_states, timestep, image_rotary_emb, ofs=ofs)
        if not return_dict:
            return (out,)
        return TransformerOutput(sample=out)


@dataclass
class TransformerOutput:
    sample: torch.Tensor
```

include/alg_hip.h:

```cpp
#ifndef ALG_HIP_H
#define ALG_HIP_H

#include <stdint.h>

#ifdef __cplusplus
extern "C" {
#endif

#define ALG_F32 0
#define ALG_BF16 1

#define ALG_OK 0
#define ALG_EINVAL (-1)
#define ALG_ELAUNCH (-2)
#define ALG_ELIMIT (-3)

#define ALG_VERSION 110

int alg_version(void);
const char* alg_last_error(void);

void alg_reload_env(void);


int alg_down_up(const void* in, void* out, int64_t planes, int H, int W, int h1, int w1, int dtype,
                int round_intermediate, const void* tables, void* workspace, int64_t workspace_bytes, void* stream);

int64_t alg_lowpass_tables_bytes(int H, int W, int h1, int w1);
int alg_lowpass_tables_build(void* tables, int64_t bytes, int H, int W, int h1, int w1, void* stream);

int64_t alg_down_up_workspace_bytes(int64_t planes, int H, int W, int h1, int w1);

int alg_gaussian_blur(const void* in, void* out, int64_t planes, int H, int W, int ksize, float sigma, int dtype,
                      void* workspace, int64_t workspace_bytes, void* stream);
int64_t alg_gaussian_blur_workspace_bytes(int64_t planes, int H, int W, int ksize);

int alg_cfg_ddim_step(const void* pred, int pred_dtype, void* latents, int lat_dtype, int n_pass, int64_t numel,
                      float guidance_scale, float sqrt_alpha_t, float sqrt_beta_t, float coef_a, float coef_b,
                      void* stream);

int alg_cfg_combine(const void* pred, void* out, int dtype, int n_pass, int64_t numel, float guidance_scale,
                    void* stream);

int alg_lincomb(const void* const* xs, const float* coefs, const int* dtypes, int n_terms, void* out, int out_dtype,
                int64_t numel, void* stream);

int alg_concat_cast(const void* const* src0, int dtype0, const void* const* src1, int dtype1, int n, int64_t O,
                    int64_t A0, int64_t A1, int64_t R, int64_t s0_ostride, int64_t s1_ostride, int64_t a1_off,
                    void* out, int out_dtype, void* stream);

int alg_unipc_update(const float* x, const float* m0, const float* m1, const float* m_new, float* out,
                     int64_t numel, float r, float c, float k, float rk, float rho0, float rho_new, void* stream);


#define ALG_ACT_NONE 0
#define ALG_ACT_GELU_TANH 1
#define ALG_ACT_SILU 2

#define ALG_GEMM_BIAS_PER_ROW 1
#define ALG_GEMM_PERMUTE_COLS 4
#define ALG_GEMM_GATE_SEG_STRIDE 16
#define ALG_GEMM_B_PACKED11 32
#define ALG_GEMM_GATE_F32 8

typedef struct alg_gemm_args {
  const void* A;
  const void* B;
  void* C;
  const void* bias;
  const void* R;
  const void* gate;
  int64_t lda, ldb, ldc, ldr;
  int64_t strideA, strideB, strideC, strideR, strideGate;
  int32_t M, N, K, batch;
  int32_t seg_split;
  int32_t act;
  int32_t flags;
  int64_t gate_seg_stride;
  int32_t perm_col0;
  int32_t conv_cin_log2;
  const float* a_scale;
  const float* b_scale;
  int64_t strideAScale, strideBScale;
  int32_t conv_wp;
  int32_t conv_hpwp;
  int32_t conv_kw;
  int32_t reserved1;
} alg_gemm_args;

int alg_gemm_bf16(const alg_gemm_args* args, void* stream);

int64_t alg_pack_b_p11_bytes(int N, int K);
int alg_pack_b_p11(const void* w, void* packed, int N, int K, int64_t ldb, void* stream);

int alg_gemm_bf16_pair(const alg_gemm_args* a, const alg_gemm_args* b, void* stream);

typedef struct alg_qk_norm_rope_args {
  const void *wq, *bq, *wk, *bk;
  const float *cos_tab, *sin_tab;
  int32_t heads, text_len;
  float eps, q_scale;
} alg_qk_norm_rope_args;
int alg_gemm_bf16_pair_qk(const alg_gemm_args* qk, const alg_gemm_args* vt, const alg_qk_norm_rope_args* e, void* stream);

int alg_gemm_fp8(const alg_gemm_args* args, void* stream);

int alg_quantize_fp8_rows(const void* x, int64_t x_rstride, void* q, float* scale, int64_t rows, int K, void* stream);

int alg_flash_attn_d64(const void* q, const void* k, const void* vt, void* o, int batch, int heads, int S,
                       int64_t q_bstride, int64_t q_rstride, int64_t vt_bstride, int64_t vt_rstride,
                       int64_t o_bstride, int64_t o_rstride, float scale, void* stream);

#define ALG_ATTN_Q_PRESCALED 1
int alg_flash_attn_d64_ex(const void* q, const void* k, const void* vt, void* o, int batch, int heads, int S,
                          int64_t q_bstride, int64_t q_rstride, int64_t vt_bstride, int64_t vt_rstride,
                          int64_t o_bstride, int64_t o_rstride, float scale, int flags, void* workspace,
                          int64_t workspace_bytes, void* stream);
int64_t alg_flash_attn_d64_workspace_bytes(int batch, int heads, int S, int flags);

int alg_flash_attn_d128(const void* q, const void* k, const void* vt, void* o, int batch, int heads, int Sq, int Skv,
                        int64_t q_bstride, int64_t q_rstride, int64_t k_bstride, int64_t k_rstride, int64_t vt_bstride,
                        int64_t vt_rstride, int64_t o_bstride, int64_t o_rstride, float scale, void* stream);

int alg_flash_attn_d128_ex(const void* q, const void* k, const void* vt, void* o, int batch, int heads, int Sq, int Skv,
                           int64_t q_bstride, int64_t q_rstride, int64_t k_bstride, int64_t k_rstride, int64_t vt_bstride,
                           int64_t vt_rstride, int64_t o_bstride, int64_t o_rstride, float scale, int kv_group, int causal,
                           void* stream);

int alg_flash_attn_d128_fp8(const void* q, const float* q_scale, const void* k, const float* k_scale, const void* vt,
                            const float* vt_scale, void* o, int batch, int heads, int Sq, int Skv, int64_t q_bstride,
                            int64_t q_rstride, int64_t k_bstride, int64_t k_rstride, int64_t vt_bstride, int64_t vt_rstride,
                            int64_t o_bstride, int64_t o_rstride, float scale, int kv_group, int causal, void* stream);

int alg_quantize_fp8_khead(const void* x, int64_t x_bstride, int64_t x_rstride, void* q, int64_t q_bstride, int64_t q_rstride,
                           float* scale, int batch, int heads, int S, int scale_given, void* stream);

int alg_rmsnorm_rope_fp8(const void* x, const void* weight, const float* cos_tab, const float* sin_tab, int64_t x_rstride,
                         int batch, int rows, int D, float eps, void* q8, int64_t q8_rstride, float* scale,
                         const float* head_scale, void* stream);
int alg_headnorm_rope_fp8(const void* x, const void* weight, const float* cos_tab, const float* sin_tab, int64_t x_rstride,
                          int64_t x_bstride, int batch, int rows, int heads, int rope_tokens, float eps, void* q8,
                          int64_t q8_rstride, int64_t q8_bstride, float* scale, int64_t scale_bstride, const float* head_scale,
                          void* stream);

int alg_quantize_fp8_vt(const void* x, int64_t x_bstride, int64_t x_rstride, void* q, int64_t q_bstride, int64_t q_rstride,
                        float* scale, int batch, int rows, int Skv, int src_permuted, void* stream);

int alg_flash_attn_d128_dual(const void* q, const void* k, const void* vt, int Skv, int64_t k_bstride, int64_t k_rstride,
                             int64_t vt_bstride, int64_t vt_rstride, const void* k2, const void* vt2, int Skv2, int64_t k2_bstride,
                             int64_t k2_rstride, int64_t vt2_bstride, int64_t vt2_rstride, void* o, int batch, int heads, int Sq,
                             int64_t q_bstride, int64_t q_rstride, int64_t o_bstride, int64_t o_rstride, float scale, void* stream);

int alg_rope_half(void* x, const float* cos_tab, const float* sin_tab, const int* pos, int64_t rows, int heads,
                  int64_t x_rstride, void* stream);


int alg_embed_rows(const int64_t* ids, const void* table, void* out, int64_t n, int D, int vocab, void* stream);

int alg_t5_layernorm(const void* x, const void* weight, void* y, int64_t rows, int D, float eps, void* stream);

int alg_attn_bias(const void* q, const void* k, const void* v, void* out, const void* bias_table, const int* rel_bucket,
                  const int* key_mask, int batch, int heads, int head_dim, int L, int64_t qkv_rstride, int64_t out_rstride,
                  float scale, int causal, void* stream);

int alg_quick_gelu(void* x, int64_t numel, void* stream);

int alg_mul_bf16(const void* a, const void* b, void* out, int64_t numel, void* stream);


#define ALG_CONV_PLAIN 0
#define ALG_CONV_PAIR 1
#define ALG_CONV_STRIDE2 2
int alg_conv_cl_bf16(const void* x, const void* w, const void* bias, const void* res, void* y, int frames, int Hp,
                     int Wp, int Cin, int Cout, int kt, int mode, void* stream);

typedef struct alg_vae_geom {
  int32_t frames, H, W, C;
  int32_t first_len, seg_len;
  int32_t lat_first_single;
  int32_t lat_rate, lat_scale;
  int32_t lat_h, lat_w;
} alg_vae_geom;

int64_t alg_vae_groupnorm_workspace(const alg_vae_geom* g);
int alg_vae_groupnorm_stats(const void* x, const alg_vae_geom* g, float eps, void* workspace, float* stats, void* stream);

int alg_vae_spatial_norm(const void* x, const float* stats, const void* gamma, const void* beta, const void* zyb,
                         void* out, const alg_vae_geom* g, int silu, void* stream);

int alg_vae_group_norm(const void* x, const float* stats, const void* gamma, const void* beta, void* out,
                       const alg_vae_geom* g, int silu, void* stream);

int alg_vae_pad(const void* x, void* out, int frames, int H, int W, int C, void* stream);

int alg_vae_repitch(const void* x, void* out, int frames, int H, int W, int C, int src_rows, int src_wp, void* stream);

int alg_vae_unpack_planes(const void* x, void* out, int frames, int H, int W, int C, void* stream);

int alg_vae_upsample(const void* x, void* out, int frames_out, int H, int W, int C, int compress_time, int first_single,
                     void* stream);

int alg_vae_pack_latent(const void* z, int64_t c_stride, int64_t frame_stride, void* out, int frames, int h, int w,
                        int channels, float scale, void* stream);

int alg_vae_unpack_video(const void* x, void* out, int frames, int H, int W, int to_uint8, void* stream);


int alg_headnorm_rope(void* x, const void* weight, const float* cos_tab, const float* sin_tab, int64_t x_rstride,
                      int64_t x_bstride, int batch, int rows, int heads, int rope_tokens, float eps, void* stream);

int alg_masked_mean(const void* x, const int* valid, void* out, int batch, int L, int D, void* stream);

int alg_silu(const void* x, void* y, int64_t numel, void* stream);


int alg_layernorm_mod_f32(const void* x, void* y, const float* weight, const float* bias, const float* scale,
                          const float* shift, int64_t mod_bstride, int batch, int rows, int D, float eps, void* stream);

int alg_layernorm_mod_f32_fp8(const void* x, void* q8, float* q8_scale, const float* weight, const float* bias,
                              const float* scale, const float* shift, int64_t mod_bstride, int batch, int rows, int D,
                              float eps, void* stream);

int alg_rmsnorm_rope(void* x, const void* weight, const float* cos_tab, const float* sin_tab, int64_t x_rstride,
                     int batch, int rows, int D, float eps, void* stream);

int alg_wan_modulation(const float* table, const void* vec, float* out, int layers, int batch, int J, int D,
                       int vec_per_j, void* stream);

int alg_patchify3d(const void* in, void* out, int n, int C, int F, int H, int W, int ph, int pw, int Kpad, void* stream);

int alg_unpatchify3d(const void* in, int64_t ldin, void* out, int n, int C, int F, int H, int W, int ph, int pw,
                     int channel_major, void* stream);

int alg_timestep_embedding_f32(const float* t, float* out, int n, int dim, void* stream);

int alg_linear_f32(const float* x, const float* W, const float* b, float* y, void* y_bf16, void* y_silu_bf16, int M,
                   int N, int K, int act, void* stream);

int alg_gelu_erf(void* x, int64_t numel, void* stream);

int alg_layernorm_modulate(const void* x, void* y, const void* weight, const void* bias, const void* scale,
                           const void* shift, int64_t mod_bstride, int batch, int rows, int D, int64_t x_bstride,
                           int64_t y_bstride, int seg_split, float eps, void* stream);
int alg_layernorm_modulate_seg(const void* x, void* y, const void* weight, const void* bias, const void* scale,
                               const void* shift, int64_t mod_bstride, int64_t seg_stride, int batch, int rows, int D,
                               int64_t x_bstride, int64_t y_bstride, int seg_split, float eps, void* stream);

int alg_layernorm_modulate_fp8(const void* x, void* q8, float* q8_scale, const void* weight, const void* bias,
                               const void* scale, const void* shift, int64_t mod_bstride, int batch, int rows, int D,
                               int64_t x_bstride, int seg_split, float eps, void* stream);

int alg_qk_norm_rope(void* qk, const void* wq, const void* bq, const void* wk, const void* bk, const float* cos_tab,
                     const float* sin_tab, int batch, int S, int heads, int text_len, float eps, void* stream);

int alg_qk_norm_rope_scaled(void* qk, const void* wq, const void* bq, const void* wk, const void* bk, const float* cos_tab,
                            const float* sin_tab, int batch, int S, int heads, int text_len, float eps, float q_scale,
                            void* stream);

int alg_patchify(const void* latents, int64_t lat_bstride, const void* const* cond_ptrs, void* out, int n_samples,
                 int frames, int C, int H, int W, int p, void* stream);

int alg_unpatchify(const void* in, void* out, int n_samples, int frames, int C, int H, int W, int p, void* stream);

int alg_patchify_t(const void* latents, int64_t lat_bstride, const void* const* cond_ptrs, void* out, int n_samples,
                   int frames, int C, int H, int W, int p, int p_t, void* stream);
int alg_unpatchify_t(const void* in, void* out, int n_samples, int frames, int C, int H, int W, int p, int p_t,
                     void* stream);

int alg_timestep_embedding(const float* t, void* out, int n, int dim, int flip_sin_to_cos, void* stream);


int alg_rms_norm_rows(const void* x, const void* gamma, void* y, int64_t rows, int C, int Cp, int silu, void* stream);

int alg_softmax_hilo(const void* neg_hi, const void* lo, void* p, int64_t rows, int cols, int64_t ld, float scale, void* stream);


int alg_calib_mfma_bf16(float* sink, int iters, unsigned seed, int blocks, uint64_t* clocks, void* stream);

int alg_wall_clock_khz(void);

void alg_attn_clock_tap(uint64_t* buffer, int slots);

#ifdef __cplusplus
}
#endif
#endif
```

Measured before the change: 1.531 frames/s.

## Fuse LayerNorm-modulate into residual GEMM epilogue via per-row-tile arrival counters

Adds a GEMM variant for the residual out-projection and FF2 GEMMs that counts finished column tiles per row block with atomic counters. The last workgroup to finish a row block runs the LayerNorm plus modulation for those rows. This removes the standalone layernorm_modulate launches and their extra read of the hidden state after gemm_out, and after ff2 for the next layer's norm1. In exchange it adds atomic and fence synchronisation and puts serial LayerNorm work on the last-arriving workgroups, which may cause tail imbalance. The standalone LN kernel is refactored onto a shared row helper.

After: 1.293 frames/s. 15.5% lower.

```diff
diff --git a/alg_amd/_lib.py b/alg_amd/_lib.py
--- a/alg_amd/_lib.py
+++ b/alg_amd/_lib.py
@@ -16,7 +16,7 @@
 GEMM_B_PACKED11 = 32
 
 EXPORTS = (
-    "alg_version", "alg_last_error", "alg_reload_env", "alg_down_up", "alg_gaussian_blur", "alg_cfg_ddim_step", "alg_gemm_bf16", "alg_gemm_bf16_pair", "alg_gemm_bf16_pair_qk", "alg_pack_b_p11", "alg_pack_b_p11_bytes",
+    "alg_version", "alg_last_error", "alg_reload_env", "alg_down_up", "alg_gaussian_blur", "alg_cfg_ddim_step", "alg_gemm_bf16", "alg_gemm_bf16_pair", "alg_gemm_bf16_pair_qk", "alg_gemm_bf16_ln_mod", "alg_gemm_ln_mod_counters_bytes", "alg_gemm_ln_mod_tiles", "alg_pack_b_p11", "alg_pack_b_p11_bytes",
     "alg_flash_attn_d64", "alg_layernorm_modulate", "alg_layernorm_modulate_fp8", "alg_qk_norm_rope", "alg_patchify", "alg_unpatchify",
     "alg_timestep_embedding", "alg_cfg_combine", "alg_lincomb", "alg_unipc_update", "alg_concat_cast", "alg_flash_attn_d128", "alg_layernorm_mod_f32", "alg_layernorm_mod_f32_fp8", "alg_rmsnorm_rope",
     "alg_wan_modulation", "alg_patchify3d", "alg_unpatchify3d", "alg_timestep_embedding_f32", "alg_linear_f32",
@@ -29,7 +29,8 @@
     "alg_flash_attn_d128_fp8", "alg_quantize_fp8_khead", "alg_quantize_fp8_vt", "alg_rmsnorm_rope_fp8", "alg_headnorm_rope_fp8",
 )
 _RET_I64 = ("alg_vae_groupnorm_workspace", "alg_lowpass_tables_bytes", "alg_down_up_workspace_bytes",
-            "alg_gaussian_blur_workspace_bytes", "alg_flash_attn_d64_workspace_bytes", "alg_pack_b_p11_bytes")
+            "alg_gaussian_blur_workspace_bytes", "alg_flash_attn_d64_workspace_bytes", "alg_pack_b_p11_bytes",
+            "alg_gemm_ln_mod_counters_bytes", "alg_gemm_ln_mod_tiles")
 
 
 class AlgHipError(RuntimeError):
@@ -54,6 +55,12 @@
     _fields_ = [("wq", c_void_p), ("bq", c_void_p), ("wk", c_void_p), ("bk", c_void_p), ("cos_tab", c_void_p),
                 ("sin_tab", c_void_p), ("heads", c_int32), ("text_len", c_int32), ("eps", c_float),
                 ("q_scale", c_float)]
+
+
+class LnModArgs(Structure):
+    _fields_ = [("y", c_void_p), ("weight", c_void_p), ("bias", c_void_p), ("scale", c_void_p), ("shift", c_void_p),
+                ("mod_bstride", c_int64), ("seg_stride", c_int64), ("y_bstride", c_int64), ("seg_split", c_int32),
+                ("eps", c_float), ("counters", c_void_p)]
 
 
 class VaeGeom(Structure):
@@ -101,6 +108,8 @@
     lib.alg_flash_attn_d64_workspace_bytes.argtypes = [c_int] * 4
     lib.alg_pack_b_p11_bytes.argtypes = [c_int, c_int]
     lib.alg_pack_b_p11_bytes.restype = c_int64
+    lib.alg_gemm_ln_mod_counters_bytes.argtypes = [c_int, c_int]
+    lib.alg_gemm_ln_mod_tiles.argtypes = [c_int] * 5 + [c_void_p]
     lib.alg_pack_b_p11.argtypes = [c_void_p, c_void_p, c_int, c_int, c_int64, c_void_p]
     lib.alg_cfg_ddim_step.argtypes = [c_void_p, c_int, c_void_p, c_int, c_int, c_int64, c_float, c_float, c_float,
                                       c_float, c_float, c_void_p]
@@ -246,6 +255,7 @@
 def clear_caches():
     _TABLES.clear()
     _SCRATCH.clear()
+    _COUNTERS.clear()
 
 
 def lowpass_tables(x, h1, w1):
@@ -805,6 +815,50 @@
     _check(lib.alg_gemm_bf16_pair_qk(ctypes.byref(a), ctypes.byref(b), ctypes.byref(e), _stream()), "alg_gemm_bf16_pair_qk")
 
 
+_COUNTERS = {}
+
+
+def ln_mod_counters(ref, nbytes):
+    key = _stream_key(ref)
+    t = _COUNTERS.get(key)
+    cap = _capturing()
+    if t is None or t.numel() * 4 < nbytes:
+        t = torch.zeros((int(nbytes) + 3) // 4, dtype=torch.int32, device=ref.device)
+        if cap:
+            return _pin(t)
+        _COUNTERS[key] = t
+    return _pin(t) if cap else t
+
+
+def gemm_ln_mod(call, y, weight, bias, scale, shift, mod_bstride, seg_split, eps, seg_stride=None, y_bstride=None, y_off=0,
+                scale_off=0, shift_off=0, counters=True):
+    lib = load_library()
+    g, fp8 = gemm_args(*call[0], **call[1])
+    if fp8:
+        raise AlgHipError("gemm_ln_mod takes a bf16 problem")
+    n = LnModArgs()
+    n.y = y.data_ptr() + 2 * y_off
+    n.weight = weight.data_ptr() if weight is not None else None
+    n.bias = bias.data_ptr() if bias is not None else None
+    n.scale = (scale.data_ptr() + 2 * scale_off) if scale is not None else None
+    n.shift = (shift.data_ptr() + 2 * shift_off) if shift is not None else None
+    n.mod_bstride, n.seg_stride = mod_bstride, g.N if seg_stride is None else seg_stride
+    n.y_bstride = g.M * g.N if y_bstride is None else y_bstride
+    n.seg_split, n.eps = seg_split, float(eps)
+    cnt = ln_mod_counters(y, int(lib.alg_gemm_ln_mod_counters_bytes(g.M, g.batch))) if counters else None
+    n.counters = cnt.data_ptr() if cnt is not None else None
+    _check(lib.alg_gemm_bf16_ln_mod(ctypes.byref(g), ctypes.byref(n), _stream()), "alg_gemm_bf16_ln_mod")
+
+
+def gemm_ln_mod_tiles(M, N, K, batch, schedule):
+    lib = load_library()
+    n = int(lib.alg_gemm_ln_mod_tiles(M, N, K, batch, schedule, None))
+    buf = (c_int32 * (3 * n))()
+    if n and int(lib.alg_gemm_ln_mod_tiles(M, N, K, batch, schedule, buf)) != n:
+        raise AlgHipError("alg_gemm_ln_mod_tiles failed")
+    return [tuple(buf[3 * i:3 * i + 3]) for i in range(n)]
+
+
 def quantize_fp8_rows(x, q, scale, rows, K, x_rstride=None, x_off=0, q_off=0, scale_off=0):
     x_rstride = K if x_rstride is None else x_rstride
     _check(load_library().alg_quantize_fp8_rows(_p(x, x_off), x_rstride, _p(q, q_off), _p(scale, scale_off), rows, K,
diff --git a/alg_amd/csrc/gemm.hip b/alg_amd/csrc/gemm.hip
--- a/alg_amd/csrc/gemm.hip
+++ b/alg_amd/csrc/gemm.hip
@@ -16,6 +16,10 @@
 int launch_gemm_p10_pair_qk(const alg_gemm_args* a, int m_tiles_a, int n_tiles_a, const alg_gemm_args* b, int m_tiles_b, int n_tiles_b,
                             const alg_qk_norm_rope_args* e, hipStream_t s);
 int launch_gemm_p11(const alg_gemm_args* a, int m_tiles, int n_tiles, int64_t nwg, hipStream_t s);
+int launch_gemm_p10_ln_mod(const alg_gemm_args* a, const alg_ln_mod_args* n, int m_tiles, int n_tiles, int64_t nwg, hipStream_t s);
+int launch_gemm_p11_ln_mod(const alg_gemm_args* a, const alg_ln_mod_args* n, int m_tiles, int n_tiles, int64_t nwg, hipStream_t s);
+int gemm_group_m_of(int pipe, int n_tiles, int K);
+void gemm_tile_at(int L, int total, int m_tiles, int n_tiles, int group_m, int32_t* out3);
 int launch_gemm_p6_fp8(const alg_gemm_args* a, int m_tiles, int n_tiles, int64_t nwg, hipStream_t s);
 int launch_gemm_p9_fp8(const alg_gemm_args* a, int m_tiles, int n_tiles, int64_t nwg, hipStream_t s);
 int launch_gemm_p6_conv(const alg_gemm_args* a, int m_tiles, int n_tiles, int64_t nwg, hipStream_t s);
@@ -210,6 +214,50 @@
   if (rc != ALG_OK) return rc;
   return alg_qk_norm_rope_scaled(a->C, e->wq, e->bq, e->wk, e->bk, e->cos_tab, e->sin_tab, a->batch, a->M, e->heads, e->text_len,
                                  e->eps, e->q_scale, stream);
+}
+
+extern "C" int alg_gemm_bf16_ln_mod(const alg_gemm_args* g, const alg_ln_mod_args* n, void* stream) {
+  int rc = gemm_entry(g, stream, false, true);
+  if (rc != ALG_OK) return rc;
+  if (!n) return gemm_entry(g, stream, false);
+  if (!n->y || g->ldc != g->N || n->seg_stride % 8 || g->N % 512 != 0 || g->N > 8192 || (n->scale == nullptr) != (n->shift == nullptr) ||
+      ((uintptr_t)g->C & 15) || ((uintptr_t)n->y & 15) || ((uintptr_t)n->weight & 15) || ((uintptr_t)n->bias & 15) ||
+      ((uintptr_t)n->scale & 15) || ((uintptr_t)n->shift & 15) || (n->mod_bstride % 8) || (g->strideC % 8) || (n->y_bstride % 8) ||
+      ((uintptr_t)n->counters & 3)) {
+    set_error("alg_gemm_bf16_ln_mod: bad LayerNorm arguments (N = ldc = %d a multiple of 512 and <= 8192, 16-byte aligned pointers and "
+              "strides, scale and shift together)", g->N);
+    return ALG_EINVAL;
+  }
+  const bool packed = (g->flags & ALG_GEMM_B_PACKED11) != 0;
+  const bool sched_ok = packed || (gemm_pipe() == 10 && g->K >= 128 && 256 * g->lda * 2 + (int64_t)g->K * 2 < (1ll << 32) &&
+                                   256 * g->ldb * 2 + (int64_t)g->K * 2 < (1ll << 32));
+  const int m_tiles = (g->M + BM - 1) / BM, n_tiles = (g->N + BN - 1) / BN;
+  const int64_t nwg = (int64_t)m_tiles * n_tiles * g->batch;
+  const bool fused = sched_ok && !g->conv_wp && g->R && g->act == ALG_ACT_NONE && g->N % BN == 0 && g->N <= 3072 &&
+                     (int64_t)g->M * g->ldc < (1ll << 31) && (int64_t)g->M * g->ldr < (1ll << 31) && nwg <= 0x7fffffff &&
+                     n->weight && n->bias && n->scale && n->counters;
+  if (fused) return (packed ? launch_gemm_p11_ln_mod : launch_gemm_p10_ln_mod)(g, n, m_tiles, n_tiles, nwg, (hipStream_t)stream);
+  rc = gemm_entry(g, stream, false);
+  if (rc != ALG_OK) return rc;
+  return alg_layernorm_modulate_seg(g->C, n->y, n->weight, n->bias, n->scale, n->shift, n->mod_bstride, n->seg_stride, g->batch, g->M,
+                                    g->N, g->strideC, n->y_bstride, n->seg_split, n->eps, stream);
+}
+
+extern "C" int64_t alg_gemm_ln_mod_counters_bytes(int M, int batch) {
+  if (M <= 0 || batch <= 0) return 0;
+  return 4ll * batch * ((M + BM - 1) / BM);
+}
+
+extern "C" int64_t alg_gemm_ln_mod_tiles(int M, int N, int K, int batch, int schedule, int32_t* out) {
+  if (M <= 0 || N <= 0 || K <= 0 || batch <= 0 || (schedule != 10 && schedule != 11)) return 0;
+  const int m_tiles = (M + BM - 1) / BM, n_tiles = (N + BN - 1) / BN;
+  const int64_t total = (int64_t)m_tiles * n_tiles * batch;
+  if (total > 0x7fffffff) return 0;
+  if (out) {
+    const int gm = gemm_group_m_of(schedule, n_tiles, K);
+    for (int L = 0; L < (int)total; ++L) gemm_tile_at(L, (int)total, m_tiles, n_tiles, gm, out + 3 * (int64_t)L);
+  }
+  return total;
 }
 
 extern "C" int alg_gemm_fp8(const alg_gemm_args* a, void* stream) { return gemm_entry(a, stream, true); }
diff --git a/alg_amd/csrc/gemm_kernel.h b/alg_amd/csrc/gemm_kernel.h
--- a/alg_amd/csrc/gemm_kernel.h
+++ b/alg_amd/csrc/gemm_kernel.h
@@ -4,6 +4,7 @@
 #include <type_traits>
 
 #include "common.h"
+#include "ln_mod.h"
 #include "qk_norm_rope.h"
 #ifdef ALG_P9_LOOP_INC
 #include ALG_P9_LOOP_INC
@@ -111,18 +112,65 @@
 struct GemmPairQkArgs : GemmPairArgs {
   QkNormRope qe;
 };
+struct GemmPostNormArgs {
+  LnModRows ln;
+  uint32_t* counters;
+  int iters;
+};
+#ifndef ALG_POSTNORM_PF
+#define ALG_POSTNORM_PF 2
+#endif
+constexpr int GEMM_POSTNORM_PF = ALG_POSTNORM_PF;
+
+__device__ __forceinline__ int64_t uniform_i64(int64_t v) {
+  const uint32_t lo = __builtin_amdgcn_readfirstlane((uint32_t)v), hi = __builtin_amdgcn_readfirstlane((uint32_t)((uint64_t)v >> 32));
+  return (int64_t)(((uint64_t)hi << 32) | lo);
+}
+template <typename T>
+__device__ __forceinline__ T* uniform_ptr(T* p) { return (T*)(uintptr_t)uniform_i64((int64_t)(uintptr_t)p); }
+template <int ITERS>
+static __device__ __attribute__((noinline)) void postnorm_wave_rows(const LnModRows v, const int64_t g0, const int64_t g1) {
+  LnModRows a;
+  a.x = uniform_ptr(v.x), a.y = uniform_ptr(v.y), a.w = uniform_ptr(v.w), a.bs = uniform_ptr(v.bs);
+  a.scale = uniform_ptr(v.scale), a.shift = uniform_ptr(v.shift);
+  a.mod_bs = uniform_i64(v.mod_bs), a.x_bs = uniform_i64(v.x_bs), a.y_bs = uniform_i64(v.y_bs), a.seg_stride = uniform_i64(v.seg_stride);
+  a.rows = __builtin_amdgcn_readfirstlane(v.rows), a.seg_split = __builtin_amdgcn_readfirstlane(v.seg_split);
+  a.eps = __uint_as_float(__builtin_amdgcn_readfirstlane(__float_as_uint(v.eps)));
+  ln_mod_wave_rows<ITERS, GEMM_POSTNORM_PF>(a, uniform_i64(g0), uniform_i64(g1), (int)(threadIdx.x & 63));
+}
+
+__host__ __device__ inline int gemm_tile_of_logical(int L, int total_wg) {
+  const int xcd = L & 7, q = total_wg >> 3, r = total_wg & 7;
+  return (xcd < r ? xcd * (q + 1) : r * (q + 1) + (xcd - r) * q) + (L >> 3);
+}
+__host__ __device__ inline void gemm_tile_coords(int wg, int m_tiles, int n_tiles, int group_m, int* b, int* mt, int* nt) {
+  const int tiles = m_tiles * n_tiles;
+  *b = wg / tiles;
+  int t = wg - *b * tiles;
+  const int grp = t / (group_m * n_tiles);
+  const int first_m = grp * group_m;
+  const int gsize = m_tiles - first_m < group_m ? m_tiles - first_m : group_m;
+  t -= grp * group_m * n_tiles;
+  *mt = first_m + t % gsize;
+  *nt = t / gsize;
+}
+
 template <int PAIR> struct GemmPairT { typedef GemmNoPair type; };
 template <> struct GemmPairT<1> { typedef GemmPairArgs type; };
 template <> struct GemmPairT<2> { typedef GemmPairQkArgs type; };
-template <int ACT, bool RES, int PIPE, int WNW = 4, bool FP8 = false, bool CONV = false, int PAIR = 0>
+template <int PAIR, int POSTNORM> struct GemmExtraT { typedef typename GemmPairT<PAIR>::type type; };
+template <> struct GemmExtraT<0, 1> { typedef GemmPostNormArgs type; };
+template <int ACT, bool RES, int PIPE, int WNW = 4, bool FP8 = false, bool CONV = false, int PAIR = 0, int POSTNORM = 0>
 __global__ __launch_bounds__((PIPE == 11 ? 1 : 2) * WNW * 64) void gemm_bf16_kernel(
-    const alg_gemm_args p1, int m_tiles1, int n_tiles1, int group_m1, const typename GemmPairT<PAIR>::type pr) {
+    const alg_gemm_args p1, int m_tiles1, int n_tiles1, int group_m1, const typename GemmExtraT<PAIR, POSTNORM>::type pr) {
   constexpr bool P9 = PIPE == 9 || PIPE == 10 || PIPE == 11;
   constexpr bool M16 = PIPE == 10 || PIPE == 11;
   constexpr bool P11 = PIPE == 11;
   constexpr int WMW = P11 ? 1 : 2;
   constexpr int MT = BM / WMW / 32;
   static_assert(!PAIR || (P9 && !P11 && !RES && ACT == ALG_ACT_NONE), "the pair launch is built for the plain schedule-9 / 10 kernels");
+  static_assert(!POSTNORM || (POSTNORM == 1 && !PAIR && RES && ACT == ALG_ACT_NONE && (PIPE == 10 || PIPE == 11) && !FP8 && !CONV),
+                "the LayerNorm fix-up is built for the residual form of schedules 10 / 11 (4 waves)");
   static_assert(!FP8 || PIPE == 6 || PIPE == 9, "the fp8 operands are built on the ping-pong schedule and on schedule 9");
   static_assert(!CONV || (PIPE == 6 && !FP8), "the convolution addressing is built on the bf16 ping-pong schedule");
   typedef typename std::conditional<FP8, uint8_t, bf16_t>::type elem_t;
@@ -1307,6 +1355,36 @@
     const int wg = (xcd < r ? xcd * (q + 1) : r * (q + 1) + (xcd - r) * q) + (L >> 3);
     if (L != (int)blockIdx.x) __syncthreads();
     do_tile(wg);
+    if constexpr (POSTNORM) {
+      int pb, pmt, pnt;
+      gemm_tile_coords(wg, m_tiles1, n_tiles1, group_m1, &pb, &pmt, &pnt);
+      __builtin_amdgcn_fence(__ATOMIC_RELEASE, "agent");
+      __syncthreads();
+      uint32_t* const slot = (uint32_t*)smem;
+      if (tid == 0) {
+        uint32_t* const c = pr.counters + pb * m_tiles1 + pmt;
+        __builtin_amdgcn_fence(__ATOMIC_RELEASE, "agent");
+        const uint32_t old = __hip_atomic_fetch_add(c, 1u, __ATOMIC_RELAXED, __HIP_MEMORY_SCOPE_AGENT);
+        if (old == (uint32_t)(n_tiles1 - 1)) __hip_atomic_store(c, 0u, __ATOMIC_RELAXED, __HIP_MEMORY_SCOPE_AGENT);
+        *slot = old;
+      }
+      __syncthreads();
+      const uint32_t arrived = *(volatile uint32_t*)slot;
+      if (arrived == (uint32_t)(n_tiles1 - 1)) {
+        __builtin_amdgcn_fence(__ATOMIC_ACQUIRE, "agent");
+        const int r0 = pmt * BM + wave * 64;
+        const int r1 = min(r0 + 64, p1.M);
+        const int64_t g0 = (int64_t)pb * p1.M + r0, g1 = (int64_t)pb * p1.M + r1;
+        switch (pr.iters) {
+          case 1: postnorm_wave_rows<1>(pr.ln, g0, g1); break;
+          case 2: postnorm_wave_rows<2>(pr.ln, g0, g1); break;
+          case 3: postnorm_wave_rows<3>(pr.ln, g0, g1); break;
+          case 4: postnorm_wave_rows<4>(pr.ln, g0, g1); break;
+          case 5: postnorm_wave_rows<5>(pr.ln, g0, g1); break;
+          default: postnorm_wave_rows<6>(pr.ln, g0, g1); break;
+        }
+      }
+    }
   }
 #ifdef ALG_GEMM_TAP
   if (threadIdx.x == 0 && blockIdx.x < 1024) {
@@ -1378,3 +1456,26 @@
   }
   return check_launch("alg_gemm_bf16");
 }
+
+template <int PIPE, int WNW>
+int launch_gemm_ln_mod(const alg_gemm_args* a, const alg_ln_mod_args* n, int m_tiles, int n_tiles, int64_t nwg, hipStream_t s) {
+  const void* fn = (const void*)gemm_bf16_kernel<ALG_ACT_NONE, true, PIPE, WNW, false, false, 0, 1>;
+  static PerDeviceOnce attr_set;
+  const int dev_slot = current_device_slot();
+  if (!device_done(attr_set, dev_slot)) {
+    hipError_t e = hipFuncSetAttribute(fn, hipFuncAttributeMaxDynamicSharedMemorySize, GEMM_LDS_P9);
+    if (e != hipSuccess) {
+      set_error("alg_gemm_bf16_ln_mod: hipFuncSetAttribute(%d B LDS): %s", GEMM_LDS_P9, hipGetErrorString(e));
+      return ALG_ELAUNCH;
+    }
+    device_mark(attr_set, dev_slot);
+  }
+  GemmPostNormArgs pn;
+  pn.ln = {(const bf16_t*)a->C, (bf16_t*)n->y, (const bf16_t*)n->weight, (const bf16_t*)n->bias, (const bf16_t*)n->scale,
+           (const bf16_t*)n->shift, n->mod_bstride, a->strideC, n->y_bstride, n->seg_stride, a->M, n->seg_split, n->eps};
+  pn.counters = (uint32_t*)n->counters;
+  pn.iters = a->N / 512;
+  hipLaunchKernelGGL((gemm_bf16_kernel<ALG_ACT_NONE, true, PIPE, WNW, false, false, 0, 1>), dim3(gemm_grid(nwg)), dim3(256),
+                     GEMM_LDS_P9, s, *a, m_tiles, n_tiles, gemm_group_m(PIPE, n_tiles, a->K), pn);
+  return check_launch("alg_gemm_bf16_ln_mod");
+}
diff --git a/alg_amd/csrc/gemm_p10.hip b/alg_amd/csrc/gemm_p10.hip
--- a/alg_amd/csrc/gemm_p10.hip
+++ b/alg_amd/csrc/gemm_p10.hip
@@ -49,6 +49,10 @@
                      GEMM_LDS_P9, s, *a, m_tiles_a, n_tiles_a, gemm_group_m(10, n_tiles_a, a->K), pr);
   return check_launch("alg_gemm_bf16_pair_qk");
 }
+
+int launch_gemm_p10_ln_mod(const alg_gemm_args* a, const alg_ln_mod_args* n, int m_tiles, int n_tiles, int64_t nwg, hipStream_t s) {
+  return launch_gemm_ln_mod<10, 2>(a, n, m_tiles, n_tiles, nwg, s);
+}
 }
 
 #ifdef ALG_GEMM_TAP
diff --git a/alg_amd/csrc/gemm_p11.hip b/alg_amd/csrc/gemm_p11.hip
--- a/alg_amd/csrc/gemm_p11.hip
+++ b/alg_amd/csrc/gemm_p11.hip
@@ -3,6 +3,17 @@
 namespace alg {
 int launch_gemm_p11(const alg_gemm_args* a, int m_tiles, int n_tiles, int64_t nwg, hipStream_t s) {
   return launch_gemm<11, 4>(a, m_tiles, n_tiles, nwg, s);
+}
+
+int launch_gemm_p11_ln_mod(const alg_gemm_args* a, const alg_ln_mod_args* n, int m_tiles, int n_tiles, int64_t nwg, hipStream_t s) {
+  return launch_gemm_ln_mod<11, 4>(a, n, m_tiles, n_tiles, nwg, s);
+}
+
+int gemm_group_m_of(int pipe, int n_tiles, int K) { return gemm_group_m(pipe, n_tiles, K) & 0xffff; }
+void gemm_tile_at(int L, int total, int m_tiles, int n_tiles, int group_m, int32_t* out3) {
+  int b, mt, nt;
+  gemm_tile_coords(gemm_tile_of_logical(L, total), m_tiles, n_tiles, group_m, &b, &mt, &nt);
+  out3[0] = b, out3[1] = mt, out3[2] = nt;
 }
 
 __global__ __launch_bounds__(256) void pack_b_p11_kernel(const bf16_t* __restrict__ w, uint4* __restrict__ out, int N, int K, int64_t ldb,
diff --git a/alg_amd/csrc/ln_mod.h b/alg_amd/csrc/ln_mod.h
--- /dev/null
+++ b/alg_amd/csrc/ln_mod.h
@@ -0,0 +1,114 @@
+#pragma once
+#include "common.h"
+#include "qk_norm_rope.h"
+
+namespace alg {
+
+struct LnModRows {
+  const bf16_t* x;
+  bf16_t* y;
+  const bf16_t *w, *bs;
+  const bf16_t *scale, *shift;
+  int64_t mod_bs, x_bs, y_bs, seg_stride;
+  int rows, seg_split;
+  float eps;
+};
+
+__device__ __forceinline__ float wave_sum(float v) {
+#pragma unroll
+  for (int m = 32; m >= 1; m >>= 1) v += __shfl_xor(v, m, 64);
+  return v;
+}
+
+template <int ITERS, int PF>
+__device__ __forceinline__ void ln_mod_wave_rows(const LnModRows& a, const int64_t row0, const int64_t row_end, const int lane) {
+#pragma clang fp contract(off)
+  constexpr int D = ITERS * 512;
+  if (row0 >= row_end) return;
+  uint4 wp[ITERS], bp[ITERS], s1p[ITERS], shp[ITERS];
+#pragma unroll
+  for (int i = 0; i < ITERS; ++i) {
+    wp[i] = *(const uint4*)(a.w + i * 512 + lane * 8);
+    bp[i] = *(const uint4*)(a.bs + i * 512 + lane * 8);
+  }
+  auto src = [&](int64_t row) -> const bf16_t* {
+    const int bidx = (int)(row / a.rows);
+    return a.x + (int64_t)bidx * a.x_bs + (int64_t)(row - (int64_t)bidx * a.rows) * D + lane * 8;
+  };
+  uint4 nxt[PF][ITERS];
+#pragma unroll
+  for (int j = 0; j < PF; ++j) {
+    if (row0 + j < row_end) {
+      const bf16_t* xr = src(row0 + j);
+#pragma unroll
+      for (int i = 0; i < ITERS; ++i) nxt[j][i] = *(const uint4*)(xr + i * 512);
+    }
+  }
+  int cur_key = -1;
+  for (int64_t base = row0; base < row_end; base += PF) {
+#pragma unroll
+    for (int j = 0; j < PF; ++j) {
+      const int64_t row = base + j;
+      if (row >= row_end) break;
+      float v[ITERS][8];
+      float s = 0.0f;
+#pragma unroll
+      for (int i = 0; i < ITERS; ++i) {
+        unpack8(nxt[j][i], v[i]);
+#pragma unroll
+        for (int k = 0; k < 8; ++k) s += v[i][k];
+      }
+      if (row + PF < row_end) {
+        const bf16_t* xr = src(row + PF);
+#pragma unroll
+        for (int i = 0; i < ITERS; ++i) nxt[j][i] = *(const uint4*)(xr + i * 512);
+      }
+      const int bidx = (int)(row / a.rows);
+      const int r = (int)(row - (int64_t)bidx * a.rows);
+      const int key = bidx * 2 + (r >= a.seg_split ? 1 : 0);
+      if (key != cur_key) {
+        cur_key = key;
+        const int64_t off = (int64_t)bidx * a.mod_bs + (int64_t)(key & 1) * a.seg_stride + lane * 8;
+#pragma unroll
+        for (int i = 0; i < ITERS; ++i) {
+          float scv[8];
+          unpack8(*(const uint4*)(a.scale + off + i * 512), scv);
+#pragma unroll
+          for (int k = 0; k < 8; ++k) scv[k] = 1.0f + scv[k];
+          s1p[i] = pack8(scv);
+          shp[i] = *(const uint4*)(a.shift + off + i * 512);
+        }
+      }
+      const float mean = wave_sum(s) * (1.0f / D);
+      float q = 0.0f;
+#pragma unroll
+      for (int i = 0; i < ITERS; ++i)
+#pragma unroll
+        for (int k = 0; k < 8; ++k) {
+          const float d = v[i][k] - mean;
+          q = fmaf(d, d, q);
+        }
+      const float var = wave_sum(q) * (1.0f / D);
+      const float rstd = rsqrtf(var + a.eps);
+      bf16_t* yr = a.y + (int64_t)bidx * a.y_bs + (int64_t)r * D + lane * 8;
+#pragma unroll
+      for (int i = 0; i < ITERS; ++i) {
+        float wv[8], bv[8], s1[8], shv[8], o[8];
+        unpack8(wp[i], wv);
+        unpack8(bp[i], bv);
+        unpack8(s1p[i], s1);
+        unpack8(shp[i], shv);
+#pragma unroll
+        for (int k = 0; k < 8; ++k) {
+          float n = (v[i][k] - mean) * rstd;
+          n = n * wv[k];
+          n = n + bv[k];
+          o[k] = rbf(rbf(rbf(n) * s1[k]) + shv[k]);
+        }
+        *(uint4*)(yr + i * 512) = pack8(o);
+      }
+    }
+  }
+}
+
+}
diff --git a/alg_amd/csrc/norm.hip b/alg_amd/csrc/norm.hip
--- a/alg_amd/csrc/norm.hip
+++ b/alg_amd/csrc/norm.hip
@@ -1,13 +1,8 @@
 #include "common.h"
+#include "ln_mod.h"
 #include "qk_norm_rope.h"
 
 namespace alg {
-
-__device__ __forceinline__ float wave_sum(float v) {
-#pragma unroll
-  for (int m = 32; m >= 1; m >>= 1) v += __shfl_xor(v, m, 64);
-  return v;
-}
 
 template <int ITERS>
 __global__ __launch_bounds__(256) void ln_mod_kernel(const bf16_t* __restrict__ x, bf16_t* __restrict__ y,
@@ -76,86 +71,12 @@
                                                           const bf16_t* __restrict__ shift, int64_t mod_bs, int64_t x_bs,
                                                           int64_t y_bs, int64_t total_rows, int rows, int seg_split,
                                                           int64_t seg_stride, float eps, int rpw) {
-  constexpr int D = ITERS * 512;
   const int lane = threadIdx.x & 63;
   const int64_t row0 = ((int64_t)blockIdx.x * 4 + (threadIdx.x >> 6)) * rpw;
   if (row0 >= total_rows) return;
   const int64_t row_end = row0 + rpw < total_rows ? row0 + rpw : total_rows;
-  uint4 wp[ITERS], bp[ITERS], s1p[ITERS], shp[ITERS];
-#pragma unroll
-  for (int i = 0; i < ITERS; ++i) {
-    wp[i] = *(const uint4*)(w + i * 512 + lane * 8);
-    bp[i] = *(const uint4*)(bs + i * 512 + lane * 8);
-  }
-  auto src = [&](int64_t row) -> const bf16_t* {
-    const int bidx = (int)(row / rows);
-    return x + (int64_t)bidx * x_bs + (int64_t)(row - (int64_t)bidx * rows) * D + lane * 8;
-  };
-  uint4 nxt[ITERS];
-  {
-    const bf16_t* xr = src(row0);
-#pragma unroll
-    for (int i = 0; i < ITERS; ++i) nxt[i] = *(const uint4*)(xr + i * 512);
-  }
-  int cur_key = -1;
-  for (int64_t row = row0; row < row_end; ++row) {
-    float v[ITERS][8];
-    float s = 0.0f;
-#pragma unroll
-    for (int i = 0; i < ITERS; ++i) {
-      unpack8(nxt[i], v[i]);
-#pragma unroll
-      for (int k = 0; k < 8; ++k) s += v[i][k];
-    }
-    if (row + 1 < row_end) {
-      const bf16_t* xr = src(row + 1);
-#pragma unroll
-      for (int i = 0; i < ITERS; ++i) nxt[i] = *(const uint4*)(xr + i * 512);
-    }
-    const int bidx = (int)(row / rows);
-    const int r = (int)(row - (int64_t)bidx * rows);
-    const int key = bidx * 2 + (r >= seg_split ? 1 : 0);
-    if (key != cur_key) {
-      cur_key = key;
-      const int64_t off = (int64_t)bidx * mod_bs + (int64_t)(key & 1) * seg_stride + lane * 8;
-#pragma unroll
-      for (int i = 0; i < ITERS; ++i) {
-        float scv[8];
-        unpack8(*(const uint4*)(scale + off + i * 512), scv);
-#pragma unroll
-        for (int k = 0; k < 8; ++k) scv[k] = 1.0f + scv[k];
-        s1p[i] = pack8(scv);
-        shp[i] = *(const uint4*)(shift + off + i * 512);
-      }
-    }
-    const float mean = wave_sum(s) * (1.0f / D);
-    float q = 0.0f;
-#pragma unroll
-    for (int i = 0; i < ITERS; ++i)
-#pragma unroll
-      for (int k = 0; k < 8; ++k) {
-        const float d = v[i][k] - mean;
-        q = fmaf(d, d, q);
-      }
-    const float rstd = rsqrtf(wave_sum(q) * (1.0f / D) + eps);
-    bf16_t* yr = y + (int64_t)bidx * y_bs + (int64_t)r * D + lane * 8;
-#pragma unroll
-    for (int i = 0; i < ITERS; ++i) {
-      float wv[8], bv[8], s1[8], shv[8], o[8];
-      unpack8(wp[i], wv);
-      unpack8(bp[i], bv);
-      unpack8(s1p[i], s1);
-      unpack8(shp[i], shv);
-#pragma unroll
-      for (int k = 0; k < 8; ++k) {
-        float n = (v[i][k] - mean) * rstd;
-        n = n * wv[k];
-        n = n + bv[k];
-        o[k] = rbf(rbf(rbf(n) * s1[k]) + shv[k]);
-      }
-      *(uint4*)(yr + i * 512) = pack8(o);
-    }
-  }
+  const LnModRows a = {x, y, w, bs, scale, shift, mod_bs, x_bs, y_bs, seg_stride, rows, seg_split, eps};
+  ln_mod_wave_rows<ITERS, 1>(a, row0, row_end, lane);
 }
 
 
diff --git a/alg_amd/transformer_cogvideox.py b/alg_amd/transformer_cogvideox.py
--- a/alg_amd/transformer_cogvideox.py
+++ b/alg_amd/transformer_cogvideox.py
@@ -76,6 +76,8 @@
         self.pair_qkv = True
         self.fuse_qk_norm = False
         self.packed_weights = True
+        self.fuse_norm_tail = True
+        self.fuse_norm_tail_out = True
         self._sincos = {}
         dev = self.device
         w = weights
@@ -403,14 +405,17 @@
         F4 = cfg.ff_inner_mult * D
         packed = self.packed_weights and os.environ.get("ALG_GEMM_PIPE", "10") == "10"
         wo_k, wf1_k, wf2_k = ("pwo", "pwf1", "pwf2") if packed else ("wo", "wf1", "wf2")
+        tail = bool(self.fuse_norm_tail) and not fp8
+        tail_out = tail and bool(self.fuse_norm_tail_out)
         for li, L in enumerate(self.layers):
             m1 = li * 12 * D
             m2 = m1 + 6 * D
             if fp8:
                 self._block_fp8(L, ws, q8, q8s, N, S, T, m1, m2, cos, sin, scale, q_scale, prescale)
                 continue
-            TM("ln_mod", _lib.layernorm_modulate, x, y, L["norm1_w"], L["norm1_b"], mod, mod, self.mod_cols, N, S, D,
-               T, cfg.norm_eps, scale_off=m1 + 2 * D, shift_off=m1)
+            if li == 0 or not tail:
+                TM("ln_mod", _lib.layernorm_modulate, x, y, L["norm1_w"], L["norm1_b"], mod, mod, self.mod_cols, N, S, D,
+                   T, cfg.norm_eps, scale_off=m1 + 2 * D, shift_off=m1)
             qk_call = ((y, L["wqk"], qk, S, 2 * D, D, D, D, 2 * D), dict(bias=L["bqk"], batch=N, strideA=S * D, strideC=S * 2 * D))
             vt_call = ((L["wv"], y, vt, D, S, D, D, D, S_pad), dict(bias=L["bv"], batch=N, strideB=S * D, strideC=D * S_pad,
                                                                    flags=_lib.GEMM_BIAS_PER_ROW | _lib.GEMM_PERMUTE_COLS))
@@ -427,14 +432,25 @@
                                    cfg.qk_norm_eps, q_scale=q_scale)
             TM("attn", _lib.flash_attn_d64, qk, qk, vt, att, N, Hn, S, S * 2 * D, 2 * D, D * S_pad, S_pad, S * D, D, scale,
                                 k_off=D, q_prescaled=prescale)
-            TM("gemm_out", G, att, L[wo_k], x, S, D, D, D, D, D, bias=L["bo"], R=x, ldr=D, gate=mod, gate_off=m1 + 4 * D,
-              strideGate=self.mod_cols, seg_split=T, batch=N, strideA=S * D, strideC=S * D, strideR=S * D)
-            TM("ln_mod", _lib.layernorm_modulate, x, y, L["norm2_w"], L["norm2_b"], mod, mod, self.mod_cols, N, S, D,
-               T, cfg.norm_eps, scale_off=m2 + 2 * D, shift_off=m2)
+            out_call = ((att, L[wo_k], x, S, D, D, D, D, D), dict(bias=L["bo"], R=x, ldr=D, gate=mod, gate_off=m1 + 4 * D,
+                        strideGate=self.mod_cols, seg_split=T, batch=N, strideA=S * D, strideC=S * D, strideR=S * D))
+            if tail_out:
+                TM("gemm_out", _lib.gemm_ln_mod, out_call, y, L["norm2_w"], L["norm2_b"], mod, mod, self.mod_cols, T, cfg.norm_eps,
+                   scale_off=m2 + 2 * D, shift_off=m2)
+            else:
+                TM("gemm_out", G, *out_call[0], **out_call[1])
+                TM("ln_mod", _lib.layernorm_modulate, x, y, L["norm2_w"], L["norm2_b"], mod, mod, self.mod_cols, N, S, D,
+                   T, cfg.norm_eps, scale_off=m2 + 2 * D, shift_off=m2)
             TM("gemm_ff1", G, y, L[wf1_k], h, S, F4, D, D, D, F4, bias=L["bf1"], act=_lib.ACT_GELU_TANH, batch=N, strideA=S * D,
               strideC=S * F4)
-            TM("gemm_ff2", G, h, L[wf2_k], x, S, D, F4, F4, F4, D, bias=L["bf2"], R=x, ldr=D, gate=mod, gate_off=m2 + 4 * D,
-              strideGate=self.mod_cols, seg_split=T, batch=N, strideA=S * F4, strideC=S * D, strideR=S * D)
+            ff2_call = ((h, L[wf2_k], x, S, D, F4, F4, F4, D), dict(bias=L["bf2"], R=x, ldr=D, gate=mod, gate_off=m2 + 4 * D,
+                        strideGate=self.mod_cols, seg_split=T, batch=N, strideA=S * F4, strideC=S * D, strideR=S * D))
+            if tail and li + 1 < len(self.layers):
+                Ln, mn = self.layers[li + 1], (li + 1) * 12 * D
+                TM("gemm_ff2", _lib.gemm_ln_mod, ff2_call, y, Ln["norm1_w"], Ln["norm1_b"], mod, mod, self.mod_cols, T,
+                   cfg.norm_eps, scale_off=mn + 2 * D, shift_off=mn)
+            else:
+                TM("gemm_ff2", G, *ff2_call[0], **ff2_call[1])
 
         _lib.layernorm_modulate(x, y, self.norm_final_w, self.norm_final_b, None, None, 0, N, S, D, T, cfg.norm_eps)
         mo = cfg.num_layers * 12 * D
diff --git a/include/alg_hip.h b/include/alg_hip.h
--- a/include/alg_hip.h
+++ b/include/alg_hip.h
@@ -103,6 +103,19 @@
 } alg_qk_norm_rope_args;
 int alg_gemm_bf16_pair_qk(const alg_gemm_args* qk, const alg_gemm_args* vt, const alg_qk_norm_rope_args* e, void* stream);
 
+typedef struct alg_ln_mod_args {
+  void* y;
+  const void *weight, *bias;
+  const void *scale, *shift;
+  int64_t mod_bstride, seg_stride, y_bstride;
+  int32_t seg_split;
+  float eps;
+  void* counters;
+} alg_ln_mod_args;
+int alg_gemm_bf16_ln_mod(const alg_gemm_args* g, const alg_ln_mod_args* n, void* stream);
+int64_t alg_gemm_ln_mod_counters_bytes(int M, int batch);
+int64_t alg_gemm_ln_mod_tiles(int M, int N, int K, int batch, int schedule, int32_t* out);
+
 int alg_gemm_fp8(const alg_gemm_args* args, void* stream);
 
 int alg_quantize_fp8_rows(const void* x, int64_t x_rstride, void* q, float* scale, int64_t rows, int K, void* stream);
```
